# TropComplique/MultiPoseNet

Hardware: AMD Instinct MI355X
Metric: images/sec keypoint fwd+bwd+Adam @512x512 bs32/GPU (higher is better)
Workload: dtype bf16; 1 GPU; MobileNet-v1+FPN+keypoint_subnet fwd+bwd+Adam, 512x512, per-GPU batch 32; global_batch=32, parallelism=dp1, hip_graph=True, rccl_ranks=1

## Files before the change

### include/mpn.h

```cpp
#ifndef MPN_H_
#define MPN_H_

#include <stddef.h>
#include <stdint.h>

#ifdef __cplusplus
extern "C" {
#endif

#define MPN_VERSION 600

enum { MPN_F32 = 0, MPN_BF16 = 1, MPN_F16 = 2  };

enum {
    MPN_OK = 0,
    MPN_ERR_BAD_SHAPE = -1,
    MPN_ERR_BAD_DTYPE = -2,
    MPN_ERR_BAD_ALIGN = -3,
    MPN_ERR_HIP = -4,
    MPN_ERR_BAD_ARG = -5,
    MPN_ERR_WORKSPACE = -6,
    MPN_ERR_BAD_DATA = -7
};

enum { MPN_ACT_NONE = 0, MPN_ACT_RELU = 1, MPN_ACT_RELU6 = 2 };

typedef void* mpn_stream_t;

int mpn_version(void);
int mpn_last_error(char* buf, size_t n);

size_t mpn_heatmap_decode_workspace_bytes(int B);
int mpn_heatmap_decode(const void* heatmaps, int dtype, int B, int h, int w, int C,
                       const double* box_hw, float threshold,
                       int32_t* out_xyv, float* out_score, int32_t* out_index,
                       void* workspace, size_t workspace_bytes, mpn_stream_t stream);

size_t mpn_conv_packed_bytes(int Cin, int Cout, int ksize, int transpose, int dtype);
int mpn_conv_pack_weights(const float* w_hwio, int Cin, int Cout, int ksize, int transpose,
                          int dtype, void* out, mpn_stream_t stream);
size_t mpn_conv_pack_desc_bytes(void);
int mpn_conv_pack_desc_fill(void* desc_host, const float* w_hwio, int Cin, int Cout, int ksize, int transpose,
                            int dtype, void* out, int block_begin);
int mpn_conv_pack_weights_batched(const void* descs_device, int ndesc, int total_blocks, int dtype,
                                  mpn_stream_t stream);
int mpn_conv_num_parts(int N, int H, int W, int ksize);
int mpn_conv_stats_rows(int N, int H, int W, int Cin, int Cout, int ksize, int dtype);
int mpn_conv_fwd(const void* x, const void* w_packed, void* y, int N, int H, int W, int Cin,
                 int Cout, int x_stride, int y_stride, int ksize, int dtype, const float* in_scale,
                 const float* in_shift, int in_act, float* stats_part, const void* up_res,
                 mpn_stream_t stream);
int mpn_conv_fwd_grouped(int njobs, const void* const* x, const void* const* w_packed, void* const* y, int N, const int* H,
                         const int* W, int Cin, int Cout, const int* x_stride, const int* y_stride, int ksize, int dtype,
                         const float* const* in_scale, const float* const* in_shift, int in_act,
                         float* const* stats_part, mpn_stream_t stream);
int mpn_conv_bwd_data_bn_supported(int K, int C, int ksize, int dtype);
int mpn_conv_bwd_data_bn(const void* dy, const void* w_packed_t, void* dx, int N, int H, int W, int K, int C, int dy_stride,
                         int dx_stride, int ksize, int dtype, const void* bn_x, int bn_x_stride, const float* bn_scale,
                         const float* bn_shift, int bn_act, float* part, mpn_stream_t stream);
int mpn_conv_bwd_data_bn_grouped(int njobs, const void* const* dy, const void* const* w_packed_t, void* const* dx, int N,
                                 const int* H, const int* W, int K, int C, const int* dy_stride, const int* dx_stride,
                                 int dtype, const void* const* bn_x, const int* bn_x_stride, const float* const* bn_scale,
                                 const float* const* bn_shift, int bn_act, float* const* part, mpn_stream_t stream);

int mpn_conv_wgrad_num_parts(int N, int H, int W, int Cin, int Cout, int ksize, int dtype);
int mpn_conv_bwd_weight(const void* x, const void* dy, float* part, int N, int H, int W, int Cin,
                        int Cout, int x_stride, int dy_stride, int ksize, int dtype, const float* in_scale,
                        const float* in_shift, int in_act, mpn_stream_t stream);

int mpn_conv1x1_bwd_fused_supported(int Cin, int Cout, int dtype);
int mpn_conv1x1_bwd_fused(const void* x, const void* dy, const float* w, void* dx, float* wpart, float* bn_part, int N, int H, int W,
                          int Cin, int Cout, int x_stride, int dy_stride, int dx_stride, int dtype, const float* in_scale,
                          const float* in_shift, int in_act, mpn_stream_t stream);
int mpn_conv1x1_bwd_fused_apply_supported(int Cin, int Cout, int dtype);
int mpn_conv1x1_bwd_fused_apply(const void* x, const void* g, const void* y_raw, const float* w, void* dx, float* wpart, float* bn_part,
                                int N, int H, int W, int Cin, int Cout, int x_stride, int g_stride, int y_stride, int dx_stride,
                                int dtype, const float* in_scale, const float* in_shift, int in_act, const float* ap_scale,
                                const float* ap_shift, const float* ap_mean, const float* ap_invstd, const float* ap_k1,
                                const float* ap_k2, int ap_act, mpn_stream_t stream);
int mpn_conv_wgrad_grouped_num_parts(int njobs, int N, const int* H, const int* W, int Cin, int Cout, int ksize, int dtype,
                                     int* nparts);
int mpn_conv_bwd_weight_grouped(int njobs, const void* const* x, const void* const* dy, float* const* part, int N,
                                const int* H, const int* W, int Cin, int Cout, const int* x_stride, const int* dy_stride,
                                int ksize, int dtype, const float* const* in_scale, const float* const* in_shift,
                                int in_act, mpn_stream_t stream);

int mpn_bn_stats_num_parts(long long M);
int mpn_bn_stats(const void* x, long long M, int C, int dtype, float* part, mpn_stream_t stream);
int mpn_bn_finalize(float* part, int nparts, int C, long long count, const float* gamma,
                    const float* beta, float* moving_mean, float* moving_var, float momentum,
                    float eps, float* scale, float* shift, float* save_mean, float* save_invstd,
                    mpn_stream_t stream);
int mpn_bn_bwd_reduce_grouped(int njobs, void* const* dA, const void* const* x, const long long* M, int C, int dtype,
                              const float* const* scale, const float* const* shift, const float* const* mean,
                              const float* const* invstd, int act, float* const* part, const int* dA_stride,
                              const int* x_stride, mpn_stream_t stream);
int mpn_bn_bwd_apply_grouped(int njobs, void* const* dA, const void* const* x, const long long* M, int C, int dtype,
                             const float* const* scale, const float* const* shift, const float* const* mean,
                             const float* const* invstd, const float* const* k1, const float* const* k2, int act,
                             const float* const* add_ch0, const int* dA_stride, const int* x_stride,
                             mpn_stream_t stream);
size_t mpn_bn_fin_desc_bytes(void);
size_t mpn_bn_bwd_fin_desc_bytes(void);
int mpn_bn_fin_desc_fill(void* desc_host, const float* part, int nparts, int C, long long count, const float* gamma,
                         const float* beta, float* moving_mean, float* moving_var, float* scale, float* shift,
                         float* save_mean, float* save_invstd, int block_begin);
int mpn_bn_bwd_fin_desc_fill(void* desc_host, const float* part, int nparts, int C, long long count, float* dgamma,
                             float* dbeta, float* k1, float* k2, int block_begin);
int mpn_bn_bwd_fin_desc_fill_raw(void* desc_host, const float* part, int nparts, int C, long long count, float* dgamma,
                                 float* dbeta, float* k1, float* k2, const float* mean, const float* invstd,
                                 int block_begin);
int mpn_bn_finalize_batched(const void* descs_device, int ndesc, int total_blocks, float momentum, float eps,
                            mpn_stream_t stream);
int mpn_bn_bwd_finalize_batched(const void* descs_device, int ndesc, int total_blocks, mpn_stream_t stream);
int mpn_bn_inference_affine(int C, const float* gamma, const float* beta, const float* moving_mean,
                            const float* moving_var, float eps, float* scale, float* shift,
                            mpn_stream_t stream);
int mpn_bn_act_apply(const void* x, void* y, long long M, int C, int dtype, const float* scale,
                     const float* shift, int act, mpn_stream_t stream);
int mpn_bn_bwd_reduce(const void* dA, const void* x, long long M, int C, int dtype,
                      const float* scale, const float* shift, const float* mean,
                      const float* invstd, int act, float* part, mpn_stream_t stream);
int mpn_bn_bwd_finalize(float* part, int nparts, int C, long long count, float* dgamma,
                        float* dbeta, float* k1, float* k2, mpn_stream_t stream);
int mpn_bn_bwd_finalize_raw(float* part, int nparts, int C, long long count, float* dgamma, float* dbeta, float* k1,
                            float* k2, const float* mean, const float* invstd, mpn_stream_t stream);
int mpn_bn_bwd_apply(void* dA, const void* x, long long M, int C, int dtype, const float* scale,
                     const float* shift, const float* mean, const float* invstd, const float* k1,
                     const float* k2, int act, const float* add_ch0, mpn_stream_t stream);

int mpn_dwconv_out_size(int size, int stride);
int mpn_dwconv_num_parts(int N, int H, int W, int C, int stride, int dtype);
int mpn_dwconv_fwd(const void* x, const float* w, void* y, int N, int H, int W, int C, int stride,
                   int dtype, const float* in_scale, const float* in_shift, int in_act, int flip,
                   float* stats_part, mpn_stream_t stream);
int mpn_dwconv_bwd_data(const void* dy, const float* w, void* dx, int N, int H, int W, int C,
                        int stride, int dtype, mpn_stream_t stream);
int mpn_dwconv_bwd_data_bn_num_parts(int N, int H, int W, int C, int stride, int dtype);
int mpn_dwconv_bwd_data_bn(const void* dy, const float* w, void* dx, int N, int H, int W, int C, int stride, int dtype,
                           const void* x_bn, const float* scale, const float* shift, const float* mean,
                           const float* invstd, int act, float* part, mpn_stream_t stream);
int mpn_dwconv_bwd_data_add_supported(int N, int H, int W, int C, int stride, int dtype);
int mpn_dwconv_bwd_data_add(const void* dy, const float* w, void* dx, int N, int H, int W, int C, int stride, int dtype,
                            const void* addend, const void* x_bn, const float* scale, const float* shift,
                            const float* mean, const float* invstd, int act, float* part, mpn_stream_t stream);
int mpn_dwconv_wgrad_num_parts(int N, int H, int W, int C, int stride, int dtype);
int mpn_dwconv_bwd_weight(const void* x, const void* dy, float* part, int N, int H, int W, int C,
                          int stride, int dtype, const float* in_scale, const float* in_shift,
                          int in_act, mpn_stream_t stream);

int mpn_dwconv_bwd_fused_supported(int N, int H, int W, int C, int stride, int dtype);
int mpn_dwconv_bwd_fused(const void* x, const void* dy, const float* w, void* dx, float* wpart, int N, int H, int W, int C,
                         int dtype, const float* in_scale, const float* in_shift, int in_act, const float* mean,
                         const float* invstd, float* bn_part, mpn_stream_t stream);
int mpn_dwconv_bwd_fused_s2(const void* x, const void* dy, const float* w, void* dx, float* wpart, int N, int H, int W, int C,
                            int dtype, const float* in_scale, const float* in_shift, int in_act, const float* mean,
                            const float* invstd, float* bn_part, const void* addend, mpn_stream_t stream);
int mpn_dwconv_bwd_fused_apply_supported(int N, int H, int W, int C, int stride, int dtype);
int mpn_dwconv_bwd_fused_apply(const void* x, const void* g, const void* y_raw, const float* w, void* dx, float* wpart, int N, int H,
                               int W, int C, int dtype, const float* in_scale, const float* in_shift, int in_act, const float* mean,
                               const float* invstd, float* bn_part, const float* ap_scale, const float* ap_shift,
                               const float* ap_mean, const float* ap_invstd, const float* ap_k1, const float* ap_k2, int ap_act,
                               mpn_stream_t stream);
int mpn_dwconv_bwd_fused_s2_apply(const void* x, const void* g, const void* y_raw, const float* w, void* dx, float* wpart, int N, int H,
                                  int W, int C, int dtype, const float* in_scale, const float* in_shift, int in_act,
                                  const float* mean, const float* invstd, float* bn_part, const void* addend, const float* ap_scale,
                                  const float* ap_shift, const float* ap_mean, const float* ap_invstd, const float* ap_k1,
                                  const float* ap_k2, int ap_act, mpn_stream_t stream);

int mpn_stem_conv_fwd(const void* images, int images_u8, const float* w, void* y, int N, int H,
                      int W, int C0, int dtype, mpn_stream_t stream);
int mpn_stem_conv_fwd_num_parts(int N, int H, int W, int C0, int dtype);
int mpn_stem_conv_fwd_stats(const void* images, int images_u8, const float* w, void* y, int N, int H, int W, int C0,
                            int dtype, float* stats_part, mpn_stream_t stream);
int mpn_stem_conv_wgrad_num_parts(int N, int H, int W);
int mpn_stem_conv_bwd_weight(const void* images, int images_u8, const void* dy, float* part, int N,
                             int H, int W, int C0, int dtype, mpn_stream_t stream);

int mpn_bilinear_up_fwd(const void* x, void* y, int N, int h, int w, int C, int upsample,
                        int y_channel_offset, int y_channels_total, int dtype,
                        const float* in_scale, const float* in_shift, int in_act,
                        mpn_stream_t stream);
int mpn_bilinear_up_bwd(const void* dy, void* dx, int N, int h, int w, int C, int upsample,
                        int y_channel_offset, int y_channels_total, int dtype, mpn_stream_t stream);
int mpn_sumpool2x2(const void* src, void* dst, int N, int h, int w, int C, int accumulate,
                   int dtype, mpn_stream_t stream);
int mpn_add_inplace(void* dst, const void* src, long long n, int dtype, mpn_stream_t stream);

int mpn_heatmap_head_fwd(const void* x, const float* w, const float* bias, long long M, int Cin,
                         int dtype, const float* in_scale, const float* in_shift, int in_act,
                         int mode, float* out, float* out_seg, mpn_stream_t stream);
int mpn_heatmap_head_bwd_num_parts(long long M);
int mpn_heatmap_head_bwd(const void* x, const float* dlogits, const float* w, long long M, int Cin,
                         int dtype, const float* in_scale, const float* in_shift, int in_act,
                         void* dA, float* part, mpn_stream_t stream);
int mpn_heatmap_head_bwd_bn_supported(int Cin, int dtype);
int mpn_heatmap_head_bwd_bn(const void* x, const float* dlogits, const float* w, long long M, int Cin, int dtype,
                            const float* in_scale, const float* in_shift, int in_act, void* dA, float* part,
                            float* bn_part, mpn_stream_t stream);

int mpn_keypoint_loss_num_parts(int B, int h, int w);
int mpn_keypoint_loss(const float* logits, const float* heatmaps, const float* loss_masks,
                      const float* segmentation_masks, const int* num_boxes, const void* p2,
                      const void* p3, const void* p4, const void* p5, int p_channels, int p_dtype,
                      float* dlogits, float* daux2, float* daux3, float* daux4, float* daux5,
                      float* part, float* losses_out, int B, int h, int w, mpn_stream_t stream);

int mpn_adam_prepare(long long* step, float* hyper, double initial_learning_rate,
                     double decay_steps, double alpha, double beta1, double beta2,
                     mpn_stream_t stream);
int mpn_adam_step(float* params, const float* grads, float* m, float* v, long long n,
                  const float* hyper, float beta1, float beta2, float eps, float clip,
                  float grad_scale, mpn_stream_t stream);
int mpn_adam_step_cast(float* params, const float* grads, float* m, float* v, long long n, const float* hyper, float beta1,
                       float beta2, float eps, float clip, float grad_scale, int ncast, const long long* cast_begin,
                       const long long* cast_count, void* const* cast_dst, int cast_dtype, mpn_stream_t stream);
int mpn_reduce_partials(const float* part, int nparts, long long n, float* out, int accumulate,
                        float scale, mpn_stream_t stream);
size_t mpn_reduce_desc_bytes(void);
int mpn_reduce_desc_fill(void* desc_host, const float* part, int nparts, long long n, float* out, float scale,
                         int block_begin);
int mpn_reduce_partials_batched(const void* descs_device, int ndesc, int total_blocks, mpn_stream_t stream);
int mpn_axpy(long long n, float a, const float* x, float* y, mpn_stream_t stream);
int mpn_axpy_batched(int count, const float* const* x, float* const* y, const long long* n, float a, mpn_stream_t stream);
int mpn_l2_loss_accumulate(long long n, const float* w, float scale, float* acc, mpn_stream_t stream);
size_t mpn_l2_loss_batched_workspace_bytes(int count, const long long* n);
int mpn_l2_loss_batched(int count, const float* const* w, const long long* n, float scale, float* acc, void* workspace,
                        size_t workspace_bytes, mpn_stream_t stream);

size_t mpn_heatmap_render_workspace_bytes(int total_persons);
int mpn_heatmap_render(const int32_t* keypoints, const float* boxes, const int32_t* first_person,
                       int B, int total_persons, int width, int height, int downsample, float* out,
                       void* workspace, size_t workspace_bytes, mpn_stream_t stream);

enum {
    MPN_AUGMENT_ROTATE = 1, MPN_AUGMENT_COLOR = 2, MPN_AUGMENT_GRAYSCALE = 4, MPN_AUGMENT_PIXEL_SCALE = 8,
    MPN_AUGMENT_FLIP = 16, MPN_AUGMENT_EVAL = 32
};
#define MPN_KEYPOINT_AUGMENT_DESC_BYTES 192
typedef struct mpn_keypoint_augment_desc {
    int64_t src_offset, mask_offset;
    int32_t src_h, src_w, mask_h, mask_w;
    int32_t crop_y, crop_x, crop_h, crop_w;
    int32_t valid_h, valid_w, valid_mh, valid_mw;
    float transform[8], mask_transform[8];
    float window[4];
    float scale_y, scale_x;
    float mask_scale_y, mask_scale_x;
    float color[3];
    uint32_t seed;
    int32_t flags;
    int32_t reserved[3];
} mpn_keypoint_augment_desc;
#ifdef __cplusplus
static_assert(sizeof(mpn_keypoint_augment_desc) == MPN_KEYPOINT_AUGMENT_DESC_BYTES, "descriptor size is fixed");
#endif
size_t mpn_keypoint_augment_desc_bytes(void);
int mpn_keypoint_augment(const uint8_t* sources, const uint8_t* masks, const void* descs, int B, int H, int W,
                         float* images, float* loss_masks, float* segmentation_masks, mpn_stream_t stream);

// ... 358 lines not shown
```

### multiposenet_amd/_lib.py

```python
import ctypes
import os

_HERE = os.path.dirname(os.path.abspath(__file__))
LIB_PATH = os.environ.get("MPN_LIB") or os.path.join(_HERE, "libmpn_hip.so")

MPN_VERSION = 600
MPN_F32, MPN_BF16, MPN_F16 = 0, 1, 2
ACT_NONE, ACT_RELU, ACT_RELU6 = 0, 1, 2

_c = ctypes
_P = _c.c_void_p
_I = _c.c_int
_F = _c.c_float
_D = _c.c_double
_Z = _c.c_size_t
_L = _c.c_longlong

SIGNATURES = {
    "mpn_version": (_I, []),
    "mpn_last_error": (_I, [_c.c_char_p, _Z]),
    "mpn_heatmap_decode_workspace_bytes": (_Z, [_I]),
    "mpn_heatmap_decode": (_I, [_P, _I, _I, _I, _I, _I, _P, _F, _P, _P, _P, _P, _Z, _P]),
    "mpn_heatmap_render_workspace_bytes": (_Z, [_I]),
    "mpn_heatmap_render": (_I, [_P, _P, _P, _I, _I, _I, _I, _I, _P, _P, _Z, _P]),
    "mpn_keypoint_augment_desc_bytes": (_Z, []),
    "mpn_keypoint_augment": (_I, [_P, _P, _P, _I, _I, _I, _P, _P, _P, _P]),
    "mpn_detector_augment_desc_bytes": (_Z, []),
    "mpn_detector_augment": (_I, [_P, _P, _I, _I, _I, _P, _P]),
    "mpn_prn_example_desc_bytes": (_Z, []),
    "mpn_prn_examples_workspace_bytes": (_Z, [_I]),
    "mpn_prn_examples": (_I, [_P, _P, _I, _P, _P, _P, _I, _P, _I, _I, _I, _I, _P, _P, _P, _Z, _P]),
    "mpn_conv_packed_bytes": (_Z, [_I, _I, _I, _I, _I]),
    "mpn_conv_pack_weights": (_I, [_P, _I, _I, _I, _I, _I, _P, _P]),
    "mpn_conv_pack_desc_bytes": (_Z, []),
    "mpn_conv_pack_desc_fill": (_I, [_P, _P, _I, _I, _I, _I, _I, _P, _I]),
    "mpn_conv_pack_weights_batched": (_I, [_P, _I, _I, _I, _P]),
    "mpn_conv_num_parts": (_I, [_I, _I, _I, _I]),
    "mpn_conv_stats_rows": (_I, [_I, _I, _I, _I, _I, _I, _I]),
    "mpn_conv_fwd": (_I, [_P, _P, _P, _I, _I, _I, _I, _I, _I, _I, _I, _I, _P, _P, _I, _P, _P, _P]),
    "mpn_conv_fwd_grouped": (_I, [_I, _P, _P, _P, _I, _P, _P, _I, _I, _P, _P, _I, _I, _P, _P, _I, _P, _P]),
    "mpn_conv_wgrad_num_parts": (_I, [_I, _I, _I, _I, _I, _I, _I]),
    "mpn_conv_bwd_weight": (_I, [_P, _P, _P, _I, _I, _I, _I, _I, _I, _I, _I, _I, _P, _P, _I, _P]),
    "mpn_conv1x1_bwd_fused_supported": (_I, [_I, _I, _I]),
    "mpn_conv1x1_bwd_fused": (_I, [_P, _P, _P, _P, _P, _P, _I, _I, _I, _I, _I, _I, _I, _I, _I, _P, _P, _I, _P]),
    "mpn_conv1x1_bwd_fused_apply_supported": (_I, [_I, _I, _I]),
    "mpn_conv1x1_bwd_fused_apply": (_I, [_P, _P, _P, _P, _P, _P, _P, _I, _I, _I, _I, _I, _I, _I, _I, _I, _I, _P, _P, _I, _P, _P, _P, _P, _P, _P, _I, _P]),
    "mpn_conv_wgrad_grouped_num_parts": (_I, [_I, _I, _P, _P, _I, _I, _I, _I, _P]),
    "mpn_conv_bwd_weight_grouped": (_I, [_I, _P, _P, _P, _I, _P, _P, _I, _I, _P, _P, _I, _I, _P, _P, _I, _P]),
    "mpn_bn_stats_num_parts": (_I, [_L]),
    "mpn_bn_stats": (_I, [_P, _L, _I, _I, _P, _P]),
    "mpn_bn_finalize": (_I, [_P, _I, _I, _L, _P, _P, _P, _P, _F, _F, _P, _P, _P, _P, _P]),
    "mpn_bn_inference_affine": (_I, [_I, _P, _P, _P, _P, _F, _P, _P, _P]),
    "mpn_bn_act_apply": (_I, [_P, _P, _L, _I, _I, _P, _P, _I, _P]),
    "mpn_bn_bwd_reduce": (_I, [_P, _P, _L, _I, _I, _P, _P, _P, _P, _I, _P, _P]),
    "mpn_bn_bwd_finalize": (_I, [_P, _I, _I, _L, _P, _P, _P, _P, _P]),
    "mpn_bn_bwd_apply": (_I, [_P, _P, _L, _I, _I, _P, _P, _P, _P, _P, _P, _I, _P, _P]),
    "mpn_dwconv_out_size": (_I, [_I, _I]),
    "mpn_dwconv_num_parts": (_I, [_I, _I, _I, _I, _I, _I]),
    "mpn_dwconv_fwd": (_I, [_P, _P, _P, _I, _I, _I, _I, _I, _I, _P, _P, _I, _I, _P, _P]),
    "mpn_dwconv_bwd_data": (_I, [_P, _P, _P, _I, _I, _I, _I, _I, _I, _P]),
    "mpn_dwconv_bwd_data_bn_num_parts": (_I, [_I, _I, _I, _I, _I, _I]),
    "mpn_dwconv_bwd_data_bn": (_I, [_P, _P, _P, _I, _I, _I, _I, _I, _I, _P, _P, _P, _P, _P, _I, _P, _P]),
    "mpn_dwconv_bwd_data_add_supported": (_I, [_I, _I, _I, _I, _I, _I]),
    "mpn_dwconv_bwd_data_add": (_I, [_P, _P, _P, _I, _I, _I, _I, _I, _I, _P, _P, _P, _P, _P, _P, _I, _P, _P]),
    "mpn_dwconv_wgrad_num_parts": (_I, [_I, _I, _I, _I, _I, _I]),
    "mpn_dwconv_bwd_weight": (_I, [_P, _P, _P, _I, _I, _I, _I, _I, _I, _P, _P, _I, _P]),
    "mpn_dwconv_bwd_fused_supported": (_I, [_I, _I, _I, _I, _I, _I]),
    "mpn_dwconv_bwd_fused": (_I, [_P, _P, _P, _P, _P, _I, _I, _I, _I, _I, _P, _P, _I, _P, _P, _P, _P]),
    "mpn_dwconv_bwd_fused_s2": (_I, [_P, _P, _P, _P, _P, _I, _I, _I, _I, _I, _P, _P, _I, _P, _P, _P, _P, _P]),
    "mpn_dwconv_bwd_fused_apply_supported": (_I, [_I, _I, _I, _I, _I, _I]),
    "mpn_dwconv_bwd_fused_apply": (_I, [_P, _P, _P, _P, _P, _P, _I, _I, _I, _I, _I, _P, _P, _I, _P, _P, _P, _P, _P, _P, _P, _P, _P, _I, _P]),
    "mpn_dwconv_bwd_fused_s2_apply": (_I, [_P, _P, _P, _P, _P, _P, _I, _I, _I, _I, _I, _P, _P, _I, _P, _P, _P, _P, _P, _P, _P, _P, _P, _P, _I, _P]),
    "mpn_stem_conv_fwd": (_I, [_P, _I, _P, _P, _I, _I, _I, _I, _I, _P]),
    "mpn_stem_conv_fwd_num_parts": (_I, [_I, _I, _I, _I, _I]),
    "mpn_stem_conv_fwd_stats": (_I, [_P, _I, _P, _P, _I, _I, _I, _I, _I, _P, _P]),
    "mpn_stem_conv_wgrad_num_parts": (_I, [_I, _I, _I]),
    "mpn_stem_conv_bwd_weight": (_I, [_P, _I, _P, _P, _I, _I, _I, _I, _I, _P]),
    "mpn_bilinear_up_fwd": (_I, [_P, _P, _I, _I, _I, _I, _I, _I, _I, _I, _P, _P, _I, _P]),
    "mpn_bilinear_up_bwd": (_I, [_P, _P, _I, _I, _I, _I, _I, _I, _I, _I, _P]),
    "mpn_sumpool2x2": (_I, [_P, _P, _I, _I, _I, _I, _I, _I, _P]),
    "mpn_add_inplace": (_I, [_P, _P, _L, _I, _P]),
    "mpn_heatmap_head_fwd": (_I, [_P, _P, _P, _L, _I, _I, _P, _P, _I, _I, _P, _P, _P]),
    "mpn_heatmap_head_bwd_num_parts": (_I, [_L]),
    "mpn_heatmap_head_bwd": (_I, [_P, _P, _P, _L, _I, _I, _P, _P, _I, _P, _P, _P]),
    "mpn_heatmap_head_bwd_bn_supported": (_I, [_I, _I]),
    "mpn_heatmap_head_bwd_bn": (_I, [_P, _P, _P, _L, _I, _I, _P, _P, _I, _P, _P, _P, _P]),
    "mpn_keypoint_loss_num_parts": (_I, [_I, _I, _I]),
    "mpn_keypoint_loss": (_I, [_P] * 9 + [_I, _I] + [_P] * 7 + [_I, _I, _I, _P]),
    "mpn_adam_prepare": (_I, [_P, _P, _D, _D, _D, _D, _D, _P]),
    "mpn_adam_step": (_I, [_P, _P, _P, _P, _L, _P, _F, _F, _F, _F, _F, _P]),
    "mpn_adam_step_cast": (_I, [_P, _P, _P, _P, _L, _P, _F, _F, _F, _F, _F, _I, _P, _P, _P, _I, _P]),
    "mpn_reduce_partials": (_I, [_P, _I, _L, _P, _I, _F, _P]),
    "mpn_reduce_desc_bytes": (_Z, []),
    "mpn_reduce_desc_fill": (_I, [_P, _P, _I, _L, _P, _F, _I]),
    "mpn_reduce_partials_batched": (_I, [_P, _I, _I, _P]),
    "mpn_gemm_nt_num_parts": (_I, [_I]),
    "mpn_gemm_nt": (_I, [_P, _P, _P, _I, _I, _I, _I, _P]),
    "mpn_transpose_cast": (_I, [_P, _I, _P, _I, _I, _I, _P]),
    "mpn_cast": (_I, [_P, _I, _P, _I, _L, _P]),
    "mpn_bias_relu_fwd": (_I, [_P, _I, _P, _P, _I, _I, _I, _P]),
    "mpn_bias_relu_bwd": (_I, [_P, _I, _P, _P, _I, _P, _I, _I, _P]),
    "mpn_prn_loss": (_I, [_P, _P, _I, _P, _I, _I, _I, _P, _P, _P, _F, _P]),
    "mpn_bn_bwd_reduce_grouped": (_I, [_I, _P, _P, _P, _I, _I, _P, _P, _P, _P, _I, _P, _P, _P, _P]),
    "mpn_bn_bwd_apply_grouped": (_I, [_I, _P, _P, _P, _I, _I, _P, _P, _P, _P, _P, _P, _I, _P, _P, _P, _P]),
    "mpn_bn_fin_desc_bytes": (_Z, []),
    "mpn_bn_bwd_fin_desc_bytes": (_Z, []),
    "mpn_bn_fin_desc_fill": (_I, [_P, _P, _I, _I, _L, _P, _P, _P, _P, _P, _P, _P, _P, _I]),
    "mpn_bn_bwd_fin_desc_fill": (_I, [_P, _P, _I, _I, _L, _P, _P, _P, _P, _I]),
    "mpn_bn_finalize_batched": (_I, [_P, _I, _I, _F, _F, _P]),
    "mpn_bn_bwd_finalize_batched": (_I, [_P, _I, _I, _P]),
    "mpn_heatmap_minmax": (_I, [_P, _I, _I, _I, _I, _P, _P]),
    "mpn_prn_crop": (_I, [_P, _P, _P, _P, _I, _I, _I, _I, _I, _I, _I, _F, _P, _P]),
    "mpn_prn_decode": (_I, [_P, _I, _I, _I, _I, _P, _P, _P]),
    "mpn_conv_bwd_data_bn_supported": (_I, [_I, _I, _I, _I]),
    "mpn_conv_bwd_data_bn": (_I, [_P, _P, _P, _I, _I, _I, _I, _I, _I, _I, _I, _I, _P, _I, _P, _P, _I, _P, _P]),
    "mpn_bn_bwd_finalize_raw": (_I, [_P, _I, _I, _L, _P, _P, _P, _P, _P, _P, _P]),
    "mpn_conv_bwd_data_bn_grouped": (_I, [_I, _P, _P, _P, _I, _P, _P, _I, _I, _P, _P, _I, _P, _P, _P, _P, _I, _P, _P]),
    "mpn_bn_bwd_fin_desc_fill_raw": (_I, [_P, _P, _I, _I, _L, _P, _P, _P, _P, _P, _P, _I]),
    "mpn_prn_crop_slots": (_I, [_P, _P, _P, _P, _I, _I, _I, _I, _I, _I, _I, _I, _I, _F, _P, _P]),
    "mpn_prn_residual": (_I, [_P, _P, _I, _L, _P, _P]),
    "mpn_retina_loss_finalize": (_I, [_P, _P, _F, _F, _P, _P, _P, _P]),
    "mpn_axpy": (_I, [_L, _F, _P, _P, _P]),
    "mpn_axpy_batched": (_I, [_I, _P, _P, _P, _F, _P]),
    "mpn_patchify3x3s2": (_I, [_P, _P, _I, _I, _I, _I, _I, _P, _P, _I, _P]),
    "mpn_unpatchify3x3s2": (_I, [_P, _P, _I, _I, _I, _I, _I, _P]),
    "mpn_retina_match_workspace_bytes": (_Z, [_I, _I]),
    "mpn_retina_match": (_I, [_P, _P, _P, _I, _I, _I, _F, _F, _P, _P, _P, _P, _Z, _P]),
    "mpn_retina_loss_num_parts": (_I, [_I, _I]),
    "mpn_retina_loss": (_I, [_P, _P, _P, _P, _P, _P, _I, _P, _P, _P, _P, _P, _I, _F, _F, _F, _F, _P, _P]),
    "mpn_retina_nms_workspace_bytes": (_Z, [_I, _I]),
    "mpn_retina_nms_overflow_offset": (_Z, [_I, _I]),
    "mpn_retina_nms": (_I, [_P, _P, _P, _P, _I, _P, _P, _P, _I, _F, _F, _I, _P, _P, _P, _P, _Z, _P]),
    "mpn_l2_loss_accumulate": (_I, [_L, _P, _F, _P, _P]),
    "mpn_l2_loss_batched_workspace_bytes": (_Z, [_I, _P]),
    "mpn_l2_loss_batched": (_I, [_I, _P, _P, _F, _P, _P, _Z, _P]),
    "mpn_pose_gather_record_bytes": (_Z, [_I, _I]),
    "mpn_pose_gather_row_offset": (_Z, [_I, _I, _I]),
    "mpn_pose_gather": (_I, [_P, _P, _P, _P, _P, _P, _I, _I, _F, _I, _I, _P, _Z, _P]),
    "mpn_pose_gather_sized": (_I, [_P, _P, _P, _P, _P, _P, _I, _I, _F, _P, _P, _Z, _P]),
    "mpn_oks_gt_row_bytes": (_Z, []),
    "mpn_oks_match_out_bytes": (_Z, [_I, _I]),
    "mpn_oks_match": (_I, [_P, _I, _I, _P, _P, _I, _P, _I, _I, _I, _P, _P, _P]),
    "mpn_pose_nms_info_bytes": (_Z, [_I, _I]),
    "mpn_pose_nms": (_I, [_P, _I, _I, _F, _F, _I, _P, _Z, _P, _Z, _P, _P]),
    "mpn_pose_track_state_bytes": (_Z, [_I, _I]),
    "mpn_pose_track_out_bytes": (_Z, [_I, _I]),
    "mpn_pose_track": (_I, [_P, _I, _I, _I, _I, _I, _F, _F, _I, _P, _P, _P, _P]),
    "mpn_pose_track_optimal": (_I, [_P, _I, _I, _I, _I, _I, _F, _F, _I, _P, _P, _P, _P]),
    "mpn_pose_track_motion_state_bytes": (_Z, [_I, _I]),
    "mpn_pose_track_coast_bytes": (_Z, [_I, _I]),
    "mpn_pose_track_motion": (_I, [_P, _I, _I, _I, _I, _I, _I, _F, _F, _I, _F, _F, _P, _P, _P, _P, _P, _P, _P]),
    "mpn_pose_smooth_state_bytes": (_Z, [_I, _I]),
    "mpn_pose_smooth_out_bytes": (_Z, [_I, _I]),
    "mpn_pose_smooth": (_I, [_P, _P, _I, _I, _I, _I, _F, _F, _F, _F, _F, _P, _P, _P, _P]),
    "mpn_coco_masks_image_desc_bytes": (_Z, []),
    "mpn_coco_masks_part_desc_bytes": (_Z, []),
    "mpn_coco_masks_plane_words": (_Z, [_I, _I]),
    "mpn_coco_masks_packed_bytes": (_Z, [_I, _I]),
    "mpn_coco_masks": (_I, [_P, _I, _I, _P, _I, _P, _L, _P, _L, _P, _L, _P, _Z, _P, _Z, _P, _Z, _P]),
    "mpn_image_resize_desc_bytes": (_Z, []),
# ... 169 lines not shown
```

### multiposenet_amd/csrc/conv_wgrad.hip

```cpp
#include "common.h"
#include <type_traits>

namespace {

template <typename T> using HT = H16<std::conditional_t<sizeof(T) == 2, T, bf16_t>>;
typedef float f32x4_t __attribute__((ext_vector_type(4)));

constexpr int kThreads = 256;
constexpr int kHaloW = 18, kHaloH = 10;

struct WgradParams {
    const void* x;
    const void* dy;
    float* part;
    const float* in_scale;
    const float* in_shift;
    int in_act;
    int N, H, W, Cin, Cout;
    int xs, dys;
    int tiles_x, tiles_y;
    long long M;
    int ntiles;
    int nsplit;
    int n_cg, n_cb;
    int xcd_remap;
    const float* wf;
    void* dx;
    int dxs;
    float* bn_part;
    const void* ap_x;
    int ap_xs;
    const float* ap_scale; const float* ap_shift; const float* ap_mean; const float* ap_invstd; const float* ap_k1; const float* ap_k2;
    int ap_act;
#ifdef MPN_DIAG
    unsigned long long* dbg;
#endif
};

__device__ __forceinline__ int fsw256(int r) { return (r & 3) | (((r >> 3) & 1) << 2); }
__device__ __forceinline__ int fsw64(int) { return 0; }
__device__ __forceinline__ int fsw128(int r) { return ((r >> 1) & 1) | (((r >> 3) & 1) << 1); }

template <int RB> __device__ __forceinline__ int lds_off(int row, int seg, int within) {
    const int f = (RB == 64) ? fsw64(row) : (RB == 128 ? fsw128(row) : fsw256(row));
    return row * RB + ((seg ^ f) << 5) + within;
}

template <typename T> struct Raw4h { uint2 v; };
__device__ __forceinline__ void raw4_unpack(const Raw4h<bf16_t>& r, float (&f)[4]) {
    f[0] = __uint_as_float(r.v.x << 16); f[1] = __uint_as_float(r.v.x & 0xffff0000u);
    f[2] = __uint_as_float(r.v.y << 16); f[3] = __uint_as_float(r.v.y & 0xffff0000u);
}
__device__ __forceinline__ void raw4_unpack(const Raw4h<half_t>& r, float (&f)[4]) {
    typedef _Float16 h2_t __attribute__((ext_vector_type(2)));
    const h2_t a = __builtin_bit_cast(h2_t, r.v.x), b = __builtin_bit_cast(h2_t, r.v.y);
    f[0] = (float)a[0]; f[1] = (float)a[1]; f[2] = (float)b[0]; f[3] = (float)b[1];
}
template <typename T> __device__ __forceinline__ float round_to_storage(float v);
template <> __device__ __forceinline__ float round_to_storage<bf16_t>(float v) { return to_f32((bf16_t)v); }
template <> __device__ __forceinline__ float round_to_storage<half_t>(float v) { return (float)(_Float16)v; }
template <typename T> __device__ __forceinline__ uint2 pack4_storage(const float (&g)[4]);
template <> __device__ __forceinline__ uint2 pack4_storage<bf16_t>(const float (&g)[4]) {
    return make_uint2(pack_bf16x2(g[0], g[1]), pack_bf16x2(g[2], g[3]));
}
template <> __device__ __forceinline__ uint2 pack4_storage<half_t>(const float (&g)[4]) {
    typedef _Float16 h2_t __attribute__((ext_vector_type(2)));
    const h2_t a = {(_Float16)g[0], (_Float16)g[1]}, b = {(_Float16)g[2], (_Float16)g[3]};
    return make_uint2(__builtin_bit_cast(unsigned, a), __builtin_bit_cast(unsigned, b));
}

template <typename H> __device__ __forceinline__ typename H::x4 tr_read(const unsigned char* base, int off) {
    return H::tr_read(base + off);
}

template <typename T, int TAPS, int RBA, int RBD>
__global__ __launch_bounds__(kThreads, 2) void conv_wgrad_kernel(const WgradParams p) {
    constexpr int ES = (int)sizeof(T);
    constexpr int VE = 16 / ES;
    constexpr int CG = RBA / ES;
    constexpr int BNW = RBD / ES;
    constexpr int DSLOTS = RBD / 16;
    constexpr int NPIXA = TAPS == 9 ? kHaloW * kHaloH : 128;
    constexpr int MT_TOTAL = CG / 16, NT_TOTAL = BNW / 16;
    constexpr int WM = MT_TOTAL >= 2 ? 2 : 1;
    constexpr int WN = 4 / WM;
    constexpr int MTW = MT_TOTAL / WM;
    constexpr int NTW = NT_TOTAL / WN;
    constexpr int KPIX = ES == 2 ? 32 : 4;
    constexpr int KSTEPS = 128 / KPIX;
    constexpr int ASLOTS = RBA / 16;
    constexpr int AVEC = (NPIXA * ASLOTS + kThreads - 1) / kThreads;
    constexpr int DVEC = 128 * DSLOTS / kThreads;

    extern __shared__ __attribute__((aligned(16))) unsigned char smem[];
    unsigned char* As = smem;
    unsigned char* Ds = smem + NPIXA * RBA;

    const int tid = threadIdx.x;
    const int lane = tid & 63, wave = tid >> 6;
    const int l15 = lane & 15, lq = lane >> 4;

    int b;
    {
        const int nwg = gridDim.x, q = nwg >> 3, r = nwg & 7, xcd = blockIdx.x & 7, k = blockIdx.x >> 3;
        b = (xcd < r ? xcd * (q + 1) : r * (q + 1) + (xcd - r) * q) + k;
    }
    const int cg = b % p.n_cg; b /= p.n_cg;
    const int cb = b % p.n_cb;
    const int split = b / p.n_cb;
    const int ci0 = cg * CG, co0 = cb * BNW;

    const int mt0 = (wave / WN) * MTW;
    const int nt0 = (wave % WN) * NTW;

    f32x4_t acc[TAPS][MTW][NTW];
#pragma unroll
// ... 166 lines not shown
    for (int t = 0; t < TAPS; ++t)
#pragma unroll
        for (int i = 0; i < MTW; ++i)
#pragma unroll
            for (int j = 0; j < NTW; ++j)
#pragma unroll
                for (int r = 0; r < 4; ++r) {
                    const int ci = ci0 + (mt0 + i) * 16 + lq * 4 + r;
                    const int co = co0 + (nt0 + j) * 16 + l15;
                    if (ci < p.Cin && co < p.Cout)
                        dst[((long long)t * p.Cin + ci) * p.Cout + co] = acc[t][i][j][r];
                }
}

template <typename T, int TAPS, int RBA, int RBD, int WM, bool STAGGER, bool DG = false, bool DAPPLY = false>
__device__ __forceinline__ void conv_wgrad_bf16_body(const WgradParams& p, const int blk, const int nblk) {
    using H = H16<T>;
    using X8 = typename H::x8;
    using X4 = typename H::x4;
    constexpr int NT = 512;
    constexpr int VE = 8;
    constexpr int CG = RBA / 2, BNW = RBD / 2;
    constexpr int ASLOTS = RBA / 16, DSLOTS = RBD / 16;
    constexpr int NPIXA = TAPS == 9 ? kHaloW * kHaloH : 128;
    constexpr int MT_TOTAL = CG / 16, NT_TOTAL = BNW / 16;
    constexpr int WN = 8 / WM;
    constexpr int MTW = MT_TOTAL / WM, NTW = NT_TOTAL / WN;
    static_assert(MTW * WM == MT_TOTAL && NTW * WN == NT_TOTAL, "wave layout must tile the block");
    constexpr int AVEC = (NPIXA * ASLOTS + NT - 1) / NT;
    constexpr int DVEC = 128 * DSLOTS / NT;
    constexpr int SA = RBA + 32, SD = RBD + 32;
    constexpr int ABYTES = NPIXA * SA, DBYTES = 128 * SD;
    static_assert(!DG || (TAPS == 1 && !STAGGER), "the fused data gradient: 1x1, waves in step");
    constexpr int OS = RBA + 16;
    constexpr int RBYTES = DG ? 128 * SA : 0, OBYTES = DG ? 128 * OS : 0;
    constexpr int KS2 = BNW / 32;

    constexpr int NBUF = DG ? 1 : 2;
    extern __shared__ __attribute__((aligned(16))) unsigned char smem[];
    float* aff = reinterpret_cast<float*>(smem + NBUF * ABYTES + NBUF * DBYTES);
    unsigned char* Rs = smem + NBUF * ABYTES + NBUF * DBYTES + 2 * CG * (int)sizeof(float);
    unsigned char* Os = Rs + RBYTES;

    const int tid = threadIdx.x;
    const int lane = tid & 63, wave = tid >> 6;
    const int l15 = lane & 15, lq = lane >> 4;

    int b = blk;
    if (p.xcd_remap) {
        const int nwg = nblk, q = nwg >> 3, r = nwg & 7, xcd = blk & 7, k = blk >> 3;
        b = (xcd < r ? xcd * (q + 1) : r * (q + 1) + (xcd - r) * q) + k;
    }
    const int cg = b % p.n_cg; b /= p.n_cg;
    const int cb = b % p.n_cb;
    const int split = b / p.n_cb;
    const int ci0 = cg * CG, co0 = cb * BNW;
    const int mt0 = (wave / WN) * MTW, nt0 = (wave % WN) * NTW;

    f32x4_t acc[TAPS][MTW][NTW];
#pragma unroll
    for (int t = 0; t < TAPS; ++t)
#pragma unroll
        for (int i = 0; i < MTW; ++i)
#pragma unroll
            for (int j = 0; j < NTW; ++j) acc[t][i][j] = (f32x4_t){0.f, 0.f, 0.f, 0.f};

    const T* __restrict__ x = reinterpret_cast<const T*>(p.x);
    const T* __restrict__ dy = reinterpret_cast<const T*>(p.dy);
    const bool affine = p.in_scale != nullptr;
    const float lo = (affine && p.in_act != MPN_ACT_NONE) ? 0.f : -INFINITY;
    const float hi = (affine && p.in_act == MPN_ACT_RELU6) ? 6.f : INFINITY;
    for (int c = tid; c < CG; c += NT) {
        const bool ok = affine && ci0 + c < p.Cin;
        aff[c] = ok ? p.in_scale[ci0 + c] : 1.f;
        aff[CG + c] = ok ? p.in_shift[ci0 + c] : 0.f;
    }

    const int aslot = tid % ASLOTS;
    const int dslot = tid % DSLOTS;

    Vec16<T> v[AVEC], dv[DVEC];
    Vec16<T> ev[DAPPLY ? DVEC : 1];
    unsigned inb = 0u, inbd = 0u;
    static_assert(!DAPPLY || DG, "the apply pass folds into the fused thin backward");
    float* apc = reinterpret_cast<float*>(Os + OBYTES + (DG ? 8 * 2 * CG * (int)sizeof(float) : 0));
    float alo = -INFINITY, ahi = INFINITY;
    if constexpr (DAPPLY) {
        for (int c = tid; c < BNW; c += NT) {
            const bool ok = co0 + c < p.Cout;
            const float s_ = ok ? p.ap_scale[co0 + c] : 0.f, h_ = ok ? p.ap_shift[co0 + c] : 0.f, m_ = ok ? p.ap_mean[co0 + c] : 0.f;
            const float i_ = ok ? p.ap_invstd[co0 + c] : 0.f, a_ = ok ? p.ap_k1[co0 + c] : 0.f, b_ = ok ? p.ap_k2[co0 + c] : 0.f;
            apc[c] = s_; apc[BNW + c] = h_;
            apc[2 * BNW + c] = -s_ * b_ * i_;
            apc[3 * BNW + c] = -s_ * (a_ - m_ * i_ * b_);
        }
        alo = (p.ap_act != MPN_ACT_NONE) ? 0.f : -INFINITY;
        ahi = (p.ap_act == MPN_ACT_RELU6) ? 6.f : INFINITY;
    }

    int relA[AVEC], hyx[AVEC], relD[DVEC];
    {
        const int ace = ci0 + aslot * VE, dce = co0 + dslot * VE;
#pragma unroll
        for (int i = 0; i < AVEC; ++i) {
            const int vi = tid + i * NT;
            const int pix = vi / ASLOTS;
            const bool ok = ace < p.Cin && vi < NPIXA * ASLOTS;
            if (TAPS == 9) {
                const int hy = pix / kHaloW, hx = pix - hy * kHaloW;
                relA[i] = ((hy - 1) * p.W + (hx - 1)) * p.xs + ace;
                hyx[i] = ok ? (hy << 8 | hx) : 0x7fff00;
            } else {
                relA[i] = pix * p.xs + ace;
                hyx[i] = ok ? pix : 0x7fffffff;
            }
        }
#pragma unroll
        for (int i = 0; i < DVEC; ++i) {
            const int r = (tid / DSLOTS) + i * (NT / DSLOTS);
            relD[i] = (TAPS == 9 ? ((r >> 4) * p.W + (r & 15)) : r) * p.dys + dce;
        }
    }
    const bool dvalid = co0 + dslot * VE < p.Cout;
    const int drow0 = tid / DSLOTS;
    constexpr bool BUF = TAPS == 1;
    typedef unsigned u32x4_t __attribute__((ext_vector_type(4)));
    unsigned relAb[BUF ? AVEC : 1], relDb[BUF ? DVEC : 1], relEb[(BUF && DAPPLY) ? DVEC : 1];
    __amdgpu_buffer_rsrc_t rsx, rsd, rse;
    if constexpr (BUF) {
        constexpr unsigned kOut = 0x80000000u;
#pragma unroll
        for (int i = 0; i < AVEC; ++i) relAb[i] = hyx[i] == 0x7fffffff ? kOut : (unsigned)relA[i] * (unsigned)sizeof(T);
#pragma unroll
        for (int i = 0; i < DVEC; ++i) relDb[i] = dvalid ? (unsigned)relD[i] * (unsigned)sizeof(T) : kOut;
        rsx = __builtin_amdgcn_make_buffer_rsrc(const_cast<T*>(x), 0, (int)(((p.M - 1) * p.xs + p.Cin) * (long long)sizeof(T)), 0x00020000);
        rsd = __builtin_amdgcn_make_buffer_rsrc(const_cast<T*>(dy), 0, (int)(((p.M - 1) * p.dys + p.Cout) * (long long)sizeof(T)), 0x00020000);
        if constexpr (DAPPLY) {
#pragma unroll
            for (int i = 0; i < DVEC; ++i)
                relEb[i] = dvalid ? (unsigned)((drow0 + i * (NT / DSLOTS)) * p.ap_xs + co0 + dslot * VE) * (unsigned)sizeof(T) : kOut;
            rse = __builtin_amdgcn_make_buffer_rsrc(const_cast<void*>(p.ap_x), 0, (int)(((p.M - 1) * p.ap_xs + p.Cout) * (long long)sizeof(T)), 0x00020000);
        }
    }

    auto load_tile = [&](int tile) {
        if constexpr (BUF) {
            const unsigned tbA = (unsigned)tile * 128u * (unsigned)p.xs * (unsigned)sizeof(T);
            const unsigned tbD = (unsigned)tile * 128u * (unsigned)p.dys * (unsigned)sizeof(T);
            if constexpr (DAPPLY) {
                const int mleft = (int)(p.M - (long long)tile * 128);
                unsigned md = 0u;
#pragma unroll
                for (int i = 0; i < DVEC; ++i) md |= ((dvalid && drow0 + i * (NT / DSLOTS) < mleft) ? 1u : 0u) << i;
                inbd = md;
            }
            __builtin_amdgcn_sched_barrier(0);
#pragma unroll
            for (int i = 0; i < AVEC; ++i) {
                const u32x4_t q = __builtin_amdgcn_raw_buffer_load_b128(rsx, (int)(relAb[i] + tbA), 0, 0);
                v[i].raw = make_uint4(q.x, q.y, q.z, q.w);
            }
#pragma unroll
            for (int i = 0; i < DVEC; ++i) {
                const u32x4_t q = __builtin_amdgcn_raw_buffer_load_b128(rsd, (int)(relDb[i] + tbD), 0, 0);
                dv[i].raw = make_uint4(q.x, q.y, q.z, q.w);
            }
            if constexpr (DAPPLY) {
                const unsigned tbE = (unsigned)tile * 128u * (unsigned)p.ap_xs * (unsigned)sizeof(T);
#pragma unroll
                for (int i = 0; i < DVEC; ++i) {
                    const u32x4_t q = __builtin_amdgcn_raw_buffer_load_b128(rse, (int)(relEb[i] + tbE), 0, 0);
                    ev[i].raw = make_uint4(q.x, q.y, q.z, q.w);
                }
            }
            __builtin_amdgcn_sched_barrier(0);
            return;
        }
        int oy0 = 0, ox0 = 0, baseA, baseD, mleft = 0;
        if (TAPS == 9) {
            const int tx = tile % p.tiles_x;
            const int t2 = tile / p.tiles_x;
            const int ty = t2 % p.tiles_y;
            const int img = t2 / p.tiles_y;
            oy0 = ty * 8;
            ox0 = tx * 16;
            const int pix0 = (img * p.H + oy0) * p.W + ox0;
            baseA = pix0 * p.xs;
            baseD = pix0 * p.dys;
        } else {
            baseA = tile * 128 * p.xs;
            baseD = tile * 128 * p.dys;
            mleft = (int)(p.M - (long long)tile * 128);
        }
        int oa[AVEC], od[DVEC];
        unsigned ma = 0u, md = 0u;
#pragma unroll
        for (int i = 0; i < AVEC; ++i) {
            bool ok;
            if (TAPS == 9) {
                const int iy = oy0 + (hyx[i] >> 8) - 1, ix = ox0 + (hyx[i] & 255) - 1;
                ok = (unsigned)iy < (unsigned)p.H && (unsigned)ix < (unsigned)p.W;
            } else {
                ok = hyx[i] < mleft;
            }
            oa[i] = ok ? baseA + relA[i] : 0;
            ma |= (ok ? 1u : 0u) << i;
        }
#pragma unroll
        for (int i = 0; i < DVEC; ++i) {
            const int r = drow0 + i * (NT / DSLOTS);
            bool ok = dvalid;
            if (TAPS == 9) ok = ok && oy0 + (r >> 4) < p.H && ox0 + (r & 15) < p.W;
            else ok = ok && r < mleft;
            od[i] = ok ? baseD + relD[i] : 0;
            md |= (ok ? 1u : 0u) << i;
        }
        inb = ma;
        inbd = md;
        __builtin_amdgcn_sched_barrier(0);
#pragma unroll
        for (int i = 0; i < AVEC; ++i) v[i].load(x + oa[i]);
#pragma unroll
        for (int i = 0; i < DVEC; ++i) dv[i].load(dy + od[i]);
        if constexpr (DAPPLY) {
            const T* __restrict__ ax = reinterpret_cast<const T*>(p.ap_x);
#pragma unroll
            for (int i = 0; i < DVEC; ++i) {
                const int r = drow0 + i * (NT / DSLOTS);
                const bool ok = (inbd >> i) & 1u;
                ev[i].load(ax + (ok ? (long long)(tile * 128 + r) * p.ap_xs + co0 + dslot * VE : 0));
            }
        }
        __builtin_amdgcn_sched_barrier(0);
    };

    auto commit_tile = [&](unsigned char* As, unsigned char* Ds) {
        float sc[VE], sh[VE];
        if (affine) {
#pragma unroll
            for (int j = 0; j < VE; j += 4) {
                const float4 a = *reinterpret_cast<const float4*>(aff + aslot * VE + j);
                const float4 c = *reinterpret_cast<const float4*>(aff + CG + aslot * VE + j);
                sc[j] = a.x; sc[j + 1] = a.y; sc[j + 2] = a.z; sc[j + 3] = a.w;
                sh[j] = c.x; sh[j + 1] = c.y; sh[j + 2] = c.z; sh[j + 3] = c.w;
            }
        }
#pragma unroll
        for (int i = 0; i < AVEC; ++i) {
            const int vi = tid + i * NT;
            if (vi < NPIXA * ASLOTS) {
                const int pix = vi / ASLOTS;
                uint4 q = *reinterpret_cast<const uint4*>(&v[i].raw);
                if (affine) {
                    float f[VE];
                    v[i].unpack(f);
#pragma unroll
                    for (int j = 0; j < VE; ++j) f[j] = __builtin_amdgcn_fmed3f(f[j] * sc[j] + sh[j], lo, hi);
                    Vec16<T> o;
                    o.pack(f);
                    q = *reinterpret_cast<const uint4*>(&o.raw);
                }
                if (!BUF && !((inb >> i) & 1u)) q = make_uint4(0u, 0u, 0u, 0u);
                *reinterpret_cast<uint4*>(As + pix * SA + aslot * 16) = q;
                if constexpr (DG) {
                    uint4 r = *reinterpret_cast<const uint4*>(&v[i].raw);
                    if (!BUF && !((inb >> i) & 1u)) r = make_uint4(0u, 0u, 0u, 0u);
                    *reinterpret_cast<uint4*>(Rs + pix * SA + aslot * 16) = r;
                }
            }
        }
#pragma unroll
        for (int i = 0; i < DVEC; ++i) {
            const int r = (tid / DSLOTS) + i * (NT / DSLOTS);
            uint4 q = *reinterpret_cast<const uint4*>(&dv[i].raw);
            if constexpr (DAPPLY) {
                float d[VE], f[VE], asc[VE], ash[VE], acb[VE], acc_[VE];
                dv[i].unpack(d);
                ev[i].unpack(f);
#pragma unroll
                for (int j4 = 0; j4 < VE; j4 += 4) {
                    const f32x4_t q0 = *reinterpret_cast<const f32x4_t*>(apc + dslot * VE + j4), q1 = *reinterpret_cast<const f32x4_t*>(apc + BNW + dslot * VE + j4);
                    const f32x4_t q2 = *reinterpret_cast<const f32x4_t*>(apc + 2 * BNW + dslot * VE + j4), q3 = *reinterpret_cast<const f32x4_t*>(apc + 3 * BNW + dslot * VE + j4);
#pragma unroll
                    for (int j = 0; j < 4; ++j) { asc[j4 + j] = q0[j]; ash[j4 + j] = q1[j]; acb[j4 + j] = q2[j]; acc_[j4 + j] = q3[j]; }
                }
#pragma unroll
                for (int j = 0; j < VE; ++j) {
                    const float pre = f[j] * asc[j] + ash[j];
                    const float gg = (pre > alo && pre < ahi) ? d[j] : 0.f;
                    d[j] = asc[j] * gg + (acb[j] * f[j] + acc_[j]);
                }
                Vec16<T> o;
                o.pack(d);
                q = *reinterpret_cast<const uint4*>(&o.raw);
            }
            if ((!BUF || DAPPLY) && !((inbd >> i) & 1u)) q = make_uint4(0u, 0u, 0u, 0u);
            *reinterpret_cast<uint4*>(Ds + r * SD + dslot * 16) = q;
        }
    };

#ifdef MPN_DIAG
    unsigned long long ph[4] = {0, 0, 0, 0}, t_prev = 0;
#define MPN_WG_STAMP(k) do { if (p.dbg) { const unsigned long long t_ = __builtin_amdgcn_s_memtime(); \
                                          ph[k] += t_ - t_prev; t_prev = t_; } } while (0)
#else
#define MPN_WG_STAMP(k) do { } while (0)
#endif
    const int grp = STAGGER ? wave >> 2 : 0;
    const int ntl = p.ntiles > split ? (p.ntiles - split + p.nsplit - 1) / p.nsplit : 0;
    const int ahead = 1 + grp;
    constexpr int DGS = MT_TOTAL >= 8 ? 4 : (MT_TOTAL >= 4 ? 2 : 1), MTH = MT_TOTAL / DGS;
    const int dg_mt0 = DG ? (wave % DGS) * MTH : 0, dg_pt0 = DG ? (wave / DGS) * DGS : 0;
    X8 wfr[DG ? MTH : 1][DG ? KS2 : 1];
    float bsum[DG ? MTH : 1][4], bsq[DG ? MTH : 1][4];
    if constexpr (DG) {
#pragma unroll
        for (int mt = 0; mt < MTH; ++mt) {
#pragma unroll
            for (int ks = 0; ks < KS2; ++ks) {
                const int ci = ci0 + (dg_mt0 + mt) * 16 + l15, co = co0 + ks * 32 + lq * 8;
                float f[8];
#pragma unroll
                for (int j = 0; j < 8; ++j) f[j] = (ci < p.Cin && co + j < p.Cout) ? p.wf[(long long)ci * p.Cout + co + j] : 0.f;
                Vec16<T> o;
                o.pack(f);
                wfr[mt][ks] = __builtin_bit_cast(X8, o.raw);
            }
#pragma unroll
            for (int r = 0; r < 4; ++r) { bsum[mt][r] = 0.f; bsq[mt][r] = 0.f; }
        }
    }
    if (ntl > 0) load_tile(split);
    __syncthreads();
    if (ntl > 0) commit_tile(smem, smem + NBUF * ABYTES);
    if (grp == 1) {
        if (ntl > 1) load_tile(split + p.nsplit);
        __syncthreads();
        if (ntl > 1) commit_tile(smem + ABYTES, smem + NBUF * ABYTES + DBYTES);
    }
#ifdef MPN_DIAG
    if (p.dbg) t_prev = __builtin_amdgcn_s_memtime();
#endif
#pragma unroll 1
    for (int it = 0; it < ntl; ++it) {
        const int buf = NBUF == 2 ? (it & 1) : 0;
        unsigned char* As = smem + buf * ABYTES;
        unsigned char* Ds = smem + NBUF * ABYTES + buf * DBYTES;
        const bool more = it + ahead < ntl;
        if (more) load_tile(split + (it + ahead) * p.nsplit);
        MPN_WG_STAMP(1);
        __syncthreads();
        MPN_WG_STAMP(2);
        const int qq = l15 >> 2, pp = l15 & 3;
        const unsigned char* a_lane = As + (4 * lq + qq) * SA + pp * 8 + mt0 * 32;
        const unsigned char* d_lane = Ds + (4 * lq + qq) * SD + pp * 8 + nt0 * 32;
        constexpr int STEPS = TAPS * MTW;
        constexpr int TOTAL = 4 * STEPS;
        constexpr int RING0 = NTW >= 4 ? 4 : ((TAPS == 9 && RBA == 256) ? 4 : 6);
        constexpr int RING = RING0 < STEPS ? RING0 : STEPS;
        constexpr int KSA = (TAPS == 9 ? 2 * kHaloW : 32) * SA, KSD = 32 * SD;
        auto a_load = [&](int gs) -> X8 {
            const int ks = gs / STEPS, step = gs % STEPS;
            const int t = step / MTW, i = step % MTW;
            const int row = TAPS == 9 ? (t / 3) * kHaloW + (t % 3) : 0;
            const int second = TAPS == 9 ? kHaloW : 16;
            const X4 l4 = tr_read<H>(a_lane, ks * KSA + row * SA + i * 32);
            const X4 h4 = tr_read<H>(a_lane, ks * KSA + (row + second) * SA + i * 32);
            return __builtin_shufflevector(l4, h4, 0, 1, 2, 3, 4, 5, 6, 7);
        };
        auto b_load = [&](int ks, int j) -> X8 {
            const X4 l4 = tr_read<H>(d_lane, ks * KSD + j * 32);
            const X4 h4 = tr_read<H>(d_lane, ks * KSD + 16 * SD + j * 32);
            return __builtin_shufflevector(l4, h4, 0, 1, 2, 3, 4, 5, 6, 7);
        };
        X8 bfr[2][NTW];
        X8 ar[RING];
#pragma unroll
        for (int j = 0; j < NTW; ++j) bfr[0][j] = b_load(0, j);
#pragma unroll
        for (int r = 0; r < RING - 1; ++r) ar[r] = a_load(r);
// ... 40 lines not shown
                        const float pre = xf[r] * sc4[r] + sh4[r];
                        const float d = round_to_storage<T>(dacc[mt][r]);
                        g[r] = (!bnr || (pre > lo && pre < hi)) ? d : 0.f;
                        bsum[mt][r] += g[r];
                        bsq[mt][r] += g[r] * xf[r];
                    }
                    *reinterpret_cast<uint2*>(Os + px * OS + cl * 2) = pack4_storage<T>(g);
                }
            }
        }
        MPN_WG_STAMP(3);
        __syncthreads();
        MPN_WG_STAMP(2);
        if (more) {
            const int nb = NBUF == 2 ? ((it + ahead) & 1) : 0;
            commit_tile(smem + nb * ABYTES, smem + NBUF * ABYTES + nb * DBYTES);
        }
        if constexpr (DG) {
            const int tile = split + it * p.nsplit;
            const int mleft = (int)(p.M - (long long)tile * 128);
            T* __restrict__ dxp = reinterpret_cast<T*>(p.dx) + (long long)tile * 128 * p.dxs + ci0;
            for (int v0 = tid; v0 < 128 * ASLOTS; v0 += NT) {
                const int pr = v0 / ASLOTS, sl = v0 - pr * ASLOTS;
                if (pr < mleft && ci0 + sl * 8 < p.Cin)
                    *reinterpret_cast<uint4*>(dxp + (long long)pr * p.dxs + sl * 8) = *reinterpret_cast<const uint4*>(Os + pr * OS + sl * 16);
            }
        }
        MPN_WG_STAMP(0);
    }
    if (STAGGER && grp == 0) __syncthreads();
#ifdef MPN_DIAG
    if (p.dbg && lane == 0) {
#pragma unroll
        for (int k = 0; k < 4; ++k) p.dbg[((size_t)blockIdx.x * 8 + wave) * 4 + k] = ph[k];
    }
#endif
#undef MPN_WG_STAMP

    if constexpr (DG) {
        float* red = reinterpret_cast<float*>(Os + OBYTES);
        __syncthreads();
        for (int o = tid; o < 8 * 2 * CG; o += NT) red[o] = 0.f;
        __syncthreads();
#pragma unroll
        for (int mt = 0; mt < MTH; ++mt)
#pragma unroll
            for (int r = 0; r < 4; ++r) {
                float a = bsum[mt][r], b = bsq[mt][r];
#pragma unroll
                for (int o = 1; o < 16; o <<= 1) { a += __shfl_xor(a, o, 64); b += __shfl_xor(b, o, 64); }
                if (l15 == 0) {
                    red[(wave * 2 + 0) * CG + (dg_mt0 + mt) * 16 + lq * 4 + r] = a;
                    red[(wave * 2 + 1) * CG + (dg_mt0 + mt) * 16 + lq * 4 + r] = b;
                }
            }
        __syncthreads();
        for (int o = tid; o < 2 * CG; o += NT) {
            const int which = o / CG, c = o - which * CG;
            if (p.bn_part != nullptr && ci0 + c < p.Cin) {
                float a = 0.f;
#pragma unroll
                for (int w8 = 0; w8 < 8; ++w8) a += red[(w8 * 2 + which) * CG + c];
                p.bn_part[((long long)split * 2 + which) * p.Cin + ci0 + c] = a;
            }
        }
    }
    float* __restrict__ dst = p.part + (long long)split * TAPS * p.Cin * p.Cout;
#pragma unroll
    for (int t = 0; t < TAPS; ++t)
#pragma unroll
        for (int i = 0; i < MTW; ++i)
#pragma unroll
            for (int j = 0; j < NTW; ++j)
#pragma unroll
                for (int r = 0; r < 4; ++r) {
                    const int ci = ci0 + (mt0 + i) * 16 + lq * 4 + r;
                    const int co = co0 + (nt0 + j) * 16 + l15;
                    if (ci < p.Cin && co < p.Cout) {
                        __builtin_nontemporal_store(acc[t][i][j][r], &dst[((long long)t * p.Cin + ci) * p.Cout + co]);
                    }
                }
}

template <typename T, int TAPS, int RBA, int RBD, int WM, bool STAGGER>
__global__ __launch_bounds__(512, 1) void conv_wgrad_bf16_kernel(const WgradParams p) {
    conv_wgrad_bf16_body<T, TAPS, RBA, RBD, WM, STAGGER>(p, blockIdx.x, gridDim.x);
}

template <typename T, int RBA, int RBD, int WM, bool DAPPLY>
__global__ __launch_bounds__(512, 1) void conv1x1_bwd_fused_kernel(const WgradParams p) {
    conv_wgrad_bf16_body<T, 1, RBA, RBD, WM, false, true, DAPPLY>(p, blockIdx.x, gridDim.x);
}

constexpr int kMaxWgradGroup = 5;
struct WgradGroup {
    WgradParams p[kMaxWgradGroup];
    int begin[kMaxWgradGroup + 1];
    int njobs;
};
template <typename T, int TAPS, int RBA, int RBD, int WM, bool STAGGER>
__global__ __launch_bounds__(512, 1) void conv_wgrad_bf16_grouped_kernel(const WgradGroup g) {
    int job = 0;
#pragma unroll
    for (int j = 1; j < kMaxWgradGroup; ++j)
        if (j < g.njobs && (int)blockIdx.x >= g.begin[j]) job = j;
    conv_wgrad_bf16_body<T, TAPS, RBA, RBD, WM, STAGGER>(g.p[job], (int)blockIdx.x - g.begin[job], g.begin[job + 1] - g.begin[job]);
}

struct WgradGeom {
    int n_cg, n_cb, ntiles, nsplit;
};

static bool wgrad_thin1x1(int Cin, int Cout, int ksize) { return ksize == 1 && Cin <= 32 && Cout <= 64; }

WgradGeom wgrad_geom(int N, int H, int W, int Cin, int Cout, int ksize, int es) {
    WgradGeom g;
    int cgsz, bnw, blocks;
    if (es == 2) {
        const bool narrow = ksize == 3 && Cout <= 64;
        cgsz = (ksize == 3 && !narrow) ? 64 : 128;
        bnw = narrow ? 64 : 128;
        if (wgrad_thin1x1(Cin, Cout, ksize)) { cgsz = 32; bnw = 64; }
        blocks = 256;
    } else {
        const bool narrow = ksize == 3 && Cout * es <= 128;
        cgsz = (narrow ? 128 : (ksize == 3 ? 64 : 256)) / es;
        bnw = (narrow ? 128 : 256) / es;
        blocks = 512;
    }
    g.n_cg = (Cin + cgsz - 1) / cgsz;
    g.n_cb = (Cout + bnw - 1) / bnw;
    g.ntiles = ksize == 3 ? N * ((H + 7) / 8) * ((W + 15) / 16) : (int)(((long long)N * H * W + 127) / 128);
    int ns = blocks / (g.n_cg * g.n_cb);
    if (ns < 1) ns = 1;
    const int min_tiles = es == 2 ? 4 : 1;
    if (ns > g.ntiles / min_tiles) ns = g.ntiles / min_tiles;
    if (ns < 1) ns = 1;
    g.nsplit = ns;
    return g;
}

template <int TAPS, int RBA, int RBD> constexpr int wgrad16_smem_bytes() {
    constexpr int smem = 2 * (TAPS == 9 ? kHaloW * kHaloH : 128) * (RBA + 32) + 2 * 128 * (RBD + 32) + 2 * (RBA / 2) * (int)sizeof(float);
    static_assert(smem <= 160 * 1024, "LDS budget");
    return smem;
}

template <int TAPS, int RBA, int RBD, int WM, bool STAGGER> struct Wgrad16 {};

template <typename T, int TAPS, int RBA, int RBD, int WM, bool STAGGER>
int launch_wgrad_bf16_grouped(Wgrad16<TAPS, RBA, RBD, WM, STAGGER>, const WgradGroup& g, int blocks, hipStream_t st) {
    constexpr int smem = wgrad16_smem_bytes<TAPS, RBA, RBD>();
    static mpn_attr_mask_t attr_mask{0};
    MPN_HIP(mpn_ensure_dynamic_lds((const void*)conv_wgrad_bf16_grouped_kernel<T, TAPS, RBA, RBD, WM, STAGGER>, smem, &attr_mask));
    conv_wgrad_bf16_grouped_kernel<T, TAPS, RBA, RBD, WM, STAGGER><<<dim3((unsigned)blocks), dim3(512), smem, st>>>(g);
    MPN_LAUNCH_CHECK();
    return MPN_OK;
}

int wgrad_group_lay(WgradGroup& grp, int njobs) {
    int begin = 0;
    for (int j = 0; j < njobs; ++j) {
        WgradParams& p = grp.p[j];
        const int blocks = p.n_cg * p.n_cb * p.nsplit;
        if (njobs > 1) p.xcd_remap = (begin % 8 == 0 && blocks % 8 == 0) ? 1 : 0;
        grp.begin[j] = begin;
        begin += blocks;
    }
    for (int j = njobs; j <= kMaxWgradGroup; ++j) grp.begin[j] = begin;
    grp.njobs = njobs;
    return begin;
}

template <typename T, int TAPS, int RBA, int RBD, int WM, bool STAGGER>
int launch_wgrad_bf16(Wgrad16<TAPS, RBA, RBD, WM, STAGGER>, const WgradParams& p, hipStream_t st) {
    constexpr int smem = wgrad16_smem_bytes<TAPS, RBA, RBD>();
    static mpn_attr_mask_t attr_mask{0};
    MPN_HIP(mpn_ensure_dynamic_lds((const void*)conv_wgrad_bf16_kernel<T, TAPS, RBA, RBD, WM, STAGGER>, smem, &attr_mask));
    conv_wgrad_bf16_kernel<T, TAPS, RBA, RBD, WM, STAGGER><<<dim3((unsigned)(p.n_cg * p.n_cb * p.nsplit)), dim3(512), smem, st>>>(p);
    MPN_LAUNCH_CHECK();
    return MPN_OK;
}
template <typename T>
int launch_wgrad_bf16(Wgrad16<9, 128, 256, 4, true> wide, const WgradParams& p, hipStream_t st) {
    WgradGroup grp = {};
    grp.p[0] = p;
    const int blocks = wgrad_group_lay(grp, 1);
    return launch_wgrad_bf16_grouped<T>(wide, grp, blocks, st);
}

template <typename Launch>
int wgrad16_dispatch(int Cin, int Cout, int ksize, Launch&& launch) {
    if (wgrad_thin1x1(Cin, Cout, ksize)) return launch(Wgrad16<1, 64, 128, 2, false>{});
    if (ksize == 1) return launch(Wgrad16<1, 256, 256, 4, false>{});
    if (Cout <= 64) return launch(Wgrad16<9, 256, 128, 4, true>{});
    return launch(Wgrad16<9, 128, 256, 4, true>{});
}

template <typename T, int TAPS, int RBA, int RBD>
int launch_wgrad_g(const WgradParams& p, hipStream_t st) {
    constexpr int NPIXA = TAPS == 9 ? kHaloW * kHaloH : 128;
    constexpr int smem = NPIXA * RBA + 128 * RBD;
    static mpn_attr_mask_t attr_mask{0};
    MPN_HIP(mpn_ensure_dynamic_lds((const void*)conv_wgrad_kernel<T, TAPS, RBA, RBD>, smem, &attr_mask));
    conv_wgrad_kernel<T, TAPS, RBA, RBD><<<dim3((unsigned)(p.n_cg * p.n_cb * p.nsplit)), dim3(kThreads), smem, st>>>(p);
    MPN_LAUNCH_CHECK();
    return MPN_OK;
}

template <typename T, int TAPS>
int launch_wgrad(const WgradParams& p, hipStream_t st) {
    constexpr int ES = (int)sizeof(T);
    if (TAPS == 9 && p.Cout * ES <= 128) return launch_wgrad_g<T, TAPS, 128, 128>(p, st);
    return launch_wgrad_g<T, TAPS, (TAPS == 9 ? 64 : 256), 256>(p, st);
}

#ifdef MPN_DIAG
void* g_wgrad_dbg = nullptr;
#endif

int wgrad_check_layer(const char* who, int N, int Cin, int Cout, int ksize, int dtype) {
    MPN_REQUIRE(ksize == 1 || ksize == 3, MPN_ERR_BAD_SHAPE, "%s: ksize must be 1 or 3", who);
    MPN_REQUIRE(dtype == MPN_F32 || dtype == MPN_BF16 || dtype == MPN_F16, MPN_ERR_BAD_DTYPE, "%s: dtype %d", who, dtype);
    const int ve = dtype == MPN_F32 ? 4 : 8;
    MPN_REQUIRE(N > 0 && Cin > 0 && Cout > 0 && Cin % ve == 0 && Cout % ve == 0, MPN_ERR_BAD_SHAPE,
                "%s: bad shape (channels must be multiples of %d)", who, ve);
    return MPN_OK;
}

int wgrad_fill_job(WgradParams& p, const char* who, const void* x, const void* dy, float* part, int N, int H, int W, int Cin, int Cout,
                   int x_stride, int dy_stride, int ksize, int es, const float* in_scale, const float* in_shift, int in_act,
                   const WgradGeom& g, int nsplit) {
    const int ve = 16 / es;
    MPN_REQUIRE(x && dy && part, MPN_ERR_BAD_ARG, "%s: null pointer", who);
    MPN_REQUIRE(mpn_aligned16(x) && mpn_aligned16(dy), MPN_ERR_BAD_ALIGN, "%s: pointers must be 16-byte aligned", who);
    MPN_REQUIRE((in_scale == nullptr) == (in_shift == nullptr), MPN_ERR_BAD_ARG, "%s: scale/shift mismatch", who);
    MPN_REQUIRE(N > 0 && H > 0 && W > 0, MPN_ERR_BAD_SHAPE, "%s: bad size %d x %d x %d", who, N, H, W);
    p = {};
    p.x = x; p.dy = dy; p.part = part;
    p.in_scale = in_scale; p.in_shift = in_shift; p.in_act = in_act;
    p.N = N; p.H = H; p.W = W; p.Cin = Cin; p.Cout = Cout;
    p.xs = x_stride > 0 ? x_stride : Cin; p.dys = dy_stride > 0 ? dy_stride : Cout;
    MPN_REQUIRE(p.xs >= Cin && p.dys >= Cout && p.xs % ve == 0 && p.dys % ve == 0, MPN_ERR_BAD_SHAPE,
                "%s: pixel strides (%d, %d) must be multiples of %d not below the channel counts", who, x_stride, dy_stride, ve);
    p.M = (long long)N * H * W;
    MPN_REQUIRE(p.M * p.xs < (1ll << 31) && p.M * p.dys < (1ll << 31), MPN_ERR_BAD_SHAPE, "%s: tensors must span fewer than 2^31 elements", who);
    MPN_REQUIRE(ksize != 1 || es != 2 || (p.M * p.xs < (1ll << 30) && p.M * p.dys < (1ll << 30)), MPN_ERR_BAD_SHAPE,
                "%s: 16-bit 1x1 tensors must span fewer than 2^31 bytes", who);
    p.tiles_x = (W + 15) / 16; p.tiles_y = (H + 7) / 8;
    p.ntiles = g.ntiles; p.nsplit = nsplit; p.n_cg = g.n_cg; p.n_cb = g.n_cb; p.xcd_remap = 1;
    return MPN_OK;
}

}

#ifdef MPN_DIAG
extern "C" void mpn_diag_set_wgrad_stamps(void* buf) { g_wgrad_dbg = buf; }
#endif

extern "C" int mpn_conv_wgrad_num_parts(int N, int H, int W, int Cin, int Cout, int ksize, int dtype) {
    return wgrad_geom(N, H, W, Cin, Cout, ksize, dtype == MPN_F32 ? 4 : 2).nsplit;
}

extern "C" int mpn_conv_bwd_weight(const void* x, const void* dy, float* part, int N, int H, int W, int Cin, int Cout,
                                   int x_stride, int dy_stride, int ksize, int dtype, const float* in_scale,
                                   const float* in_shift, int in_act, mpn_stream_t stream) {
    if (int rc = wgrad_check_layer("conv wgrad", N, Cin, Cout, ksize, dtype)) return rc;
    const int es = dtype == MPN_F32 ? 4 : 2;
    const WgradGeom g = wgrad_geom(N, H, W, Cin, Cout, ksize, es);
    WgradParams p;
    if (int rc = wgrad_fill_job(p, "conv wgrad", x, dy, part, N, H, W, Cin, Cout, x_stride, dy_stride, ksize, es, in_scale, in_shift, in_act,
                                g, g.nsplit))
        return rc;
#ifdef MPN_DIAG
    p.dbg = (unsigned long long*)g_wgrad_dbg;
#endif
    hipStream_t st = (hipStream_t)stream;
    if (dtype == MPN_F32) return ksize == 3 ? launch_wgrad<float, 9>(p, st) : launch_wgrad<float, 1>(p, st);
    if (dtype == MPN_F16)
        return wgrad16_dispatch(Cin, Cout, ksize, [&](auto geo) { return launch_wgrad_bf16<half_t>(geo, p, st); });
    return wgrad16_dispatch(Cin, Cout, ksize, [&](auto geo) { return launch_wgrad_bf16<bf16_t>(geo, p, st); });
}

namespace {

void wgrad_group_splits(int njobs, int N, const int* H, const int* W, int Cin, int Cout, int ksize, int* nsplit, WgradGeom* geoms) {
    long long total_tiles = 0;
    for (int j = 0; j < njobs; ++j) {
        geoms[j] = wgrad_geom(N, H[j], W[j], Cin, Cout, ksize, 2);
        total_tiles += geoms[j].ntiles;
    }
    const int units = geoms[0].n_cg * geoms[0].n_cb;
    int quantum = 1;
    while ((quantum * units) % 8 != 0) ++quantum;
    int budget = 256 / units;
    if (budget < quantum * njobs) budget = quantum * njobs;
    int used = 0, big = 0;
    for (int j = 0; j < njobs; ++j) {
        const double ideal = (double)budget * geoms[j].ntiles / (double)total_tiles;
        long long ns = ideal >= 4.0 * quantum ? (long long)ideal / quantum * quantum : (long long)(ideal + 0.5);
        const int cap = geoms[j].ntiles / 4 > 0 ? geoms[j].ntiles / 4 : 1;
        if (ns > cap) ns = cap;
        if (ns < 1) ns = 1;
        nsplit[j] = (int)ns;
        used += (int)ns;
        if (geoms[j].ntiles > geoms[big].ntiles) big = j;
    }
    while (used > budget && nsplit[big] > quantum) { nsplit[big] -= quantum; used -= quantum; }
    while (used + quantum <= budget && nsplit[big] + quantum <= geoms[big].ntiles / 4) { nsplit[big] += quantum; used += quantum; }
}

bool wgrad_groupable(int njobs, int dtype) { return njobs >= 2 && njobs <= kMaxWgradGroup && (dtype == MPN_BF16 || dtype == MPN_F16); }

}

extern "C" int mpn_conv_wgrad_grouped_num_parts(int njobs, int N, const int* H, const int* W, int Cin, int Cout, int ksize, int dtype,
                                                int* nparts) {
    MPN_REQUIRE(njobs > 0 && H && W && nparts, MPN_ERR_BAD_ARG, "conv wgrad grouped: bad arguments");
    if (!wgrad_groupable(njobs, dtype)) {
        for (int j = 0; j < njobs; ++j) nparts[j] = mpn_conv_wgrad_num_parts(N, H[j], W[j], Cin, Cout, ksize, dtype);
        return MPN_OK;
    }
    WgradGeom geoms[kMaxWgradGroup];
    wgrad_group_splits(njobs, N, H, W, Cin, Cout, ksize, nparts, geoms);
    return MPN_OK;
}

extern "C" int mpn_conv_bwd_weight_grouped(int njobs, const void* const* x, const void* const* dy, float* const* part, int N,
                                           const int* H, const int* W, int Cin, int Cout, const int* x_stride, const int* dy_stride,
                                           int ksize, int dtype, const float* const* in_scale, const float* const* in_shift,
                                           int in_act, mpn_stream_t stream) {
    const char* who = "conv wgrad grouped";
    MPN_REQUIRE(njobs > 0 && x && dy && part && H && W && in_scale && in_shift, MPN_ERR_BAD_ARG, "%s: bad arguments", who);
    if (!wgrad_groupable(njobs, dtype)) {
        for (int j = 0; j < njobs; ++j)
            if (int rc = mpn_conv_bwd_weight(x[j], dy[j], part[j], N, H[j], W[j], Cin, Cout, x_stride ? x_stride[j] : 0,
                                             dy_stride ? dy_stride[j] : 0, ksize, dtype, in_scale[j], in_shift[j], in_act, stream))
                return rc;
        return MPN_OK;
    }
    if (int rc = wgrad_check_layer(who, N, Cin, Cout, ksize, dtype)) return rc;
    WgradGeom geoms[kMaxWgradGroup];
    int nsplit[kMaxWgradGroup];
    wgrad_group_splits(njobs, N, H, W, Cin, Cout, ksize, nsplit, geoms);
    WgradGroup grp = {};
    for (int j = 0; j < njobs; ++j)
        if (int rc = wgrad_fill_job(grp.p[j], who, x[j], dy[j], part[j], N, H[j], W[j], Cin, Cout, x_stride ? x_stride[j] : 0,
                                    dy_stride ? dy_stride[j] : 0, ksize, 2, in_scale[j], in_shift[j], in_act, geoms[j], nsplit[j]))
            return rc;
    const int blocks = wgrad_group_lay(grp, njobs);
    hipStream_t st = (hipStream_t)stream;
    if (dtype == MPN_F16) return wgrad16_dispatch(Cin, Cout, ksize, [&](auto geo) { return launch_wgrad_bf16_grouped<half_t>(geo, grp, blocks, st); });
    return wgrad16_dispatch(Cin, Cout, ksize, [&](auto geo) { return launch_wgrad_bf16_grouped<bf16_t>(geo, grp, blocks, st); });
}

namespace {
template <typename T, int RBA, int RBD, int WM, bool DAPPLY = false>
int launch_conv1x1_bwd_fused(const WgradParams& p, hipStream_t st) {
    constexpr int CG = RBA / 2;
    constexpr int smem = 128 * (RBA + 32) + 128 * (RBD + 32) + 2 * CG * (int)sizeof(float) + 128 * (RBA + 32) + 128 * (RBA + 16) +
                         8 * 2 * CG * (int)sizeof(float) + (DAPPLY ? 4 * (RBD / 2) * (int)sizeof(float) : 0);
    static_assert(smem <= 160 * 1024, "LDS budget");
    static mpn_attr_mask_t attr_mask{0};
    MPN_HIP(mpn_ensure_dynamic_lds((const void*)conv1x1_bwd_fused_kernel<T, RBA, RBD, WM, DAPPLY>, smem, &attr_mask));
// ... 65 lines not shown
```

### multiposenet_amd/csrc/dwconv_walk.h

```cpp
#pragma once
#include "common.h"

namespace {

constexpr int kThreads = 256;
typedef float f32x2_t __attribute__((ext_vector_type(2)));
typedef __bf16 bf16x2_t __attribute__((ext_vector_type(2)));

template <typename T> struct Raw4;
template <> struct Raw4<float> { float4 v; };
template <> struct Raw4<bf16_t> { uint2 v; };
__device__ __forceinline__ void raw_load(Raw4<float>& r, const float* p) { r.v = *reinterpret_cast<const float4*>(p); }
__device__ __forceinline__ void raw_load(Raw4<bf16_t>& r, const bf16_t* p) { r.v = *reinterpret_cast<const uint2*>(p); }
__device__ __forceinline__ void raw_unpack(const Raw4<float>& r, float (&f)[4]) { f[0] = r.v.x; f[1] = r.v.y; f[2] = r.v.z; f[3] = r.v.w; }
__device__ __forceinline__ void raw_unpack(const Raw4<bf16_t>& r, float (&f)[4]) {
    f[0] = __uint_as_float(r.v.x << 16); f[1] = __uint_as_float(r.v.x & 0xffff0000u);
    f[2] = __uint_as_float(r.v.y << 16); f[3] = __uint_as_float(r.v.y & 0xffff0000u);
}
template <typename T> __device__ __forceinline__ void raw_unpack2(const Raw4<T>& r, f32x2_t& v01, f32x2_t& v23) {
    float f[4];
    raw_unpack(r, f);
    v01 = (f32x2_t){f[0], f[1]};
    v23 = (f32x2_t){f[2], f[3]};
}
__device__ __forceinline__ void store4x2(float* p, f32x2_t a, f32x2_t b) {
    *reinterpret_cast<float4*>(p) = make_float4(a.x, a.y, b.x, b.y);
}
__device__ __forceinline__ void store4x2(bf16_t* p, f32x2_t a, f32x2_t b) {
    const bf16x2_t lo = __builtin_convertvector(a, bf16x2_t), hi = __builtin_convertvector(b, bf16x2_t);
    uint2 q;
    q.x = __builtin_bit_cast(unsigned, lo);
    q.y = __builtin_bit_cast(unsigned, hi);
    *reinterpret_cast<uint2*>(p) = q;
}
template <typename T> __device__ __forceinline__ f32x2_t round_storage(f32x2_t a);
template <> __device__ __forceinline__ f32x2_t round_storage<float>(f32x2_t a) { return a; }
template <> __device__ __forceinline__ f32x2_t round_storage<bf16_t>(f32x2_t a) {
    return __builtin_convertvector(__builtin_convertvector(a, bf16x2_t), f32x2_t);
}

__device__ __forceinline__ int xcd_work_id() {
    const int wid = blockIdx.x, nwg = gridDim.x, q = nwg >> 3, r = nwg & 7, xcd = wid & 7;
    return (xcd < r ? xcd * (q + 1) : r * (q + 1) + (xcd - r) * q) + (wid >> 3);
}

struct SwLane {
    int img, yb, cgb, unit;
    int ox;
    int cc;
    bool ok;
};
template <int XT, bool CB_INNER>
__device__ __forceinline__ SwLane sw_lane(int C, int OW, int ncg, int cols, int xblocks, int yblocks, int cblocks) {
    SwLane l;
    int b = xcd_work_id(), xb;
    if (CB_INNER) {
        l.cgb = b % cblocks; b /= cblocks;
        l.unit = b;
        xb = b % xblocks; b /= xblocks;
        l.yb = b % yblocks;
        l.img = b / yblocks;
    } else {
        xb = b % xblocks; b /= xblocks;
        l.yb = b % yblocks; b /= yblocks;
        l.cgb = b % cblocks;
        l.img = b / cblocks;
        l.unit = (l.img * yblocks + l.yb) * xblocks + xb;
    }
    const int cgl = threadIdx.x % ncg, col = threadIdx.x / ncg;
    const int c = (l.cgb * ncg + cgl) * 4, ox = (xb * cols + col) * XT;
    l.ok = c < C && ox < OW && col < cols;
    l.cc = l.ok ? c : 0;
    l.ox = l.ok ? ox : 0;
    return l;
}

struct InAffine {
    f32x2_t sc01, sc23, sh01, sh23;
    float lo, hi;
    template <bool NULLABLE>
    __device__ __forceinline__ void load(const float* scale, const float* shift, int act, int cc) {
        const bool on = !NULLABLE || scale != nullptr;
        float4 s4 = make_float4(1.f, 1.f, 1.f, 1.f), h4 = make_float4(0.f, 0.f, 0.f, 0.f);
        if (on) { s4 = *reinterpret_cast<const float4*>(scale + cc); h4 = *reinterpret_cast<const float4*>(shift + cc); }
// ... 34 lines not shown
    long long rstep;
    __device__ __forceinline__ void init(int ix0, bool lane_ok, int H_, int W, int C) {
        H = H_;
        rstep = (long long)W * C;
#pragma unroll
        for (int k = 0; k < NC; ++k) {
            const int ix = ix0 + k;
            ok[k] = lane_ok && ix >= 0 && ix < W;
            off[k] = (ok[k] ? ix : 0) * C;
        }
    }
    __device__ __forceinline__ void load(Raw4<T> (&r)[NC], const T* img, int iy) const {
        const T* rowp = img + (long long)min(max(iy, 0), H - 1) * rstep;
#pragma unroll
        for (int k = 0; k < NC; ++k) raw_load(r[k], rowp + off[k]);
    }
    template <bool AFF, bool EDGE, int INSIDE>
    __device__ __forceinline__ void act(const Raw4<T> (&r)[NC], int iy, const InAffine& aff, f32x2_t (&a)[NC][2]) const {
        if (iy < 0 || iy >= H) {
#pragma unroll
            for (int k = 0; k < NC; ++k) { a[k][0] = (f32x2_t){0.f, 0.f}; a[k][1] = (f32x2_t){0.f, 0.f}; }
            return;
        }
#pragma unroll
        for (int k = 0; k < NC; ++k) {
            float f[4];
            raw_unpack(r[k], f);
            if constexpr (AFF) aff.apply(f);
            if (EDGE && k != INSIDE) zero_unless(ok[k], f);
            store_pairs(a[k], f);
        }
    }
};

__device__ __forceinline__ void add_stats(f32x2_t y01, f32x2_t y23, f32x2_t& s01, f32x2_t& s23, f32x2_t& q01, f32x2_t& q23) {
    s01 += y01; s23 += y23;
    q01 += y01 * y01; q23 += y23 * y23;
}
template <typename T> struct BnReduce {
    f32x2_t sc01, sc23, sh01, sh23, is01, is23, nm01, nm23;
    float lo, hi;
    __device__ __forceinline__ void load(const float* scale, const float* shift, const float* mean, const float* invstd, int act, int cc) {
        const float4 s4 = *reinterpret_cast<const float4*>(scale + cc), h4 = *reinterpret_cast<const float4*>(shift + cc);
        const float4 m4 = *reinterpret_cast<const float4*>(mean + cc), i4 = *reinterpret_cast<const float4*>(invstd + cc);
        sc01 = (f32x2_t){s4.x, s4.y}; sc23 = (f32x2_t){s4.z, s4.w};
        sh01 = (f32x2_t){h4.x, h4.y}; sh23 = (f32x2_t){h4.z, h4.w};
        is01 = (f32x2_t){i4.x, i4.y}; is23 = (f32x2_t){i4.z, i4.w};
        nm01 = (f32x2_t){-m4.x * i4.x, -m4.y * i4.y}; nm23 = (f32x2_t){-m4.z * i4.z, -m4.w * i4.w};
        lo = (act != MPN_ACT_NONE) ? 0.f : -INFINITY;
        hi = (act == MPN_ACT_RELU6) ? 6.f : INFINITY;
    }
    __device__ __forceinline__ void add(f32x2_t d01, f32x2_t d23, const Raw4<T>& xr, f32x2_t& s01, f32x2_t& s23, f32x2_t& q01, f32x2_t& q23) const {
        f32x2_t x01, x23;
        raw_unpack2(xr, x01, x23);
        const f32x2_t p01 = x01 * sc01 + sh01, p23 = x23 * sc23 + sh23;
        d01 = round_storage<T>(d01); d23 = round_storage<T>(d23);
        f32x2_t g01, g23;
        g01.x = (p01.x > lo && p01.x < hi) ? d01.x : 0.f; g01.y = (p01.y > lo && p01.y < hi) ? d01.y : 0.f;
        g23.x = (p23.x > lo && p23.x < hi) ? d23.x : 0.f; g23.y = (p23.y > lo && p23.y < hi) ? d23.y : 0.f;
        s01 += g01; s23 += g23;
        q01 += g01 * (x01 * is01 + nm01); q23 += g23 * (x23 * is23 + nm23);
    }
};
template <typename T> struct DyApply {
    f32x2_t sc01, sc23, cb01, cb23, cc01, cc23;
    bool pair67;
    __device__ __forceinline__ void load(const float* scale, const float* mean, const float* invstd, const float* k1, const float* k2, int cc) {
        const float4 s4 = *reinterpret_cast<const float4*>(scale + cc), m4 = *reinterpret_cast<const float4*>(mean + cc);
        const float4 i4 = *reinterpret_cast<const float4*>(invstd + cc);
        const float4 a4 = *reinterpret_cast<const float4*>(k1 + cc), b4 = *reinterpret_cast<const float4*>(k2 + cc);
        const float ss[4] = {s4.x, s4.y, s4.z, s4.w}, mm[4] = {m4.x, m4.y, m4.z, m4.w}, ii[4] = {i4.x, i4.y, i4.z, i4.w};
        const float aa[4] = {a4.x, a4.y, a4.z, a4.w}, bb[4] = {b4.x, b4.y, b4.z, b4.w};
        float cb[4], cc_[4];
#pragma unroll
        for (int j = 0; j < 4; ++j) {
            cb[j] = -ss[j] * bb[j] * ii[j];
            cc_[j] = -ss[j] * (aa[j] - mm[j] * ii[j] * bb[j]);
        }
        sc01 = (f32x2_t){ss[0], ss[1]}; sc23 = (f32x2_t){ss[2], ss[3]};
        cb01 = (f32x2_t){cb[0], cb[1]}; cb23 = (f32x2_t){cb[2], cb[3]};
        cc01 = (f32x2_t){cc_[0], cc_[1]}; cc23 = (f32x2_t){cc_[2], cc_[3]};
        pair67 = (cc & 4) != 0;
    }
    static __device__ __forceinline__ f32x2_t unfused(f32x2_t sc, f32x2_t g, f32x2_t cb, f32x2_t y, f32x2_t cc) {
#pragma clang fp contract(off)
        const f32x2_t t = cb * y, u = sc * g;
        return (cc + t) + u;
    }
    __device__ __forceinline__ void apply(float (&f)[4], const Raw4<T>& yr, unsigned elem) const {
        f32x2_t y01, y23;
        raw_unpack2(yr, y01, y23);
        const f32x2_t g01 = {f[0], f[1]}, g23 = {f[2], f[3]};
        const f32x2_t o01 = __builtin_elementwise_fma(sc01, g01, __builtin_elementwise_fma(cb01, y01, cc01));
        f32x2_t o23 = __builtin_elementwise_fma(sc23, g23, __builtin_elementwise_fma(cb23, y23, cc23));
        const f32x2_t v23 = unfused(sc23, g23, cb23, y23, cc23);
        if (pair67 && ((elem >> 11) & 3u) != 2u) o23 = v23;
        const f32x2_t r01 = round_storage<T>(o01), r23 = round_storage<T>(o23);
        f[0] = r01.x; f[1] = r01.y; f[2] = r23.x; f[3] = r23.y;
    }
};

__device__ __forceinline__ void write_sums_row(float* red, const SwLane& l, int ncg, int cols, int C, float* part, f32x2_t s01, f32x2_t s23,
                                               f32x2_t q01, f32x2_t q23) {
    float st[8] = {s01.x, s01.y, s23.x, s23.y, q01.x, q01.y, q23.x, q23.y};
#pragma unroll
    for (int j = 0; j < 8; ++j) red[threadIdx.x * 8 + j] = l.ok ? st[j] : 0.f;
    __syncthreads();
    if ((int)threadIdx.x < ncg && (l.cgb * ncg + (int)threadIdx.x) * 4 < C) {
        float acc8[8] = {0.f, 0.f, 0.f, 0.f, 0.f, 0.f, 0.f, 0.f};
        for (int cidx = 0; cidx < cols; ++cidx)
#pragma unroll
            for (int j = 0; j < 8; ++j) acc8[j] += red[(cidx * ncg + threadIdx.x) * 8 + j];
        float* dst = part + (long long)l.unit * 2 * C + (l.cgb * ncg + threadIdx.x) * 4;
#pragma unroll
        for (int j = 0; j < 4; ++j) { dst[j] = acc8[j]; dst[C + j] = acc8[4 + j]; }
    }
}
__device__ __forceinline__ void write_taps_row(float* red, const SwLane& l, int ncg, int cols, int C, float* part, const f32x2_t (&a01)[9],
                                               const f32x2_t (&a23)[9]) {
#pragma unroll
    for (int t = 0; t < 9; ++t) {
        float4 v = make_float4(a01[t].x, a01[t].y, a23[t].x, a23[t].y);
        if (!l.ok) v = make_float4(0.f, 0.f, 0.f, 0.f);
        *reinterpret_cast<float4*>(&red[(t * kThreads + threadIdx.x) * 4]) = v;
    }
    __syncthreads();
    const int nch = ncg * 4;
    float* dst = part + (long long)l.unit * 9 * C + l.cgb * nch;
    for (int o = threadIdx.x; o < 9 * nch; o += kThreads) {
        const int t = o / nch, cj = o - t * nch;
        if (l.cgb * nch + cj < C) {
            float sum = 0.f;
            for (int cidx = 0; cidx < cols; ++cidx) sum += red[(t * kThreads + cidx * ncg) * 4 + cj];
            dst[t * C + cj] = sum;
        }
    }
}

template <typename T> __device__ __forceinline__ void quad_load(Raw4<T> (&r)[4], const T* q, long long xrow, int C) {
    raw_load(r[0], q); raw_load(r[1], q + C); raw_load(r[2], q + xrow); raw_load(r[3], q + xrow + C);
}
template <typename T> __device__ __forceinline__ void add_raw4(const Raw4<T>& r, f32x2_t& o01, f32x2_t& o23) {
    float f[4];
    raw_unpack(r, f);
    o01 += (f32x2_t){f[0], f[1]};
    o23 += (f32x2_t){f[2], f[3]};
}

}
```

### multiposenet_amd/csrc/stem.hip

```cpp
#include "common.h"

namespace {

constexpr int kThreads = 256;
constexpr int kTile = 16;
constexpr int kIn = 2 * kTile + 1;
constexpr int kMaxC0 = 64;
constexpr int kFwdTW = 2 * kTile;

template <typename T, bool U8>
__device__ __forceinline__ void stage_patch(const void* images, float* patch, int img, int oy0, int ox0, int H, int W,
                                            int pad_t, int pad_l) {
    const int iy0 = oy0 * 2 - pad_t, ix0 = ox0 * 2 - pad_l;
    constexpr int NEL = kIn * kIn * 3;
    constexpr int PER = (NEL + kThreads - 1) / kThreads;
    float v[PER];
#pragma unroll
    for (int k = 0; k < PER; ++k) {
        const int i = threadIdx.x + k * kThreads;
        const int ch = i % 3;
        const int px = (i / 3) % kIn;
        const int py = i / (3 * kIn);
        const int iy = iy0 + py, ix = ix0 + px;
        float raw = 0.5f;
        if (i < NEL && iy >= 0 && iy < H && ix >= 0 && ix < W) {
            const long long off = (((long long)img * H + iy) * W + ix) * 3 + ch;
            raw = U8 ? (float)reinterpret_cast<const unsigned char*>(images)[off] * (1.0f / 255.0f)
                     : reinterpret_cast<const float*>(images)[off];
        }
        v[k] = raw;
    }
#pragma unroll
    for (int k = 0; k < PER; ++k) {
        const int i = threadIdx.x + k * kThreads;
        if (i < NEL) patch[i] = 2.0f * v[k] - 1.0f;
    }
}

template <typename T>
__device__ __forceinline__ void stem_copy_out(unsigned char* otile, int orow, T* __restrict__ y, int img, int ty, int tx, int OH,
                                              int OW, int C0, float* __restrict__ stats_part) {
    constexpr int VE = Vec16<T>::N;
    const int ppr = C0 * (int)sizeof(T) / 16;
    float ssum[VE], ssq[VE];
#pragma unroll
    for (int j = 0; j < VE; ++j) { ssum[j] = 0.f; ssq[j] = 0.f; }
    for (int i = threadIdx.x; i < kTile * kFwdTW * ppr; i += kThreads) {
        const int pxl = i / ppr, piece = i - pxl * ppr;
        const int r = pxl / kFwdTW, cx = pxl - r * kFwdTW;
        const int yy = ty * kTile + r, xx = tx * kFwdTW + cx;
        if (yy < OH && xx < OW) {
            Vec16<T> ov;
            *reinterpret_cast<uint4*>(&ov.raw) = *reinterpret_cast<const uint4*>(otile + pxl * orow + piece * 16);
            *reinterpret_cast<uint4*>(reinterpret_cast<unsigned char*>(y + (((long long)img * OH + yy) * OW + xx) * C0) + piece * 16) =
                *reinterpret_cast<const uint4*>(&ov.raw);
            if (stats_part != nullptr) {
                float f[VE];
                ov.unpack(f);
#pragma unroll
                for (int j = 0; j < VE; ++j) { ssum[j] += f[j]; ssq[j] += f[j] * f[j]; }
            }
        }
    }
    if (stats_part != nullptr) {
        __syncthreads();
        float* red = reinterpret_cast<float*>(otile);
#pragma unroll
        for (int j = 0; j < VE; ++j) { red[threadIdx.x * 2 * VE + j] = ssum[j]; red[threadIdx.x * 2 * VE + VE + j] = ssq[j]; }
        __syncthreads();
        if ((int)threadIdx.x < 2 * C0) {
            const int which = (int)threadIdx.x / C0, c = (int)threadIdx.x - which * C0;
            const int piece = c / VE, j = c - piece * VE;
            float acc = 0.f;
            for (int t = piece; t < kThreads; t += ppr) acc += red[t * 2 * VE + which * VE + j];
            stats_part[((long long)blockIdx.x * 2 + which) * C0 + c] = acc;
        }
    }
}

typedef float f32x2_t __attribute__((ext_vector_type(2)));

template <typename T, bool U8>
__global__ __launch_bounds__(kThreads) void stem_fwd_kernel(const void* __restrict__ images, const float* __restrict__ w,
// ... 230 lines not shown
            pmask |= (ok ? 1u : 0u) << k;
        }
#pragma unroll
        for (int k = 0; k < DPER; ++k) {
            if (k < ndv) {
                const int i = threadIdx.x + k * kThreads;
                const int vq = i % vpp, px = i / vpp;
                const int oy = oy0 + px / kTile, ox = ox0 + px % kTile;
                const bool ok = oy < OH && ox < OW;
                dvv[k].load(dy + (ok ? (((long long)img * OH + oy) * OW + ox) * C0 + vq * VE : 0));
                dmask |= (ok ? 1u : 0u) << k;
            }
        }
    };
    auto commit_tile = [&]() {
#pragma unroll
        for (int k = 0; k < PER; ++k) {
            const int i = threadIdx.x + k * kThreads;
            if (i < NEL) patch[i] = ((pmask >> k) & 1u) ? 2.0f * pv[k] - 1.0f : 0.0f;
        }
#pragma unroll
        for (int k = 0; k < DPER; ++k) {
            if (k < ndv) {
                const int i = threadIdx.x + k * kThreads;
                const int vq = i % vpp, px = i / vpp;
                float f[VE];
                dvv[k].unpack(f);
                const bool ok = (dmask >> k) & 1u;
#pragma unroll
                for (int j = 0; j < VE; j += 4)
                    *reinterpret_cast<float4*>(g + px * C0 + vq * VE + j) =
                        ok ? make_float4(f[j], f[j + 1], f[j + 2], f[j + 3]) : make_float4(0.f, 0.f, 0.f, 0.f);
            }
        }
    };

    int t = blockIdx.x;
    if (t < ntiles) {
        load_tile(t);
        commit_tile();
    }
    for (; t < ntiles; t += gridDim.x) {
        const bool more = t + (int)gridDim.x < ntiles;
        if (more) load_tile(t + gridDim.x);
        __syncthreads();
        if (active) {
            for (int px = ph; px < kTile * kTile; px += nphase) {
                const int ly = px / kTile, lx = px - ly * kTile;
                const float* pp = patch + ((2 * ly + ky) * kIn + 2 * lx + kx) * 3;
                const float a0 = pp[0], a1 = pp[1], a2 = pp[2];
                const float4 g0 = *reinterpret_cast<const float4*>(g + px * C0 + cq * 8);
                const float4 g1 = *reinterpret_cast<const float4*>(g + px * C0 + cq * 8 + 4);
                const f32x2_t gv[4] = {(f32x2_t){g0.x, g0.y}, (f32x2_t){g0.z, g0.w}, (f32x2_t){g1.x, g1.y}, (f32x2_t){g1.z, g1.w}};
                const f32x2_t b0 = (f32x2_t){a0, a0}, b1 = (f32x2_t){a1, a1}, b2 = (f32x2_t){a2, a2};
#pragma unroll
                for (int j = 0; j < 4; ++j) {
                    acc[0][j] += b0 * gv[j];
                    acc[1][j] += b1 * gv[j];
                    acc[2][j] += b2 * gv[j];
                }
            }
        }
        __syncthreads();
        if (more) commit_tile();
    }
    __syncthreads();
    if (active) {
#pragma unroll
        for (int a = 0; a < 3; ++a)
#pragma unroll
            for (int j = 0; j < 4; ++j) {
                g[ph * nout + (pos * 3 + a) * C0 + cq * 8 + 2 * j] = acc[a][j].x;
                g[ph * nout + (pos * 3 + a) * C0 + cq * 8 + 2 * j + 1] = acc[a][j].y;
            }
    }
    __syncthreads();
    for (int o = threadIdx.x; o < nout; o += kThreads) {
        float s = 0.f;
        for (int q = 0; q < nphase; ++q) s += g[q * nout + o];
        part[(long long)blockIdx.x * nout + o] = s;
    }
}

template <bool U8, int MB>
__global__ __launch_bounds__(kThreads) void stem_wgrad_mfma_kernel(const void* __restrict__ images, const bf16_t* __restrict__ dy,
                                                                   float* __restrict__ part, int N, int H, int W, int OH, int OW,
                                                                   int pad_t, int pad_l, int tiles_x, int tiles_y) {
    typedef H16<bf16_t> HT;
    typedef HT::x8 x8;
    typedef HT::x4 x4;
    typedef HT::acc_t acc_t;
    constexpr int C0 = 16 * MB;
    constexpr int DRS = C0 * 2 + 16;
    extern __shared__ __attribute__((aligned(16))) unsigned char stem_smem[];
    float* patch = reinterpret_cast<float*>(stem_smem);
    unsigned char* dimg = stem_smem + kPR * kPS * sizeof(float);
    const int ntiles = N * tiles_y * tiles_x;
    const int lane = threadIdx.x & 63, wv = threadIdx.x >> 6;
    const int n = lane & 15, kg = lane >> 4, q = n >> 2, pq = n & 3;
    constexpr int VPP = C0 / 8;
    constexpr int DV = kTile * kFwdTW * VPP / kThreads;
    float pv[kPR];
    uint4 dv[DV];
    unsigned long long pmask = 0ull;
    unsigned dmask = 0u;
    const int p_pc = threadIdx.x < kPC ? threadIdx.x : 0;
    auto load_tile = [&](int t) __attribute__((always_inline)) {
        const int tx = t % tiles_x;
        const int t2 = t / tiles_x;
        const int ty = t2 % tiles_y;
        const int img = t2 / tiles_y;
        const int iy0 = ty * kTile * 2 - pad_t, ix0 = tx * kFwdTW * 2 - pad_l;
        pmask = 0ull;
        dmask = 0u;
        int tid = threadIdx.x;
        asm volatile("" : "+v"(tid));
        {
            const int ix = ix0 + p_pc / 3;
            const bool col_ok = tid < kPC && ix >= 0 && ix < W;
            const long long base = ((long long)img * H * W + ix0) * 3 + p_pc;
#pragma unroll
            for (int py = 0; py < kPR; ++py) {
                const int iy = iy0 + py;
                const bool ok = col_ok && iy >= 0 && iy < H;
                const long long off = ok ? base + (long long)iy * W * 3 : 0;
                pv[py] = U8 ? (float)reinterpret_cast<const unsigned char*>(images)[off] * (1.0f / 255.0f)
                            : reinterpret_cast<const float*>(images)[off];
                pmask |= (unsigned long long)(ok ? 1u : 0u) << py;
            }
        }
#pragma unroll
        for (int k = 0; k < DV; ++k) {
            const int i = tid + k * kThreads;
            const int vq = i % VPP, px = i / VPP;
            const int oy = ty * kTile + px / kFwdTW, ox = tx * kFwdTW + px % kFwdTW;
            const bool ok = oy < OH && ox < OW;
            dv[k] = *reinterpret_cast<const uint4*>(dy + (ok ? (((long long)img * OH + oy) * OW + ox) * C0 + vq * 8 : 0));
            dmask |= (ok ? 1u : 0u) << k;
        }
    };
    auto commit_tile = [&]() __attribute__((always_inline)) {
        int tid = threadIdx.x;
        asm volatile("" : "+v"(tid));
        if (tid < kPC) {
#pragma unroll
            for (int py = 0; py < kPR; ++py)
                patch[py * kPS + p_pc] = ((pmask >> py) & 1ull) ? 2.0f * pv[py] - 1.0f : 0.0f;
        }
#pragma unroll
        for (int k = 0; k < DV; ++k) {
            const int i = tid + k * kThreads;
            const int vq = i % VPP, px = i / VPP;
            *reinterpret_cast<uint4*>(dimg + px * DRS + vq * 16) = ((dmask >> k) & 1u) ? dv[k] : make_uint4(0u, 0u, 0u, 0u);
        }
    };
    int kbase[2];
    bool kval[2];
#pragma unroll
    for (int nb = 0; nb < 2; ++nb) {
        const int k = nb * 16 + n;
        kval[nb] = k < 27;
        kbase[nb] = kval[nb] ? (k / 9) * kPS + (k % 9) : 0;
    }
    acc_t acc[MB][2];
#pragma unroll
    for (int mb = 0; mb < MB; ++mb)
#pragma unroll
        for (int nb = 0; nb < 2; ++nb) acc[mb][nb] = (acc_t){0.f, 0.f, 0.f, 0.f};

    int t = blockIdx.x;
    if (t < ntiles) {
        load_tile(t);
        commit_tile();
    }
    for (; t < ntiles; t += gridDim.x) {
        const bool more = t + (int)gridDim.x < ntiles;
        if (more) load_tile(t + gridDim.x);
        __syncthreads();
#pragma unroll 1
        for (int sr = 0; sr < 4; ++sr) {
            const int r = wv * 4 + sr;
            x8 a[MB];
#pragma unroll
            for (int mb = 0; mb < MB; ++mb) {
                const unsigned char* src = dimg + (r * kFwdTW + 8 * kg + q) * DRS + (mb * 16 + 4 * pq) * 2;
                const x4 lo4 = HT::tr_read(src);
                const x4 hi4 = HT::tr_read(src + 4 * DRS);
                a[mb] = __builtin_shufflevector(lo4, hi4, 0, 1, 2, 3, 4, 5, 6, 7);
            }
#pragma unroll
            for (int nb = 0; nb < 2; ++nb) {
                const float* src = patch + (2 * r) * kPS + 6 * (8 * kg) + kbase[nb];
                x8 b_hi, b_lo;
#pragma unroll
                for (int i = 0; i < 8; ++i) {
                    const float raw = src[6 * i];
                    const float f = kval[nb] ? raw : 0.0f;
                    const bf16_t h = (bf16_t)f;
                    b_hi[i] = h;
                    b_lo[i] = (bf16_t)(f - (float)h);
                }
#pragma unroll
                for (int mb = 0; mb < MB; ++mb) {
                    acc[mb][nb] = HT::mfma(a[mb], b_lo, acc[mb][nb]);
                    acc[mb][nb] = HT::mfma(a[mb], b_hi, acc[mb][nb]);
                }
            }
        }
        __syncthreads();
        if (more) commit_tile();
    }
    __syncthreads();
    float* red = reinterpret_cast<float*>(stem_smem);
#pragma unroll
    for (int mb = 0; mb < MB; ++mb)
#pragma unroll
        for (int nb = 0; nb < 2; ++nb)
            *reinterpret_cast<float4*>(red + ((wv * (MB * 2) + mb * 2 + nb) * 64 + lane) * 4) =
                make_float4(acc[mb][nb][0], acc[mb][nb][1], acc[mb][nb][2], acc[mb][nb][3]);
    __syncthreads();
    for (int o = threadIdx.x; o < 27 * C0; o += kThreads) {
        const int k = o / C0, co = o - k * C0;
        const int nb = k >> 4, nn = k & 15, mb = co >> 4, m = co & 15;
        const int ln = (m >> 2) * 16 + nn, e = m & 3;
        float sacc = 0.f;
#pragma unroll
        for (int w4 = 0; w4 < 4; ++w4) sacc += red[((w4 * (MB * 2) + mb * 2 + nb) * 64 + ln) * 4 + e];
        part[(long long)blockIdx.x * (27 * C0) + o] = sacc;
    }
}

template <bool U8, int MB>
int launch_stem_wgrad_mfma(int grid, hipStream_t st, const void* images, const void* dy, float* part, int N, int H, int W, int OH,
                           int OW, int pt, int pl, int tiles_x, int tiles_y) {
    constexpr int sm = kPR * kPS * (int)sizeof(float) + kTile * kFwdTW * (16 * MB * 2 + 16);
    static mpn_attr_mask_t attr_mask{0};
    MPN_HIP(mpn_ensure_dynamic_lds((const void*)stem_wgrad_mfma_kernel<U8, MB>, sm, &attr_mask));
    stem_wgrad_mfma_kernel<U8, MB><<<grid, kThreads, sm, st>>>(images, (const bf16_t*)dy, part, N, H, W, OH, OW, pt, pl, tiles_x, tiles_y);
    return MPN_OK;
}

void same_pad(int size, int* out, int* pad_before) {
    *out = (size + 1) / 2;
    int total = (*out - 1) * 2 + 3 - size;
    if (total < 0) total = 0;
    *pad_before = total / 2;
}

int check(int N, int H, int W, int C0, int dtype) {
    MPN_REQUIRE(dtype == MPN_F32 || dtype == MPN_BF16, MPN_ERR_BAD_DTYPE, "stem: dtype %d", dtype);
    const int ve = dtype == MPN_F32 ? 4 : 8;
    MPN_REQUIRE(N > 0 && H > 0 && W > 0, MPN_ERR_BAD_SHAPE, "stem: bad shape");
    MPN_REQUIRE(C0 > 0 && C0 <= kMaxC0 && C0 % ve == 0, MPN_ERR_BAD_SHAPE, "stem: C0 (%d) must be <= %d and a multiple of %d",
                C0, kMaxC0, ve);
    return MPN_OK;
}

}

extern "C" int mpn_stem_conv_fwd_num_parts(int N, int H, int W, int C0, int dtype) {
    if (check(N, H, W, C0, dtype)) return 0;
    const int ppr = C0 * (dtype == MPN_F32 ? 4 : 2) / 16;
    if (ppr <= 0 || kThreads % ppr != 0 || 2 * C0 > kThreads) return 0;
    int OH, OW, pt, pl;
    same_pad(H, &OH, &pt);
    same_pad(W, &OW, &pl);
    return N * ((OH + kTile - 1) / kTile) * ((OW + kFwdTW - 1) / kFwdTW);
}

extern "C" int mpn_stem_conv_fwd(const void* images, int images_u8, const float* w, void* y, int N, int H, int W, int C0,
                                 int dtype, mpn_stream_t stream) {
    return mpn_stem_conv_fwd_stats(images, images_u8, w, y, N, H, W, C0, dtype, nullptr, stream);
}

extern "C" int mpn_stem_conv_fwd_stats(const void* images, int images_u8, const float* w, void* y, int N, int H, int W, int C0,
                                       int dtype, float* stats_part, mpn_stream_t stream) {
    if (int rc = check(N, H, W, C0, dtype)) return rc;
    MPN_REQUIRE(images && w && y, MPN_ERR_BAD_ARG, "stem_fwd: null pointer");
    MPN_REQUIRE(stats_part == nullptr || mpn_stem_conv_fwd_num_parts(N, H, W, C0, dtype) > 0, MPN_ERR_BAD_SHAPE,
                "stem_fwd: fused statistics not available for C0 = %d (mpn_stem_conv_fwd_num_parts == 0)", C0);
    int OH, OW, pt, pl;
    same_pad(H, &OH, &pt);
    same_pad(W, &OW, &pl);
    const int tiles_y = (OH + kTile - 1) / kTile, tiles_x = (OW + kFwdTW - 1) / kFwdTW;
    const int grid = N * tiles_y * tiles_x;
    hipStream_t st = (hipStream_t)stream;
    if (dtype == MPN_BF16 && C0 % 16 == 0) {
        const int otile_bytes = 2 * kThreads * (C0 * 2 + 16), patch_bytes = kPR * kPS * (int)sizeof(float);
        const int sm = otile_bytes > patch_bytes ? otile_bytes : patch_bytes;
#define MPN_STEM_MFMA(MB)                                                                                                       \
    do {                                                                                                                        \
        if (images_u8) stem_fwd_mfma_kernel<true, MB><<<grid, kThreads, sm, st>>>(images, w, (bf16_t*)y, N, H, W, OH, OW, pt, pl, tiles_x, tiles_y, stats_part); \
        else stem_fwd_mfma_kernel<false, MB><<<grid, kThreads, sm, st>>>(images, w, (bf16_t*)y, N, H, W, OH, OW, pt, pl, tiles_x, tiles_y, stats_part); \
    } while (0)
        if (sm <= 64 * 1024) {
            switch (C0 / 16) {
                case 1: MPN_STEM_MFMA(1); break;
                case 2: MPN_STEM_MFMA(2); break;
                case 3: MPN_STEM_MFMA(3); break;
                default: MPN_STEM_MFMA(4); break;
            }
#undef MPN_STEM_MFMA
            MPN_LAUNCH_CHECK();
            return MPN_OK;
        }
    }
    MPN_DISPATCH_DTYPE(dtype, {
        const int sm = 2 * kThreads * (C0 * (int)sizeof(T) + 16);
        if (images_u8) {
            if (sm > 48 * 1024)
                MPN_HIP(hipFuncSetAttribute((const void*)stem_fwd_kernel<T, true>, hipFuncAttributeMaxDynamicSharedMemorySize, sm));
            stem_fwd_kernel<T, true><<<grid, kThreads, sm, st>>>(images, w, (T*)y, N, H, W, C0, OH, OW, pt, pl, tiles_x, tiles_y, stats_part);
        } else {
            if (sm > 48 * 1024)
                MPN_HIP(hipFuncSetAttribute((const void*)stem_fwd_kernel<T, false>, hipFuncAttributeMaxDynamicSharedMemorySize, sm));
            stem_fwd_kernel<T, false><<<grid, kThreads, sm, st>>>(images, w, (T*)y, N, H, W, C0, OH, OW, pt, pl, tiles_x, tiles_y, stats_part);
        }
    });
    MPN_LAUNCH_CHECK();
    return MPN_OK;
}

extern "C" int mpn_stem_conv_wgrad_num_parts(int N, int H, int W) {
    const int ntiles = N * (((H + 1) / 2 + kTile - 1) / kTile) * (((W + 1) / 2 + kTile - 1) / kTile);
    return ntiles < 512 ? ntiles : 512;
}

extern "C" int mpn_stem_conv_bwd_weight(const void* images, int images_u8, const void* dy, float* part, int N, int H, int W,
                                        int C0, int dtype, mpn_stream_t stream) {
    if (int rc = check(N, H, W, C0, dtype)) return rc;
    MPN_REQUIRE(images && dy && part, MPN_ERR_BAD_ARG, "stem_wgrad: null pointer");
    int OH, OW, pt, pl;
    same_pad(H, &OH, &pt);
    same_pad(W, &OW, &pl);
    const int tiles_y = (OH + kTile - 1) / kTile, tiles_x = (OW + kTile - 1) / kTile;
    const int grid = mpn_stem_conv_wgrad_num_parts(N, H, W);
    hipStream_t st = (hipStream_t)stream;
    MPN_REQUIRE(C0 % 8 == 0, MPN_ERR_BAD_SHAPE, "stem_wgrad: C0 must be a multiple of 8");
    if (dtype == MPN_BF16 && C0 % 16 == 0) {
        const int tx32 = (OW + kFwdTW - 1) / kFwdTW;
        int rc;
#define MPN_STEM_WG(MB)                                                                                                         \
    rc = images_u8 ? launch_stem_wgrad_mfma<true, MB>(grid, st, images, dy, part, N, H, W, OH, OW, pt, pl, tx32, tiles_y)       \
                   : launch_stem_wgrad_mfma<false, MB>(grid, st, images, dy, part, N, H, W, OH, OW, pt, pl, tx32, tiles_y)
        switch (C0 / 16) {
            case 1: MPN_STEM_WG(1); break;
            case 2: MPN_STEM_WG(2); break;
            case 3: MPN_STEM_WG(3); break;
            default: MPN_STEM_WG(4); break;
        }
#undef MPN_STEM_WG
        if (rc) return rc;
        MPN_LAUNCH_CHECK();
        return MPN_OK;
    }
    const size_t sm = (size_t)(kIn * kIn * 3 + 1 + kTile * kTile * C0) * sizeof(float);
    MPN_REQUIRE(sm <= 64 * 1024, MPN_ERR_BAD_SHAPE, "stem_wgrad: C0 too large");
    MPN_DISPATCH_DTYPE(dtype, {
        if (images_u8)
            stem_wgrad_kernel<T, true><<<grid, kThreads, sm, st>>>(images, (const T*)dy, part, N, H, W, C0, OH, OW, pt, pl, tiles_x, tiles_y);
        else
            stem_wgrad_kernel<T, false><<<grid, kThreads, sm, st>>>(images, (const T*)dy, part, N, H, W, C0, OH, OW, pt, pl, tiles_x, tiles_y);
    });
    MPN_LAUNCH_CHECK();
    return MPN_OK;
}
```

### multiposenet_amd/net.py

```python
import math
import os
from collections import OrderedDict

import numpy as np
import torch

from . import _lib, ops
from ._lib import ACT_NONE, ACT_RELU, ACT_RELU6
from .model_state import ModelState, _Arena, is_trainable, resolve_device

NUM_KEYPOINTS = 17
DOWNSAMPLE = 4
DIVISOR = 128
DEPTH = 128
STRIDES_AND_FILTERS = [(1, 64), (2, 128), (1, 128), (2, 256), (1, 256), (2, 512), (1, 512), (1, 512),
                       (1, 512), (1, 512), (1, 512), (2, 1024), (1, 1024)]
FEATURE_BLOCKS = {3: "c2", 5: "c3", 11: "c4", 13: "c5"}


def depth(x, depth_multiplier):
    return max(int(x * depth_multiplier), 8)


def variable_shapes(depth_multiplier=1.0):
    s = OrderedDict()

    def bn(prefix, c):
        for n in ("gamma", "beta", "moving_mean", "moving_variance"):
            s[f"{prefix}/{n}"] = (c,)

    c = depth(32, depth_multiplier)
    s["MobilenetV1/Conv2d_0/weights"] = (3, 3, 3, c)
    bn("MobilenetV1/Conv2d_0/BatchNorm", c)
    for i, (_, f) in enumerate(STRIDES_AND_FILTERS, 1):
        s[f"MobilenetV1/Conv2d_{i}_depthwise/depthwise_weights"] = (3, 3, c, 1)
        bn(f"MobilenetV1/Conv2d_{i}_depthwise/BatchNorm", c)
        f = depth(f, depth_multiplier)
        s[f"MobilenetV1/Conv2d_{i}_pointwise/weights"] = (1, 1, c, f)
        bn(f"MobilenetV1/Conv2d_{i}_pointwise/BatchNorm", f)
        c = f
    feat = {2: depth(128, depth_multiplier), 3: depth(256, depth_multiplier),
            4: depth(512, depth_multiplier), 5: depth(1024, depth_multiplier)}
    s["keypoint_fpn/lateral5/kernel"] = (1, 1, feat[5], DEPTH)
    s["keypoint_fpn/p5/kernel"] = (3, 3, DEPTH, DEPTH)
    for i in (4, 3, 2):
        s[f"keypoint_fpn/lateral{i}/kernel"] = (1, 1, feat[i], DEPTH)
        s[f"keypoint_fpn/p{i}/kernel"] = (3, 3, DEPTH, DEPTH)
    for l in (2, 3, 4, 5):
        bn(f"p{l}_batch_norm", DEPTH)
    for l in (2, 3, 4, 5):
        s[f"phi_subnet_{l}/conv1/kernel"] = (3, 3, DEPTH, DEPTH)
        bn(f"phi_subnet_{l}/bn1", DEPTH)
        s[f"phi_subnet_{l}/conv2/kernel"] = (3, 3, DEPTH, DEPTH)
        bn(f"phi_subnet_{l}/bn2", DEPTH)
    s["final_conv3x3/kernel"] = (3, 3, 4 * DEPTH, 64)
    bn("final_bn", 64)
    s["heatmaps/kernel"] = (1, 1, 64, NUM_KEYPOINTS + 1)
    s["heatmaps/bias"] = (NUM_KEYPOINTS + 1,)
    return s


def internal_shapes(depth_multiplier=1.0):
    ref = variable_shapes(depth_multiplier)
    c0 = depth(32, depth_multiplier)
    c0p = (c0 + 15) // 16 * 16
    if c0p == c0:
        return ref, {}
    shapes, pads = OrderedDict(), {}
    for name, shape in ref.items():
        axis = None
        if name.startswith("MobilenetV1/Conv2d_0/") or name.startswith("MobilenetV1/Conv2d_1_depthwise/BatchNorm/"):
            axis = len(shape) - 1
        elif name in ("MobilenetV1/Conv2d_1_depthwise/depthwise_weights", "MobilenetV1/Conv2d_1_pointwise/weights"):
            axis = 2
        if axis is not None:
            assert shape[axis] == c0
            pads[name] = (axis, c0)
            shape = tuple(c0p if i == axis else d for i, d in enumerate(shape))
        shapes[name] = shape
    return shapes, pads


def initial_values(seed=0, depth_multiplier=1.0):
    rs = np.random.RandomState(seed)
    out = OrderedDict()
    for name, shape in variable_shapes(depth_multiplier).items():
        if name.endswith("/gamma") or name.endswith("moving_variance"):
            v = np.ones(shape)
        elif name.endswith("/beta") or name.endswith("moving_mean"):
            v = np.zeros(shape)
        elif name == "heatmaps/bias":
            v = np.array([-math.log(99.0)] * NUM_KEYPOINTS + [0.0])
        elif name == "heatmaps/kernel":
            v = rs.randn(*shape) * 1e-4
        else:
            fan_in = shape[0] * shape[1] * (shape[2] if not name.endswith("depthwise_weights") else 1)
            v = rs.randn(*shape) * math.sqrt(1.0 / fan_in) * 1.2
        out[name] = v.astype(np.float32)
    return out


DP_DEEP_FROM_BLOCK = 7


def backbone_deep_begin_of(arena, first_block=DP_DEEP_FROM_BLOCK):
    return arena.offsets[f"MobilenetV1/Conv2d_{first_block}_depthwise/depthwise_weights"][0]


def backbone_grad_end_of(arena):
    end = 0
    for k, (o, n, _) in arena.offsets.items():
        if k.startswith("MobilenetV1/"):
            end = max(end, o + (n + 3) // 4 * 4)
    return end


@ops._lib.device_guarded("_init", "load_state_dict", "repack_weights", "prepare_inference", "forward", "predict",
                         "backbone_forward", "subnet_forward", "compute_losses", "backward", "add_weight_decay_gradients",
                         "add_weight_decay_loss", "optimizer_step")
class KeypointNet(ModelState):
    def __init__(self, values=None, depth_multiplier=1.0, dtype=torch.bfloat16, device="cuda:0", seed=0):
        if dtype not in (torch.float32, torch.bfloat16):
            raise ValueError("dtype must be torch.float32 or torch.bfloat16")
        self.dtype, self.device, self.dm = dtype, resolve_device(device), depth_multiplier
        self._init(values, depth_multiplier, dtype, seed)

    def _init(self, values, depth_multiplier, dtype, seed):
        shapes, pads = internal_shapes(depth_multiplier)
        for n, s in shapes.items():
            if n.endswith("gamma") and (s[0] % 16 != 0):
                raise ValueError(f"depth_multiplier={depth_multiplier}: {n} has {s[0]} channels; every layer behind the stem "
                                 f"must be a multiple of 16 channels wide (depth multipliers that are multiples of 0.25)")
        self._init_state(shapes, pads=pads)
        self.load_state_dict(values if values is not None else initial_values(seed, depth_multiplier))
        self._build_layers()
        self._bufs = {}

    def _build_layers(self):
        self.stem_w = self.vars["MobilenetV1/Conv2d_0/weights"]
        self.stem_dw = self.grads["MobilenetV1/Conv2d_0/weights"]
        self.stem_bn = self._bn("MobilenetV1/Conv2d_0/BatchNorm", ACT_RELU6)
        self.blocks = []
        for i, (stride, _) in enumerate(STRIDES_AND_FILTERS, 1):
            d, p = f"MobilenetV1/Conv2d_{i}_depthwise", f"MobilenetV1/Conv2d_{i}_pointwise"
            self.blocks.append(dict(
                i=i, stride=stride,
                dw_w=self.vars[d + "/depthwise_weights"], dw_dw=self.grads[d + "/depthwise_weights"],
                dw_bn=self._bn(d + "/BatchNorm", ACT_RELU6),
                pw=self._conv(p + "/weights"), pw_bn=self._bn(p + "/BatchNorm", ACT_RELU6)))
        self.lateral = {l: self._conv(f"keypoint_fpn/lateral{l}/kernel") for l in (5, 4, 3, 2)}
        self.pconv = {l: self._conv(f"keypoint_fpn/p{l}/kernel") for l in (5, 4, 3, 2)}
        self.p_bn = {l: self._bn(f"p{l}_batch_norm", ACT_RELU) for l in (2, 3, 4, 5)}
        self.phi = {}
        for l in (2, 3, 4, 5):
            s = f"phi_subnet_{l}"
            self.phi[l] = dict(conv1=self._conv(s + "/conv1/kernel"), bn1=self._bn(s + "/bn1", ACT_RELU),
                               conv2=self._conv(s + "/conv2/kernel"), bn2=self._bn(s + "/bn2", ACT_RELU))
        self.final_conv = self._conv("final_conv3x3/kernel")
        self.final_bn = self._bn("final_bn", ACT_RELU)
        self.concat_scale = torch.ones(4 * DEPTH, dtype=torch.float32, device=self.device)
        self.concat_shift = torch.zeros(4 * DEPTH, dtype=torch.float32, device=self.device)
        self.phi[2]["bn2"].scale = self.concat_scale[:DEPTH]
        self.phi[2]["bn2"].shift = self.concat_shift[:DEPTH]
        self.concat_affine = ops.Affine(self.concat_scale, self.concat_shift, ACT_RELU)
        self.heat_w, self.heat_b = self.vars["heatmaps/kernel"], self.vars["heatmaps/bias"]
        ok, nk, _ = self._train_arena.offsets["heatmaps/kernel"]
        ob, nb, _ = self._train_arena.offsets["heatmaps/bias"]
        assert ob == ok + nk, "heatmaps/kernel and heatmaps/bias must be adjacent in the arena"
        self._head_grad = self.grad[ok:ob + nb]
        self.fuse_dw_bn = True
        self.fuse_dw_apply = True
        self.fuse_conv_bn = True
        self._l2 = None
        self._wd = None
        self.cache_inference_affine = False
        self._infer_clean = False
        self.fuse_stem_stats = True
        self._build_pack_table()
        self.all_bn = [self.stem_bn] + [b[k] for b in self.blocks for k in ("dw_bn", "pw_bn")] + \
            [self.p_bn[l] for l in (2, 3, 4, 5)] + [self.phi[l][k] for l in (2, 3, 4, 5) for k in ("bn1", "bn2")] + [self.final_bn]

    def _build_pack_table(self):
        import ctypes
        lib = ops._lib.lib()
        nb = lib.mpn_conv_pack_desc_bytes()
        jobs = [(c, t) for c in self.convs for t in (0, 1)]
        host = (ctypes.c_ubyte * (nb * len(jobs)))()
        begin = 0
        dc = ops._lib.dtype_code(self.dtype)
        for j, (c, t) in enumerate(jobs):
            out = c.packed.bwd if t else c.packed.fwd
            blocks = lib.mpn_conv_pack_desc_fill(ctypes.byref(host, j * nb), ops.ptr(c.w), c.cin, c.cout, c.ksize, t, dc,
                                                 ops.ptr(out), begin)
            assert blocks > 0
            begin += blocks
        self._pack_table = torch.frombuffer(bytearray(host), dtype=torch.uint8).to(self.device)
        self._pack_jobs, self._pack_blocks = len(jobs), begin

    def repack_weights(self):
        if ops.LAUNCH_JOBS_ALONE:
            for c in self.convs:
                c.packed.repack()
            return
        ops.call("mpn_conv_pack_weights_batched", ops.ptr(self._pack_table), self._pack_jobs, self._pack_blocks,
                 ops._lib.dtype_code(self.dtype), ops.stream_ptr())

    def _buffers(self, N, H, W, head=True):
        key = (N, H, W) if head else (N, H, W, "backbone")
        b = self._bufs.get(key)
        if b is not None:
            return b
        if H % DIVISOR or W % DIVISOR:
            raise ValueError(f"image height and width must be multiples of {DIVISOR} (got {H}x{W})")
        dt, dev = self.dtype, self.device

        def act(h, w, c):
            return torch.empty((N, h, w, c), dtype=dt, device=dev)

        b = {"shape": (N, H, W)}
        h, w = H // 2, W // 2
        c = self.stem_w.shape[3]
        b["stem"] = act(h, w, c)
        b["dw"], b["pw"], b["hw"] = [], [], [(h, w)]
        for blk in self.blocks:
            if blk["stride"] == 2:
                h, w = h // 2, w // 2
            b["dw"].append(act(h, w, c))
            c = blk["pw"].cout
            b["pw"].append(act(h, w, c))
            b["hw"].append((h, w))
        if not head:
            nbn0 = ops._lib.lib().mpn_bn_stats_num_parts
            b["stat_part"] = torch.empty(nbn0(N * (H // 2) * (W // 2)) * 2 * b["stem"].shape[3], dtype=torch.float32, device=dev)
            self._bufs[key] = b
            return b
        lv = {l: (H >> l, W >> l) for l in (2, 3, 4, 5)}
        b["lv"] = lv
        b["x"] = {l: act(*lv[l], DEPTH) for l in lv}
        b["p"] = {l: act(*lv[l], DEPTH) for l in lv}
        b["y1"] = {l: act(*lv[l], DEPTH) for l in lv}
        b["concat"] = act(*lv[2], 4 * DEPTH)
        b["y2"] = {l: act(*lv[l], DEPTH) for l in lv if l != 2}
        b["y2"][2] = b["concat"][..., :DEPTH]
        b["final"] = act(*lv[2], 64)
        b["logits"] = torch.empty((N, lv[2][0], lv[2][1], NUM_KEYPOINTS + 1), dtype=torch.float32, device=dev)
        nbn = ops._lib.lib().mpn_bn_stats_num_parts

        def rows(t):
            return t.numel() // t.shape[3]

        stat_floats = nbn(rows(b["stem"])) * 2 * b["stem"].shape[3]
        for i, blk in enumerate(self.blocks):
            hh, ww = b["hw"][i]
            cdw, cpw = b["dw"][i].shape[3], blk["pw"].cout
            stat_floats = max(stat_floats, ops.dwconv_num_parts(N, hh, ww, cdw, blk["stride"], dt) * 2 * cdw,
                              nbn(rows(b["dw"][i])) * 2 * cdw,
                              ops.conv_num_parts(N, *b["hw"][i + 1], 1) * 2 * cpw, nbn(rows(b["pw"][i])) * 2 * cpw,
                              ops.dwconv_bwd_data_bn_num_parts(N, hh, ww, cdw, blk["stride"], dt) * 2 * cdw,
                              ops.dwconv_wgrad_num_parts(N, hh, ww, cdw, blk["stride"], dt) * 2 * cdw,
                              ops.conv_wgrad_num_parts(N, *b["hw"][i + 1], cdw, cpw, 1, dt) * 2 * cdw)
        for l in lv:
            stat_floats = max(stat_floats, ops.conv_num_parts(N, *lv[l], 3) * 2 * DEPTH, nbn(N * lv[l][0] * lv[l][1]) * 2 * DEPTH)
        b["stat_part"] = torch.empty(stat_floats, dtype=torch.float32, device=dev)
        b["stat_lv"] = {l: torch.empty(max(ops.conv_num_parts(N, *lv[l], 3), nbn(N * lv[l][0] * lv[l][1])) * 2 * DEPTH,
                                       dtype=torch.float32, device=dev) for l in lv}
        b["fin"] = None
        b["loss_part"] = torch.empty(ops._lib.lib().mpn_keypoint_loss_num_parts(N, *lv[2]) * 8, dtype=torch.float32, device=dev)
        b["losses"] = torch.zeros(8, dtype=torch.float32, device=dev)
        self._bufs[key] = b
        return b

    def _grad_buffers(self, b):
        if "g" in b:
            return b["g"]
        N, H, W = b["shape"]
        dt, dev = self.dtype, self.device
        g = {}
        g["dlogits"] = torch.empty_like(b["logits"])
        g["daux"] = {l: torch.empty((N, *b["lv"][l]), dtype=torch.float32, device=dev) for l in b["lv"]}
        g["final"] = torch.empty_like(b["final"])
        g["concat"] = torch.empty_like(b["concat"])
        for k in ("y1", "p", "x"):
            g[k] = {l: torch.empty_like(b[k][l]) for l in b["lv"]}
        g["y2"] = {l: torch.empty_like(b["y2"][l]) for l in b["lv"] if l != 2}
        g["y2"][2] = g["concat"][..., :DEPTH]
        g["c"] = {}
        for i, name in FEATURE_BLOCKS.items():
            g["c"][name] = torch.empty_like(b["pw"][i - 1])
        g["pw"] = [torch.empty_like(t) for t in b["pw"]]
        g["dw"] = [torch.empty_like(t) for t in b["dw"]]
        g["stem"] = torch.empty_like(b["stem"])
        lib, dc = ops._lib.lib(), ops._lib.dtype_code(dt)
        sites = []
        grouped_np = {}
        for group in self._wgrad_groups():
            hws = [self._conv_hw(b, c) for c in group]
            for c, np_ in zip(group, ops.conv_wgrad_grouped_num_parts(N, hws, group[0].cin, group[0].cout, group[0].ksize, dt)):
                grouped_np[id(c.dw)] = np_
        for c in self.convs:
            hw = self._conv_hw(b, c)
            np_ = grouped_np.get(id(c.dw))
            if np_ is None:
                np_ = ops.conv_wgrad_num_parts(N, hw[0], hw[1], c.cin, c.cout, c.ksize, dt)
            sites.append((id(c.dw), np_, c.w.numel(), c.dw))
        for i, blk in enumerate(self.blocks):
            hh, ww = b["hw"][i]
            cc = b["dw"][i].shape[3]
            sites.append((id(blk["dw_dw"]), lib.mpn_dwconv_wgrad_num_parts(N, hh, ww, cc, blk["stride"], dc), 9 * cc, blk["dw_dw"]))
        sites.append((id(self.stem_dw), lib.mpn_stem_conv_wgrad_num_parts(N, H, W), self.stem_w.numel(), self.stem_dw))
        sites.append((id(self._head_grad), lib.mpn_heatmap_head_bwd_num_parts(N * b["lv"][2][0] * b["lv"][2][1]),
                      self._head_grad.numel(), self._head_grad))
        total = sum(((np_ * n + 3) // 4) * 4 for _, np_, n, _ in sites)
        slab = torch.empty(total, dtype=torch.float32, device=dev)
        deep_keys = {id(blk[k]) if k == "dw_dw" else id(blk[k].dw) for blk in self.blocks if blk["i"] >= DP_DEEP_FROM_BLOCK
                     for k in ("pw", "dw_dw")}
        shallow_keys = {id(blk[k]) if k == "dw_dw" else id(blk[k].dw) for blk in self.blocks if blk["i"] < DP_DEEP_FROM_BLOCK
                        for k in ("pw", "dw_dw")} | {id(self.stem_dw)}
        g["slab"], jobs, off = {}, ([], [], []), 0
        for key, np_, n, out in sites:
            view = slab[off:off + np_ * n]
            g["slab"][key] = view
            jobs[1 if key in deep_keys else (2 if key in shallow_keys else 0)].append((view, np_, n, out.view(-1)))
            off += ((np_ * n + 3) // 4) * 4
        g["reducer"] = tuple(ops.SlabReducer(j, dev) for j in jobs)
        b["g"] = g
        return g

    def _wgrad_groups(self):
        LV = (2, 3, 4, 5)
        return [[self.phi[l]["conv2"] for l in LV], [self.phi[l]["conv1"] for l in LV], [self.pconv[l] for l in LV]]

    def _conv_hw(self, b, c):
        n = c.name
        if n.startswith("MobilenetV1"):
            i = int(n.split("Conv2d_")[1].split("_")[0])
            return b["hw"][i]
        if n.startswith("keypoint_fpn") or n.startswith("phi_subnet"):
            l = int(n.split("/")[0][-1]) if n.startswith("phi") else int(n.split("/")[1].replace("lateral", "").replace("p", ""))
            return b["lv"][l]
        return b["lv"][2]

    def _finish_bn(self, bn, b, nparts, count, training):
        if training:
            ops.bn_finalize(bn, b["stat_part"], nparts, count, training=True)

    def prepare_inference(self):
        if self.cache_inference_affine and self._infer_clean:
            return
        for bn in self.all_bn:
            ops.bn_inference_affine(bn)
        self._infer_clean = True

    def backbone_forward(self, images, is_training, b=None):
        N, H, W, _ = images.shape
        b = b or self._buffers(N, H, W)
        if not is_training:
            self.prepare_inference()
        else:
            self.mark_variables_changed()
        sp = b["stat_part"]
        c0 = self.stem_w.shape[3]
        stem_rows = ops.stem_conv_fwd_num_parts(N, H, W, c0, self.dtype) if (is_training and self.fuse_stem_stats) else 0
        if stem_rows * 2 * c0 > sp.numel():
            stem_rows = 0
        stem = ops.stem_conv_fwd(images, self.stem_w, c0, self.dtype, out=b["stem"], stats_part=sp if stem_rows > 0 else None)
        if is_training:
            cnt = stem.numel() // stem.shape[3]
            if stem_rows > 0:
                ops.bn_finalize(self.stem_bn, sp, stem_rows, cnt)
            else:
                _, nparts = ops.bn_stats(stem, sp)
                ops.bn_finalize(self.stem_bn, sp, nparts, cnt)
        x, aff = stem, self.stem_bn.affine
        feats = {}
# ... 112 lines not shown
        if part in (None, 0):
            self._backward_head(b, g, feats, sp, slab)
            g["reducer"][0].run()
        for ph in (1, 2):
            if part in (None, ph):
                self._backward_backbone(b, g, images, sp, slab, ph)
                g["reducer"][ph].run()

    def _backward_head(self, b, g, feats, sp, slab):
        if self._fused_conv_bn() and ops.heatmap_head_bwd_bn_supported(b["final"].shape[3], self.dtype):
            rows = ops.heatmap_head_bwd(b["final"], g["dlogits"], self.heat_w, self.final_bn.affine, g["final"], self._head_grad,
                                        slab[id(self._head_grad)], reduce=False, bn_part=sp)
            ops.bn_backward(self.final_bn, g["final"], b["final"], sp, reduced_parts=rows, raw=True)
        else:
            ops.heatmap_head_bwd(b["final"], g["dlogits"], self.heat_w, self.final_bn.affine, g["final"], self._head_grad,
                                 slab[id(self._head_grad)], reduce=False)
            ops.bn_backward(self.final_bn, g["final"], b["final"], sp)
        ops.conv_bwd_weight(b["concat"], g["final"], 3, self.concat_affine, self.final_conv.dw, slab[id(self.final_conv.dw)], reduce=False)
        ops.conv_fwd(g["final"], self.final_conv.packed.bwd, 4 * DEPTH, 3, None, out=g["concat"])
        if b["fin"] is None:
            b["fin"] = self._finalize_tables(b)
        fin, spl = b["fin"], b["stat_lv"]
        LV = (2, 3, 4, 5)
        sps = [spl[l] for l in LV]
        bn2s, bn1s, pbns = [self.phi[l]["bn2"] for l in LV], [self.phi[l]["bn1"] for l in LV], [self.p_bn[l] for l in LV]
        gy2, gy1, gp = [g["y2"][l] for l in LV], [g["y1"][l] for l in LV], [g["p"][l] for l in LV]
        by2, by1, bp = [b["y2"][l] for l in LV], [b["y1"][l] for l in LV], [b["p"][l] for l in LV]
        for l in (3, 4, 5):
            ops.bilinear_up_bwd(g["concat"], 2 ** (l - 2), (l - 2) * DEPTH, DEPTH, out=g["y2"][l])
        ops.bn_bwd_reduce_grouped(bn2s, gy2, by2, sps)
        fin["dbn2"].run()
        none4 = [None] * 4
        fused = self._fused_conv_bn()
        ops.bn_bwd_apply_grouped(bn2s, gy2, by2)
        ops.conv_bwd_weight_grouped(by1, gy2, 3, [self.phi[l]["bn1"].affine for l in LV], [slab[id(self.phi[l]["conv2"].dw)] for l in LV])
        if fused:
            ops.conv_bwd_data_bn_grouped(gy2, [self.phi[l]["conv2"].packed.bwd for l in LV], DEPTH, bn1s, by1, gy1, sps)
        else:
            ops.conv_fwd_grouped([g["y2"][l] for l in LV], [self.phi[l]["conv2"].packed.bwd for l in LV], DEPTH, 3, none4,
                                 [g["y1"][l] for l in LV], none4)
            ops.bn_bwd_reduce_grouped(bn1s, gy1, by1, sps)
        fin["dbn1"].run()
        ops.bn_bwd_apply_grouped(bn1s, gy1, by1)
        ops.conv_bwd_weight_grouped(bp, gy1, 3, [self.p_bn[l].affine for l in LV], [slab[id(self.phi[l]["conv1"].dw)] for l in LV])
        if fused:
            ops.conv_bwd_data_bn_grouped(gy1, [self.phi[l]["conv1"].packed.bwd for l in LV], DEPTH, pbns, bp, gp, sps)
        else:
            ops.conv_fwd_grouped([g["y1"][l] for l in LV], [self.phi[l]["conv1"].packed.bwd for l in LV], DEPTH, 3, none4,
                                 [g["p"][l] for l in LV], none4)
            ops.bn_bwd_reduce_grouped(pbns, gp, bp, sps)
        fin["dp"].run()
        ops.bn_bwd_apply_grouped(pbns, gp, bp, [g["daux"][l] for l in LV])
        ops.conv_bwd_weight_grouped([b["x"][l] for l in LV], gp, 3, none4, [slab[id(self.pconv[l].dw)] for l in LV])
        ops.conv_fwd_grouped(gp, [self.pconv[l].packed.bwd for l in LV], DEPTH, 3, none4, [g["x"][l] for l in LV], none4)
        g["c5_reduced"] = 0
        for l in (2, 3, 4, 5):
            if l > 2:
                ops.sumpool2x2(g["x"][l - 1], g["x"][l], accumulate=True)
            raw, aff = feats[f"c{l}"]
            ops.conv_bwd_weight(raw, g["x"][l], 1, aff, self.lateral[l].dw, slab[id(self.lateral[l].dw)], reduce=False)
            if l == 5 and self.fuse_conv_bn and ops.conv_bwd_data_bn_supported(DEPTH, raw.shape[3], 1, self.dtype):
                g["c5_reduced"] = ops.conv_bwd_data_bn(g["x"][l], self.lateral[l].packed.bwd, raw.shape[3], 1, self.blocks[-1]["pw_bn"], raw,
                                                       g["c"][f"c{l}"], sp)
            else:
                ops.conv_fwd(g["x"][l], self.lateral[l].packed.bwd, raw.shape[3], 1, None, out=g["c"][f"c{l}"])

    def _backward_backbone(self, b, g, images, sp, slab, phase):
        first, last = DP_DEEP_FROM_BLOCK - 1, len(self.blocks) - 1
        if phase == 1:
            dA, reduced, lateral_added = g["c"]["c5"], g.get("c5_reduced", 0), False
            rng = range(last, first - 1, -1)
        else:
            dA, reduced, lateral_added = g["bb_chain"]
            rng = range(first - 1, -1, -1)
        for i in rng:
            feature = FEATURE_BLOCKS.get(self.blocks[i]["i"])
            if feature in ("c2", "c3", "c4") and not lateral_added:
                ops.add_inplace(dA, g["c"][feature])
            dY, applied = self._backward_pointwise(b, g, sp, slab, i, dA, reduced, raw=i == last, fold=self._dw_folds_apply(b, g, i))
            dA, reduced, lateral_added = self._backward_depthwise(b, g, sp, slab, i, dY, apply=not applied)
        if phase == 1:
            g["bb_chain"] = (dA, reduced, lateral_added)
            return
        ops.bn_backward(self.stem_bn, g["stem"], b["stem"], sp, reduced_parts=reduced)
        ops.stem_conv_bwd_weight(images, g["stem"], self.stem_dw, slab[id(self.stem_dw)], reduce=False)

    def _dw_lateral(self, g, i):
        return g["c"][FEATURE_BLOCKS[self.blocks[i - 1]["i"]]] if i > 0 and self.blocks[i - 1]["i"] in FEATURE_BLOCKS else None

    def _dw_walks_fused(self, b, g, i):
        s, (N, _, _, C) = self.blocks[i]["stride"], b["dw"][i].shape
        return (self.fuse_dw_bn and (s == 2 or self._dw_lateral(g, i) is None)
                and ops.dwconv_bwd_fused_supported(N, *b["hw"][i], C, s, self.dtype))

    def _dw_folds_apply(self, b, g, i):
        s, (N, _, _, C) = self.blocks[i]["stride"], b["dw"][i].shape
        return (self.fuse_dw_apply and self._dw_walks_fused(b, g, i)
                and ops.dwconv_bwd_fused_apply_supported(N, *b["hw"][i], C, s, self.dtype))

    def _backward_pointwise(self, b, g, sp, slab, i, dA, reduced, raw, fold=False):
        blk = self.blocks[i]
        pw, x, dY = blk["pw"], b["dw"][i], g["dw"][i]
        fused = self.fuse_conv_bn and ops.conv1x1_bwd_fused_supported(pw.cin, pw.cout, self.dtype) and pw.cin <= 64
        apply = fused and ops.conv1x1_bwd_fused_apply_supported(pw.cin, pw.cout, self.dtype)
        ops.bn_backward(blk["pw_bn"], dA, b["pw"][i], sp, reduced_parts=reduced, raw=raw, apply=not apply)
        rows = 0
        with _lib.tagged("pointwise"):
            if fused:
                rows = ops.conv1x1_bwd_fused(x, dA, pw.w, blk["dw_bn"], dY, slab[id(pw.dw)], sp,
                                             apply_bn=blk["pw_bn"] if apply else None, y_raw=b["pw"][i] if apply else None)
            else:
                ops.conv_bwd_weight(x, dA, 1, blk["dw_bn"].affine, pw.dw, slab[id(pw.dw)], reduce=False)
                if self.fuse_conv_bn and ops.conv_bwd_data_bn_supported(pw.cout, pw.cin, 1, self.dtype):
                    rows = ops.conv_bwd_data_bn(dA, pw.packed.bwd, pw.cin, 1, blk["dw_bn"], x, dY, sp)
                else:
                    ops.conv_fwd(dA, pw.packed.bwd, pw.cin, 1, None, out=dY)
        applied = not (fold and rows > 0)
        ops.bn_backward(blk["dw_bn"], dY, x, sp, reduced_parts=rows, raw=True, apply=applied)
        return dY, applied

    def _backward_depthwise(self, b, g, sp, slab, i, dY, apply=False):
        blk = self.blocks[i]
        x, bn, dA = (b["pw"][i - 1], self.blocks[i - 1]["pw_bn"], g["pw"][i - 1]) if i > 0 else (b["stem"], self.stem_bn, g["stem"])
        N, hw, C, s = dA.shape[0], b["hw"][i], dA.shape[3], blk["stride"]
        lateral = self._dw_lateral(g, i)
        if self._dw_walks_fused(b, g, i):
            _, reduced = ops.dwconv_bwd_fused(x, dY, blk["dw_w"], bn, None, out=dA, wpart=slab[id(blk["dw_dw"])], bn_part=sp,
                                              reduce=False, stride=s, addend=lateral, apply_bn=blk["dw_bn"] if apply else None,
                                              y_raw=b["dw"][i] if apply else None)
            return dA, reduced, lateral is not None
        assert not apply, "only the fused depthwise walk applies the batch-norm backward on load"
        ops.dwconv_bwd_weight(x, dY, s, bn.affine, blk["dw_dw"], slab[id(blk["dw_dw"])], reduce=False)
        late = lateral is not None and not ops.dwconv_bwd_data_add_supported(N, *hw, C, s, self.dtype)
        addend = None if late else lateral
        if self.fuse_dw_bn and not late and ops.dwconv_bwd_data_bn_num_parts(N, *hw, C, s, self.dtype) > 0:
            _, reduced = ops.dwconv_bwd_data(dY, blk["dw_w"], hw, s, out=dA, bn=bn, x_bn=x, part=sp, addend=addend)
            return dA, reduced, addend is not None
        ops.dwconv_bwd_data(dY, blk["dw_w"], hw, s, out=dA, addend=addend)
        return dA, 0, addend is not None

    def add_weight_decay_gradients(self, weight_decay):
        if self._wd is None:
            ks = [k for k in self.vars if ("weights" in k or "kernel" in k) and "depthwise_weights" not in k]
            self._wd = ops.AxpyBatch([self.vars[k] for k in ks], [self.grads[k] for k in ks])
        self._wd.run(weight_decay)

    def add_weight_decay_loss(self, weight_decay):
        total = self._last[0]["losses"][6:7]
        if self._l2 is None:
            self._l2 = ops.L2LossBatch([w for k, w in self.vars.items()
                                        if ("weights" in k or "kernel" in k) and "depthwise_weights" not in k])
        self._l2.run(weight_decay, total)

    def optimizer_step(self, initial_learning_rate, num_steps, grad_scale=1.0):
        ops.adam_prepare(self.global_step, self.hyper, initial_learning_rate, num_steps)
        ops.adam_step(self.theta, self.grad, self.adam_m, self.adam_v, self.hyper, grad_scale=grad_scale)
        self.mark_variables_changed()
        self.repack_weights()
```

### multiposenet_amd/ops.py

```python
import ctypes
from collections import namedtuple

import torch

from . import _lib
from ._lib import ACT_NONE, ACT_RELU, ACT_RELU6, call, ptr, stream_ptr

BN_MOMENTUM = 0.95
BN_EPSILON = 1e-3

LAUNCH_JOBS_ALONE = False

Affine = namedtuple("Affine", ["scale", "shift", "act"])


def _f32(n, dev):
    return torch.empty(n, dtype=torch.float32, device=dev)


def _check_nhwc(x, name="x"):
    if x.dim() != 4 or not x.is_contiguous():
        raise ValueError(f"{name} must be a contiguous NHWC tensor, got shape {tuple(x.shape)}")
    if x.dtype not in (torch.float32, torch.bfloat16):
        raise ValueError(f"{name}: unsupported dtype {x.dtype}")
# ... 83 lines not shown


def conv_fwd_grouped(xs, packeds, cout, ksize, affines, outs, stats_parts):
    n = len(xs)
    if LAUNCH_JOBS_ALONE and n > 1:
        _each_job_alone(conv_fwd_grouped, n, xs, packeds, cout, ksize, affines, outs, stats_parts)
        return outs
    N, _, _, cin = xs[0].shape
    act = next((int(a.act) for a in reversed(affines) if a is not None), ACT_NONE)
    call("mpn_conv_fwd_grouped", n, _arr(xs), _arr(packeds), _arr(outs), N, _arr([x.shape[1] for x in xs], ctypes.c_int),
         _arr([x.shape[2] for x in xs], ctypes.c_int), cin, cout, _arr([_slice_stride(x, cin) for x in xs], ctypes.c_int),
         _arr([_slice_stride(o, cout) for o in outs], ctypes.c_int), ksize, _lib.dtype_code(xs[0].dtype),
         _arr([a.scale if a else None for a in affines]), _arr([a.shift if a else None for a in affines]), act, _arr(stats_parts), stream_ptr())
    return outs


def conv_bwd_data_bn_supported(k, c, ksize, dtype):
    return bool(_lib.lib().mpn_conv_bwd_data_bn_supported(int(k), int(c), int(ksize), _lib.dtype_code(dtype)))


def conv_bwd_data_bn(dy, packed_t, c, ksize, bn, x_bn, out, part):
    N, H, W, k = dy.shape
    call("mpn_conv_bwd_data_bn", ptr(dy), ptr(packed_t), ptr(out), N, H, W, k, int(c), _slice_stride(dy, k), _slice_stride(out, c), int(ksize),
         _lib.dtype_code(dy.dtype), ptr(x_bn), _slice_stride(x_bn, c), ptr(bn.scale), ptr(bn.shift), int(bn.act), ptr(part), stream_ptr())
    return conv_stats_rows(N, H, W, k, c, ksize, dy.dtype)


def conv_bwd_data_bn_grouped(dys, packeds_t, c, bns, xs_bn, outs, parts):
    n = len(dys)
    if LAUNCH_JOBS_ALONE and n > 1:
        return [rows[0] for rows in _each_job_alone(conv_bwd_data_bn_grouped, n, dys, packeds_t, c, bns, xs_bn, outs, parts)]
    N, _, _, k = dys[0].shape
    call("mpn_conv_bwd_data_bn_grouped", n, _arr(dys), _arr(packeds_t), _arr(outs), N, _arr([t.shape[1] for t in dys], ctypes.c_int),
         _arr([t.shape[2] for t in dys], ctypes.c_int), k, int(c), _arr([_slice_stride(t, k) for t in dys], ctypes.c_int),
         _arr([_slice_stride(o, c) for o in outs], ctypes.c_int), _lib.dtype_code(dys[0].dtype), _arr(xs_bn),
         _arr([_slice_stride(x, c) for x in xs_bn], ctypes.c_int), _arr([b.scale for b in bns]), _arr([b.shift for b in bns]),
         int(bns[0].act), _arr(parts), stream_ptr())
    return [conv_stats_rows(N, t.shape[1], t.shape[2], k, c, 3, t.dtype) for t in dys]


def conv1x1_bwd_fused_supported(cin, cout, dtype):
    return _lib.lib().mpn_conv1x1_bwd_fused_supported(int(cin), int(cout), _lib.dtype_code(dtype)) == 1


def conv1x1_bwd_fused_apply_supported(cin, cout, dtype):
    return _lib.lib().mpn_conv1x1_bwd_fused_apply_supported(int(cin), int(cout), _lib.dtype_code(dtype)) == 1


def conv1x1_bwd_fused(x, dy, w, bn, out, wpart, bn_part, apply_bn=None, y_raw=None):
    N, H, W, cin = x.shape
    cout = dy.shape[3]
    rows = conv_wgrad_num_parts(N, H, W, cin, cout, 1, x.dtype)
    if wpart.numel() < rows * cin * cout or (bn_part is not None and bn_part.numel() < rows * 2 * cin):
        raise ValueError("conv1x1_bwd_fused: partial slab too small")
    if apply_bn is not None:
        a = apply_bn
        call("mpn_conv1x1_bwd_fused_apply", ptr(x), ptr(dy), ptr(y_raw), ptr(w), ptr(out), ptr(wpart), ptr(bn_part), N, H, W, cin, cout,
             _slice_stride(x, cin), _slice_stride(dy, cout), _slice_stride(y_raw, cout), _slice_stride(out, cin), _lib.dtype_code(x.dtype),
             ptr(bn.scale), ptr(bn.shift), int(bn.act), ptr(a.scale), ptr(a.shift), ptr(a.mean), ptr(a.invstd), ptr(a.k1), ptr(a.k2),
             int(a.act), stream_ptr())
        return rows
    call("mpn_conv1x1_bwd_fused", ptr(x), ptr(dy), ptr(w), ptr(out), ptr(wpart), ptr(bn_part), N, H, W, cin, cout, _slice_stride(x, cin),
         _slice_stride(dy, cout), _slice_stride(out, cin), _lib.dtype_code(x.dtype), ptr(bn.scale), ptr(bn.shift), int(bn.act), stream_ptr())
    return rows


def conv_wgrad_num_parts(N, H, W, cin, cout, ksize, dtype):
    return _lib.lib().mpn_conv_wgrad_num_parts(N, H, W, cin, cout, ksize, _lib.dtype_code(dtype))


def conv_bwd_weight(x, dy, ksize, affine, dw_out, part=None, reduce=True):
    N, H, W, cin = x.shape
    cout = dy.shape[3]
    nparts = conv_wgrad_num_parts(N, H, W, cin, cout, ksize, x.dtype)
    n = ksize * ksize * cin * cout
    if part is None:
        part = _f32(nparts * n, x.device)
    sc, sh, act = _aff(affine)
    call("mpn_conv_bwd_weight", ptr(x), ptr(dy), ptr(part), N, H, W, cin, cout, _slice_stride(x, cin), _slice_stride(dy, cout),
         ksize, _lib.dtype_code(x.dtype), sc, sh, act, stream_ptr())
    if reduce:
        call("mpn_reduce_partials", ptr(part), nparts, n, ptr(dw_out), 0, 1.0, stream_ptr())
    return dw_out


class SlabReducer:

    def __init__(self, jobs, device):
        self._alone = [SlabReducer([j], device) for j in jobs] if LAUNCH_JOBS_ALONE and len(jobs) > 1 else None
        lib = _lib.lib()
        nb = lib.mpn_reduce_desc_bytes()
        host = (ctypes.c_ubyte * (nb * len(jobs)))()
        begin = 0
        for j, (part, nparts, n, out) in enumerate(jobs):
            blocks = lib.mpn_reduce_desc_fill(ctypes.byref(host, j * nb), ptr(part), int(nparts), int(n), ptr(out), 1.0, begin)
            if blocks <= 0:
                raise ValueError("bad slab reduction job")
            begin += blocks
        self.table = torch.frombuffer(bytearray(host), dtype=torch.uint8).to(device)
        self.njobs, self.blocks = len(jobs), begin
        self._keep = jobs

    def run(self):
        if self._alone is not None:
            for r in self._alone:
                r.run()
            return
        call("mpn_reduce_partials_batched", ptr(self.table), self.njobs, self.blocks, stream_ptr())


def conv_wgrad_grouped_num_parts(N, hws, cin, cout, ksize, dtype):
    n = len(hws)
    if LAUNCH_JOBS_ALONE and n > 1:
        return [nps[0] for nps in _each_job_alone(conv_wgrad_grouped_num_parts, n, N, list(hws), cin, cout, ksize, dtype)]
    out = (ctypes.c_int * n)()
    call("mpn_conv_wgrad_grouped_num_parts", n, N, _arr([h for h, _ in hws], ctypes.c_int), _arr([w for _, w in hws], ctypes.c_int),
         cin, cout, ksize, _lib.dtype_code(dtype), out)
    return list(out)


def conv_bwd_weight_grouped(xs, dys, ksize, affines, parts):
    n = len(xs)
    if LAUNCH_JOBS_ALONE and n > 1:
        _each_job_alone(conv_bwd_weight_grouped, n, xs, dys, ksize, affines, parts)
        return
    N, cin, cout = xs[0].shape[0], xs[0].shape[3], dys[0].shape[3]
    acts = {int(a.act) if a is not None else ACT_NONE for a in affines}
    if len(acts) != 1:
        raise ValueError("grouped jobs must share the activation")
    call("mpn_conv_bwd_weight_grouped", n, _arr(xs), _arr(dys), _arr(parts), N, _arr([t.shape[1] for t in xs], ctypes.c_int),
         _arr([t.shape[2] for t in xs], ctypes.c_int), cin, cout, _arr([_slice_stride(t, cin) for t in xs], ctypes.c_int),
         _arr([_slice_stride(t, cout) for t in dys], ctypes.c_int), ksize, _lib.dtype_code(xs[0].dtype),
         _arr([a.scale if a else None for a in affines]), _arr([a.shift if a else None for a in affines]), acts.pop(), stream_ptr())


class BNState:

    def __init__(self, gamma, beta, moving_mean, moving_var, act):
        C = gamma.numel()
        dev = gamma.device
        self.C, self.act = C, act
        self.gamma, self.beta, self.moving_mean, self.moving_var = gamma, beta, moving_mean, moving_var
        self.scale, self.shift = _f32(C, dev), _f32(C, dev)
        self.mean, self.invstd = _f32(C, dev), _f32(C, dev)
        self.k1, self.k2 = _f32(C, dev), _f32(C, dev)
        self.dgamma = self.dbeta = None

    @property
    def affine(self):
        return Affine(self.scale, self.shift, self.act)

    def channel_slice(self, lo, hi):
        s = object.__new__(BNState)
        s.C, s.act = hi - lo, self.act
        for k in ("gamma", "beta", "moving_mean", "moving_var", "scale", "shift", "mean", "invstd", "k1", "k2"):
            setattr(s, k, getattr(self, k)[lo:hi])
        s.dgamma = self.dgamma[lo:hi] if self.dgamma is not None else None
        s.dbeta = self.dbeta[lo:hi] if self.dbeta is not None else None
        return s


def bn_stats(x, part=None):
    M, C = x.numel() // x.shape[-1], x.shape[-1]
    nparts = _lib.lib().mpn_bn_stats_num_parts(M)
    if part is None:
        part = _f32(nparts * 2 * C, x.device)
# ... 227 lines not shown
    return _lib.lib().mpn_dwconv_bwd_fused_supported(N, H, W, C, stride, _lib.dtype_code(dtype)) == 1


def dwconv_bwd_fused_apply_supported(N, H, W, C, stride, dtype):
    return _lib.lib().mpn_dwconv_bwd_fused_apply_supported(N, H, W, C, stride, _lib.dtype_code(dtype)) == 1


def dwconv_bwd_fused(x, dy, w, bn, dw_out, out=None, wpart=None, bn_part=None, reduce=True, reduce_bn=True, stride=1, addend=None,
                     apply_bn=None, y_raw=None):
    N, H, W, C = x.shape
    dc = _lib.dtype_code(x.dtype)
    if not dwconv_bwd_fused_supported(N, H, W, C, stride, x.dtype):
        raise ValueError("dwconv_bwd_fused: shape not supported")
    if apply_bn is not None:
        if not dwconv_bwd_fused_apply_supported(N, H, W, C, stride, x.dtype):
            raise ValueError("dwconv_bwd_fused: apply_bn not supported for this shape or dtype")
        if y_raw is None or y_raw.shape != dy.shape or y_raw.dtype != dy.dtype or not y_raw.is_contiguous():
            raise ValueError("dwconv_bwd_fused: apply_bn needs y_raw of dy's shape and dtype")
    if addend is not None and (stride != 2 or addend.shape != x.shape or addend.dtype != x.dtype or not addend.is_contiguous()):
        raise ValueError("dwconv_bwd_fused: addend needs stride 2 and the result's shape and dtype")
    if out is None:
        out = torch.empty_like(x)
    rows = _lib.lib().mpn_dwconv_wgrad_num_parts(N, H, W, C, stride, dc)
    if wpart is None:
        wpart = _f32(rows * 9 * C, x.device)
    if reduce_bn and bn_part is None:
        bn_part = _f32(rows * 2 * C, x.device)
    if wpart.numel() < rows * 9 * C or (reduce_bn and bn_part.numel() < rows * 2 * C):
        raise ValueError("dwconv_bwd_fused: partial slab too small")
    ab = apply_bn
    if ab is not None:
        aps = (ptr(ab.scale), ptr(ab.shift), ptr(ab.mean), ptr(ab.invstd), ptr(ab.k1), ptr(ab.k2), int(ab.act))
        name, add = ("mpn_dwconv_bwd_fused_s2_apply", (ptr(addend),)) if stride == 2 else ("mpn_dwconv_bwd_fused_apply", ())
        call(name, ptr(x), ptr(dy), ptr(y_raw), ptr(w), ptr(out), ptr(wpart), N, H, W, C, dc, ptr(bn.scale), ptr(bn.shift), int(bn.act),
             ptr(bn.mean), ptr(bn.invstd), ptr(bn_part) if reduce_bn else None, *add, *aps, stream_ptr())
    elif stride == 2:
        call("mpn_dwconv_bwd_fused_s2", ptr(x), ptr(dy), ptr(w), ptr(out), ptr(wpart), N, H, W, C, dc, ptr(bn.scale), ptr(bn.shift),
             int(bn.act), ptr(bn.mean), ptr(bn.invstd), ptr(bn_part) if reduce_bn else None, ptr(addend), stream_ptr())
    else:
        call("mpn_dwconv_bwd_fused", ptr(x), ptr(dy), ptr(w), ptr(out), ptr(wpart), N, H, W, C, dc, ptr(bn.scale), ptr(bn.shift),
             int(bn.act), ptr(bn.mean), ptr(bn.invstd), ptr(bn_part) if reduce_bn else None, stream_ptr())
    if reduce:
        call("mpn_reduce_partials", ptr(wpart), rows, 9 * C, ptr(dw_out), 0, 1.0, stream_ptr())
    return out, (rows if reduce_bn else 0)


def stem_conv_fwd_num_parts(N, H, W, c0, dtype):
    return _lib.lib().mpn_stem_conv_fwd_num_parts(N, H, W, c0, _lib.dtype_code(dtype))


def stem_conv_fwd(images, w, c0, dtype, out=None, stats_part=None):
    if images.dim() != 4 or images.shape[3] != 3 or not images.is_contiguous():
        raise ValueError("images must be contiguous [N,H,W,3]")
    u8 = images.dtype == torch.uint8
    if not u8 and images.dtype != torch.float32:
        raise ValueError("images must be float32 in [0,1] or uint8")
    N, H, W, _ = images.shape
    if out is None:
        out = torch.empty((N, (H + 1) // 2, (W + 1) // 2, c0), dtype=dtype, device=images.device)
    if stats_part is not None:
        rows = stem_conv_fwd_num_parts(N, H, W, c0, dtype)
        if rows <= 0 or stats_part.numel() < rows * 2 * c0:
            raise ValueError("stem_conv_fwd: fused statistics not available for this shape, or slab too small")
        call("mpn_stem_conv_fwd_stats", ptr(images), int(u8), ptr(w), ptr(out), N, H, W, c0, _lib.dtype_code(dtype),
             ptr(stats_part), stream_ptr())
        return out
    call("mpn_stem_conv_fwd", ptr(images), int(u8), ptr(w), ptr(out), N, H, W, c0, _lib.dtype_code(dtype), stream_ptr())
    return out


def stem_conv_bwd_weight(images, dy, dw_out, part=None, reduce=True):
    N, H, W, _ = images.shape
    c0 = dy.shape[3]
    nparts = _lib.lib().mpn_stem_conv_wgrad_num_parts(N, H, W)
    if part is None:
        part = _f32(nparts * 27 * c0, dy.device)
    call("mpn_stem_conv_bwd_weight", ptr(images), int(images.dtype == torch.uint8), ptr(dy), ptr(part), N, H, W, c0,
         _lib.dtype_code(dy.dtype), stream_ptr())
    if reduce:
        call("mpn_reduce_partials", ptr(part), nparts, 27 * c0, ptr(dw_out), 0, 1.0, stream_ptr())
    return dw_out


def bilinear_up_fwd(x, upsample, out, channel_offset, affine=None):
    N, h, w, C = x.shape
    sc, sh, act = _aff(affine)
    call("mpn_bilinear_up_fwd", ptr(x), ptr(out), N, h, w, C, upsample, channel_offset, out.shape[3],
         _lib.dtype_code(x.dtype), sc, sh, act, stream_ptr())
    return out


def bilinear_up_bwd(dy, upsample, channel_offset, C, out=None):
    N, OH, OW, ctot = dy.shape
    h, w = OH // upsample, OW // upsample
    if out is None:
        out = torch.empty((N, h, w, C), dtype=dy.dtype, device=dy.device)
    call("mpn_bilinear_up_bwd", ptr(dy), ptr(out), N, h, w, C, upsample, channel_offset, ctot, _lib.dtype_code(dy.dtype),
         stream_ptr())
    return out


def sumpool2x2(src, dst=None, accumulate=False):
    N, H2, W2, C = src.shape
    if dst is None:
        dst = torch.empty((N, H2 // 2, W2 // 2, C), dtype=src.dtype, device=src.device)
    call("mpn_sumpool2x2", ptr(src), ptr(dst), N, H2 // 2, W2 // 2, C, int(accumulate), _lib.dtype_code(src.dtype), stream_ptr())
    return dst


def add_inplace(dst, src):
    if dst.shape != src.shape or dst.dtype != src.dtype:
        raise ValueError("add_inplace: shape/dtype mismatch")
    call("mpn_add_inplace", ptr(dst), ptr(src), dst.numel(), _lib.dtype_code(dst.dtype), stream_ptr())
    return dst


def heatmap_head_fwd(x, w, bias, affine, inference=False, out=None, out_seg=None):
    N, H, W, cin = x.shape
    M = N * H * W
    sc, sh, act = _aff(affine)
    if inference:
        if out is None:
            out = torch.empty((N, H, W, 17), dtype=torch.float32, device=x.device)
        if out_seg is None:
            out_seg = torch.empty((N, H, W), dtype=torch.float32, device=x.device)
    elif out is None:
        out = torch.empty((N, H, W, 18), dtype=torch.float32, device=x.device)
    call("mpn_heatmap_head_fwd", ptr(x), ptr(w), ptr(bias), M, cin, _lib.dtype_code(x.dtype), sc, sh, act,
         int(inference), ptr(out), ptr(out_seg), stream_ptr())
    return (out, out_seg) if inference else out


def heatmap_head_bwd_bn_supported(cin, dtype):
    return bool(_lib.lib().mpn_heatmap_head_bwd_bn_supported(int(cin), _lib.dtype_code(dtype)))


def heatmap_head_bwd(x, dlogits, w, affine, dA, dw_db_out, part=None, reduce=True, bn_part=None):
    N, H, W, cin = x.shape
    M = N * H * W
    nparts = _lib.lib().mpn_heatmap_head_bwd_num_parts(M)
    nout = cin * 18 + 18
    if part is None:
        part = _f32(nparts * nout, x.device)
    sc, sh, act = _aff(affine)
    if bn_part is not None:
        if bn_part.numel() < nparts * 2 * cin:
            raise ValueError("heatmap_head_bwd: bn_part too small")
        call("mpn_heatmap_head_bwd_bn", ptr(x), ptr(dlogits), ptr(w), M, cin, _lib.dtype_code(x.dtype), sc, sh, act, ptr(dA),
             ptr(part), ptr(bn_part), stream_ptr())
    else:
        call("mpn_heatmap_head_bwd", ptr(x), ptr(dlogits), ptr(w), M, cin, _lib.dtype_code(x.dtype), sc, sh, act, ptr(dA),
             ptr(part), stream_ptr())
    if reduce:
        call("mpn_reduce_partials", ptr(part), nparts, nout, ptr(dw_db_out), 0, 1.0, stream_ptr())
    return nparts if bn_part is not None else dA


LOSS_NAMES = ["focal_loss", "regression_loss", "segmentation_loss_at_level_2", "segmentation_loss_at_level_3",
              "segmentation_loss_at_level_4", "segmentation_loss_at_level_5", "total_loss", "per_pixel_reg_loss"]


def keypoint_loss(logits, labels, ps, dlogits=None, daux=None, part=None, losses_out=None):
    B, h, w, _ = logits.shape
    dev = logits.device
    nparts = _lib.lib().mpn_keypoint_loss_num_parts(B, h, w)
    if part is None:
# ... 120 lines not shown
```

Baseline: 4367 images/s.

## Fold BN backward apply into pointwise and stem weight-gradient kernels

Adds variants of the 1x1 conv weight-gradient kernel and the stem weight-gradient kernel that apply the batch-norm backward elementwise transform while staging dy. This lets bn_backward skip its separate apply pass for wide pointwise layers and the stem. The pointwise variant also writes the applied gradient to a scratch buffer so the data-gradient conv can consume it. The aim is to remove a full read/write pass over activation gradients, at the cost of more LDS, extra loads in the staging path and bit-exact emulation of the unfused rounding pattern.

```diff
diff --git a/include/mpn.h b/include/mpn.h
--- a/include/mpn.h
+++ b/include/mpn.h
@@ -78,6 +78,11 @@
                                 int dtype, const float* in_scale, const float* in_shift, int in_act, const float* ap_scale,
                                 const float* ap_shift, const float* ap_mean, const float* ap_invstd, const float* ap_k1,
                                 const float* ap_k2, int ap_act, mpn_stream_t stream);
+int mpn_conv_bwd_weight_apply_supported(int Cin, int Cout, int dtype);
+int mpn_conv_bwd_weight_apply(const void* x, const void* g, const void* y_raw, void* dy_out, float* part, int N, int H, int W, int Cin,
+                              int Cout, int x_stride, int g_stride, int y_stride, int ksize, int dtype, const float* in_scale,
+                              const float* in_shift, int in_act, const float* ap_scale, const float* ap_shift, const float* ap_mean,
+                              const float* ap_invstd, const float* ap_k1, const float* ap_k2, int ap_act, mpn_stream_t stream);
 int mpn_conv_wgrad_grouped_num_parts(int njobs, int N, const int* H, const int* W, int Cin, int Cout, int ksize, int dtype,
                                      int* nparts);
 int mpn_conv_bwd_weight_grouped(int njobs, const void* const* x, const void* const* dy, float* const* part, int N,
@@ -176,6 +181,10 @@
 int mpn_stem_conv_wgrad_num_parts(int N, int H, int W);
 int mpn_stem_conv_bwd_weight(const void* images, int images_u8, const void* dy, float* part, int N,
                              int H, int W, int C0, int dtype, mpn_stream_t stream);
+int mpn_stem_conv_bwd_weight_apply_supported(int C0, int dtype);
+int mpn_stem_conv_bwd_weight_apply(const void* images, int images_u8, const void* g, const void* y_raw, float* part, int N, int H, int W,
+                                   int C0, int dtype, const float* ap_scale, const float* ap_shift, const float* ap_mean,
+                                   const float* ap_invstd, const float* ap_k1, const float* ap_k2, int ap_act, mpn_stream_t stream);
 
 int mpn_bilinear_up_fwd(const void* x, void* y, int N, int h, int w, int C, int upsample,
                         int y_channel_offset, int y_channels_total, int dtype,
diff --git a/multiposenet_amd/_lib.py b/multiposenet_amd/_lib.py
--- a/multiposenet_amd/_lib.py
+++ b/multiposenet_amd/_lib.py
@@ -43,6 +43,8 @@
     "mpn_conv_bwd_weight": (_I, [_P, _P, _P, _I, _I, _I, _I, _I, _I, _I, _I, _I, _P, _P, _I, _P]),
     "mpn_conv1x1_bwd_fused_supported": (_I, [_I, _I, _I]),
     "mpn_conv1x1_bwd_fused": (_I, [_P, _P, _P, _P, _P, _P, _I, _I, _I, _I, _I, _I, _I, _I, _I, _P, _P, _I, _P]),
+    "mpn_conv_bwd_weight_apply_supported": (_I, [_I, _I, _I]),
+    "mpn_conv_bwd_weight_apply": (_I, [_P, _P, _P, _P, _P, _I, _I, _I, _I, _I, _I, _I, _I, _I, _I, _P, _P, _I, _P, _P, _P, _P, _P, _P, _I, _P]),
     "mpn_conv1x1_bwd_fused_apply_supported": (_I, [_I, _I, _I]),
     "mpn_conv1x1_bwd_fused_apply": (_I, [_P, _P, _P, _P, _P, _P, _P, _I, _I, _I, _I, _I, _I, _I, _I, _I, _I, _P, _P, _I, _P, _P, _P, _P, _P, _P, _I, _P]),
     "mpn_conv_wgrad_grouped_num_parts": (_I, [_I, _I, _P, _P, _I, _I, _I, _I, _P]),
@@ -76,6 +78,8 @@
     "mpn_stem_conv_fwd_stats": (_I, [_P, _I, _P, _P, _I, _I, _I, _I, _I, _P, _P]),
     "mpn_stem_conv_wgrad_num_parts": (_I, [_I, _I, _I]),
     "mpn_stem_conv_bwd_weight": (_I, [_P, _I, _P, _P, _I, _I, _I, _I, _I, _P]),
+    "mpn_stem_conv_bwd_weight_apply_supported": (_I, [_I, _I]),
+    "mpn_stem_conv_bwd_weight_apply": (_I, [_P, _I, _P, _P, _P, _I, _I, _I, _I, _I, _P, _P, _P, _P, _P, _P, _I, _P]),
     "mpn_bilinear_up_fwd": (_I, [_P, _P, _I, _I, _I, _I, _I, _I, _I, _I, _P, _P, _I, _P]),
     "mpn_bilinear_up_bwd": (_I, [_P, _P, _I, _I, _I, _I, _I, _I, _I, _I, _P]),
     "mpn_sumpool2x2": (_I, [_P, _P, _I, _I, _I, _I, _I, _I, _P]),
diff --git a/multiposenet_amd/csrc/bn_apply_exact.h b/multiposenet_amd/csrc/bn_apply_exact.h
--- /dev/null
+++ b/multiposenet_amd/csrc/bn_apply_exact.h
@@ -0,0 +1,9 @@
+#pragma once
+
+__device__ __forceinline__ bool bn_apply_pair67_unfused(unsigned elem) { return ((elem >> 11) & 3u) != 2u; }
+
+template <typename V> __device__ __forceinline__ V bn_apply_unfused(V sc, V g, V cb, V y, V cc) {
+#pragma clang fp contract(off)
+    const V t = cb * y, u = sc * g;
+    return (cc + t) + u;
+}
diff --git a/multiposenet_amd/csrc/conv_wgrad.hip b/multiposenet_amd/csrc/conv_wgrad.hip
--- a/multiposenet_amd/csrc/conv_wgrad.hip
+++ b/multiposenet_amd/csrc/conv_wgrad.hip
@@ -1,4 +1,5 @@
 #include "common.h"
+#include "bn_apply_exact.h"
 #include <type_traits>
 
 namespace {
@@ -32,6 +33,7 @@
     int ap_xs;
     const float* ap_scale; const float* ap_shift; const float* ap_mean; const float* ap_invstd; const float* ap_k1; const float* ap_k2;
     int ap_act;
+    void* ap_out;
 #ifdef MPN_DIAG
     unsigned long long* dbg;
 #endif
@@ -364,7 +366,7 @@
     Vec16<T> v[AVEC], dv[DVEC];
     Vec16<T> ev[DAPPLY ? DVEC : 1];
     unsigned inb = 0u, inbd = 0u;
-    static_assert(!DAPPLY || DG, "the apply pass folds into the fused thin backward");
+    static_assert(!DAPPLY || TAPS == 1, "the apply pass folds into the 1x1 staging (buffer loads)");
     float* apc = reinterpret_cast<float*>(Os + OBYTES + (DG ? 8 * 2 * CG * (int)sizeof(float) : 0));
     float alo = -INFINITY, ahi = INFINITY;
     if constexpr (DAPPLY) {
@@ -408,7 +410,8 @@
     constexpr bool BUF = TAPS == 1;
     typedef unsigned u32x4_t __attribute__((ext_vector_type(4)));
     unsigned relAb[BUF ? AVEC : 1], relDb[BUF ? DVEC : 1], relEb[(BUF && DAPPLY) ? DVEC : 1];
-    __amdgpu_buffer_rsrc_t rsx, rsd, rse;
+    __amdgpu_buffer_rsrc_t rsx, rsd, rse, rso;
+    unsigned tbDc = 0u;
     if constexpr (BUF) {
         constexpr unsigned kOut = 0x80000000u;
 #pragma unroll
@@ -422,6 +425,7 @@
             for (int i = 0; i < DVEC; ++i)
                 relEb[i] = dvalid ? (unsigned)((drow0 + i * (NT / DSLOTS)) * p.ap_xs + co0 + dslot * VE) * (unsigned)sizeof(T) : kOut;
             rse = __builtin_amdgcn_make_buffer_rsrc(const_cast<void*>(p.ap_x), 0, (int)(((p.M - 1) * p.ap_xs + p.Cout) * (long long)sizeof(T)), 0x00020000);
+            if constexpr (!DG) rso = __builtin_amdgcn_make_buffer_rsrc(p.ap_out, 0, (int)(p.M * p.Cout * (long long)sizeof(T)), 0x00020000);
         }
     }
 
@@ -435,12 +439,28 @@
 #pragma unroll
                 for (int i = 0; i < DVEC; ++i) md |= ((dvalid && drow0 + i * (NT / DSLOTS) < mleft) ? 1u : 0u) << i;
                 inbd = md;
+                tbDc = tbD;
             }
             __builtin_amdgcn_sched_barrier(0);
 #pragma unroll
             for (int i = 0; i < AVEC; ++i) {
                 const u32x4_t q = __builtin_amdgcn_raw_buffer_load_b128(rsx, (int)(relAb[i] + tbA), 0, 0);
                 v[i].raw = make_uint4(q.x, q.y, q.z, q.w);
+            }
+            if constexpr (DAPPLY && !DG) if (p.n_cg == 1) {
+                const unsigned tbE = (unsigned)tile * 128u * (unsigned)p.ap_xs * (unsigned)sizeof(T);
+#pragma unroll
+                for (int i = 0; i < DVEC; ++i) {
+                    const u32x4_t q = __builtin_amdgcn_raw_buffer_load_b128(rsd, (int)(relDb[i] + tbD), 0, 2);
+                    dv[i].raw = make_uint4(q.x, q.y, q.z, q.w);
+                }
+#pragma unroll
+                for (int i = 0; i < DVEC; ++i) {
+                    const u32x4_t q = __builtin_amdgcn_raw_buffer_load_b128(rse, (int)(relEb[i] + tbE), 0, 2);
+                    ev[i].raw = make_uint4(q.x, q.y, q.z, q.w);
+                }
+                __builtin_amdgcn_sched_barrier(0);
+                return;
             }
 #pragma unroll
             for (int i = 0; i < DVEC; ++i) {
@@ -566,11 +586,25 @@
 #pragma unroll
                     for (int j = 0; j < 4; ++j) { asc[j4 + j] = q0[j]; ash[j4 + j] = q1[j]; acb[j4 + j] = q2[j]; acc_[j4 + j] = q3[j]; }
                 }
-#pragma unroll
-                for (int j = 0; j < VE; ++j) {
-                    const float pre = f[j] * asc[j] + ash[j];
-                    const float gg = (pre > alo && pre < ahi) ? d[j] : 0.f;
-                    d[j] = asc[j] * gg + (acb[j] * f[j] + acc_[j]);
+                if constexpr (DG) {
+#pragma unroll
+                    for (int j = 0; j < VE; ++j) {
+                        const float pre = f[j] * asc[j] + ash[j];
+                        const float gg = (pre > alo && pre < ahi) ? d[j] : 0.f;
+                        d[j] = asc[j] * gg + (acb[j] * f[j] + acc_[j]);
+                    }
+                } else {
+                    float gg[VE];
+#pragma unroll
+                    for (int j = 0; j < VE; ++j) {
+                        const float pre = __builtin_fmaf(f[j], asc[j], ash[j]);
+                        gg[j] = (pre > alo && pre < ahi) ? d[j] : 0.f;
+                        d[j] = __builtin_fmaf(asc[j], gg[j], __builtin_fmaf(acb[j], f[j], acc_[j]));
+                    }
+                    if (bn_apply_pair67_unfused((relDb[i] + tbDc) >> 1)) {
+#pragma unroll
+                        for (int j = 6; j < VE; ++j) d[j] = bn_apply_unfused(asc[j], gg[j], acb[j], f[j], acc_[j]);
+                    }
                 }
                 Vec16<T> o;
                 o.pack(d);
@@ -578,6 +612,9 @@
             }
             if ((!BUF || DAPPLY) && !((inbd >> i) & 1u)) q = make_uint4(0u, 0u, 0u, 0u);
             *reinterpret_cast<uint4*>(Ds + r * SD + dslot * 16) = q;
+            if constexpr (DAPPLY && !DG) {
+                if (cg == 0) __builtin_amdgcn_raw_buffer_store_b128((u32x4_t){q.x, q.y, q.z, q.w}, rso, (int)(relDb[i] + tbDc), 0, 0);
+            }
         }
     };
 
@@ -784,9 +821,9 @@
                 }
 }
 
-template <typename T, int TAPS, int RBA, int RBD, int WM, bool STAGGER>
+template <typename T, int TAPS, int RBA, int RBD, int WM, bool STAGGER, bool DAPPLY = false>
 __global__ __launch_bounds__(512, 1) void conv_wgrad_bf16_kernel(const WgradParams p) {
-    conv_wgrad_bf16_body<T, TAPS, RBA, RBD, WM, STAGGER>(p, blockIdx.x, gridDim.x);
+    conv_wgrad_bf16_body<T, TAPS, RBA, RBD, WM, STAGGER, false, DAPPLY>(p, blockIdx.x, gridDim.x);
 }
 
 template <typename T, int RBA, int RBD, int WM, bool DAPPLY>
@@ -842,8 +879,9 @@
     return g;
 }
 
-template <int TAPS, int RBA, int RBD> constexpr int wgrad16_smem_bytes() {
-    constexpr int smem = 2 * (TAPS == 9 ? kHaloW * kHaloH : 128) * (RBA + 32) + 2 * 128 * (RBD + 32) + 2 * (RBA / 2) * (int)sizeof(float);
+template <int TAPS, int RBA, int RBD, bool DAPPLY = false> constexpr int wgrad16_smem_bytes() {
+    constexpr int smem = 2 * (TAPS == 9 ? kHaloW * kHaloH : 128) * (RBA + 32) + 2 * 128 * (RBD + 32) + 2 * (RBA / 2) * (int)sizeof(float) +
+                         (DAPPLY ? 4 * (RBD / 2) * (int)sizeof(float) : 0);
     static_assert(smem <= 160 * 1024, "LDS budget");
     return smem;
 }
@@ -874,12 +912,12 @@
     return begin;
 }
 
-template <typename T, int TAPS, int RBA, int RBD, int WM, bool STAGGER>
+template <typename T, bool DAPPLY = false, int TAPS, int RBA, int RBD, int WM, bool STAGGER>
 int launch_wgrad_bf16(Wgrad16<TAPS, RBA, RBD, WM, STAGGER>, const WgradParams& p, hipStream_t st) {
-    constexpr int smem = wgrad16_smem_bytes<TAPS, RBA, RBD>();
+    constexpr int smem = wgrad16_smem_bytes<TAPS, RBA, RBD, DAPPLY>();
     static mpn_attr_mask_t attr_mask{0};
-    MPN_HIP(mpn_ensure_dynamic_lds((const void*)conv_wgrad_bf16_kernel<T, TAPS, RBA, RBD, WM, STAGGER>, smem, &attr_mask));
-    conv_wgrad_bf16_kernel<T, TAPS, RBA, RBD, WM, STAGGER><<<dim3((unsigned)(p.n_cg * p.n_cb * p.nsplit)), dim3(512), smem, st>>>(p);
+    MPN_HIP(mpn_ensure_dynamic_lds((const void*)conv_wgrad_bf16_kernel<T, TAPS, RBA, RBD, WM, STAGGER, DAPPLY>, smem, &attr_mask));
+    conv_wgrad_bf16_kernel<T, TAPS, RBA, RBD, WM, STAGGER, DAPPLY><<<dim3((unsigned)(p.n_cg * p.n_cb * p.nsplit)), dim3(512), smem, st>>>(p);
     MPN_LAUNCH_CHECK();
     return MPN_OK;
 }
@@ -982,6 +1020,39 @@
     if (dtype == MPN_F16)
         return wgrad16_dispatch(Cin, Cout, ksize, [&](auto geo) { return launch_wgrad_bf16<half_t>(geo, p, st); });
     return wgrad16_dispatch(Cin, Cout, ksize, [&](auto geo) { return launch_wgrad_bf16<bf16_t>(geo, p, st); });
+}
+
+extern "C" int mpn_conv_bwd_weight_apply_supported(int Cin, int Cout, int dtype) {
+    if (dtype != MPN_BF16 || Cin <= 0 || Cout <= 0 || Cin % 8 != 0 || Cout % 8 != 0 || wgrad_thin1x1(Cin, Cout, 1)) return 0;
+    const int cvec = Cout / 8;
+    return ((cvec & (cvec - 1)) == 0 && cvec <= 256) ? 1 : 0;
+}
+
+extern "C" int mpn_conv_bwd_weight_apply(const void* x, const void* g, const void* y_raw, void* dy_out, float* part, int N, int H, int W,
+                                         int Cin, int Cout, int x_stride, int g_stride, int y_stride, int ksize, int dtype,
+                                         const float* in_scale, const float* in_shift, int in_act, const float* ap_scale,
+                                         const float* ap_shift, const float* ap_mean, const float* ap_invstd, const float* ap_k1,
+                                         const float* ap_k2, int ap_act, mpn_stream_t stream) {
+    const char* who = "conv wgrad apply";
+    if (int rc = wgrad_check_layer(who, N, Cin, Cout, ksize, dtype)) return rc;
+    MPN_REQUIRE(ksize == 1 && mpn_conv_bwd_weight_apply_supported(Cin, Cout, dtype), MPN_ERR_BAD_SHAPE,
+                "%s: layer not covered (ksize %d, Cin %d, Cout %d, dtype %d)", who, ksize, Cin, Cout, dtype);
+    MPN_REQUIRE(y_raw && dy_out && ap_scale && ap_shift && ap_mean && ap_invstd && ap_k1 && ap_k2, MPN_ERR_BAD_ARG, "%s: null pointer", who);
+    MPN_REQUIRE(mpn_aligned16(y_raw) && mpn_aligned16(dy_out), MPN_ERR_BAD_ALIGN, "%s: pointers must be 16-byte aligned", who);
+    MPN_REQUIRE(dy_out != g && dy_out != y_raw && dy_out != x, MPN_ERR_BAD_ARG, "%s: dy_out must not alias an input", who);
+    MPN_REQUIRE((g_stride == 0 || g_stride == Cout) && (y_stride == 0 || y_stride == Cout), MPN_ERR_BAD_SHAPE,
+                "%s: g and y_raw must be dense", who);
+    const WgradGeom geo = wgrad_geom(N, H, W, Cin, Cout, 1, 2);
+    WgradParams p;
+    if (int rc = wgrad_fill_job(p, who, x, g, part, N, H, W, Cin, Cout, x_stride, g_stride, 1, 2, in_scale, in_shift, in_act, geo, geo.nsplit))
+        return rc;
+    p.ap_x = y_raw; p.ap_xs = Cout; p.ap_out = dy_out;
+    p.ap_scale = ap_scale; p.ap_shift = ap_shift; p.ap_mean = ap_mean; p.ap_invstd = ap_invstd; p.ap_k1 = ap_k1; p.ap_k2 = ap_k2; p.ap_act = ap_act;
+    hipStream_t st = (hipStream_t)stream;
+    return wgrad16_dispatch(Cin, Cout, 1, [&](auto g16) {
+        if constexpr (std::is_same_v<decltype(g16), Wgrad16<1, 256, 256, 4, false>>) return launch_wgrad_bf16<bf16_t, true>(g16, p, st);
+        else return (int)MPN_ERR_BAD_SHAPE;
+    });
 }
 
 namespace {
diff --git a/multiposenet_amd/csrc/dwconv_walk.h b/multiposenet_amd/csrc/dwconv_walk.h
--- a/multiposenet_amd/csrc/dwconv_walk.h
+++ b/multiposenet_amd/csrc/dwconv_walk.h
@@ -1,5 +1,6 @@
 #pragma once
 #include "common.h"
+#include "bn_apply_exact.h"
 
 namespace {
 
@@ -200,19 +201,14 @@
         cc01 = (f32x2_t){cc_[0], cc_[1]}; cc23 = (f32x2_t){cc_[2], cc_[3]};
         pair67 = (cc & 4) != 0;
     }
-    static __device__ __forceinline__ f32x2_t unfused(f32x2_t sc, f32x2_t g, f32x2_t cb, f32x2_t y, f32x2_t cc) {
-#pragma clang fp contract(off)
-        const f32x2_t t = cb * y, u = sc * g;
-        return (cc + t) + u;
-    }
     __device__ __forceinline__ void apply(float (&f)[4], const Raw4<T>& yr, unsigned elem) const {
         f32x2_t y01, y23;
         raw_unpack2(yr, y01, y23);
         const f32x2_t g01 = {f[0], f[1]}, g23 = {f[2], f[3]};
         const f32x2_t o01 = __builtin_elementwise_fma(sc01, g01, __builtin_elementwise_fma(cb01, y01, cc01));
         f32x2_t o23 = __builtin_elementwise_fma(sc23, g23, __builtin_elementwise_fma(cb23, y23, cc23));
-        const f32x2_t v23 = unfused(sc23, g23, cb23, y23, cc23);
-        if (pair67 && ((elem >> 11) & 3u) != 2u) o23 = v23;
+        const f32x2_t v23 = bn_apply_unfused(sc23, g23, cb23, y23, cc23);
+        if (pair67 && bn_apply_pair67_unfused(elem)) o23 = v23;
         const f32x2_t r01 = round_storage<T>(o01), r23 = round_storage<T>(o23);
         f[0] = r01.x; f[1] = r01.y; f[2] = r23.x; f[3] = r23.y;
     }
diff --git a/multiposenet_amd/csrc/stem.hip b/multiposenet_amd/csrc/stem.hip
--- a/multiposenet_amd/csrc/stem.hip
+++ b/multiposenet_amd/csrc/stem.hip
@@ -1,4 +1,5 @@
 #include "common.h"
+#include "bn_apply_exact.h"
 
 namespace {
 
@@ -395,10 +396,16 @@
     }
 }
 
-template <bool U8, int MB>
+struct StemApply {
+    const bf16_t* y_raw;
+    const float *scale, *shift, *mean, *invstd, *k1, *k2;
+    int act;
+};
+template <bool U8, int MB, bool APPLY = false>
 __global__ __launch_bounds__(kThreads) void stem_wgrad_mfma_kernel(const void* __restrict__ images, const bf16_t* __restrict__ dy,
                                                                    float* __restrict__ part, int N, int H, int W, int OH, int OW,
-                                                                   int pad_t, int pad_l, int tiles_x, int tiles_y) {
+                                                                   int pad_t, int pad_l, int tiles_x, int tiles_y,
+                                                                   const StemApply ap = StemApply{}) {
     typedef H16<bf16_t> HT;
     typedef HT::x8 x8;
     typedef HT::x4 x4;
@@ -408,6 +415,7 @@
     extern __shared__ __attribute__((aligned(16))) unsigned char stem_smem[];
     float* patch = reinterpret_cast<float*>(stem_smem);
     unsigned char* dimg = stem_smem + kPR * kPS * sizeof(float);
+    float* apc = reinterpret_cast<float*>(dimg + kTile * kFwdTW * DRS);
     const int ntiles = N * tiles_y * tiles_x;
     const int lane = threadIdx.x & 63, wv = threadIdx.x >> 6;
     const int n = lane & 15, kg = lane >> 4, q = n >> 2, pq = n & 3;
@@ -415,6 +423,21 @@
     constexpr int DV = kTile * kFwdTW * VPP / kThreads;
     float pv[kPR];
     uint4 dv[DV];
+    uint4 yv[APPLY ? DV : 1];
+    int ctile = 0;
+    float alo = -INFINITY, ahi = INFINITY;
+    if constexpr (APPLY) {
+        static_assert(kThreads % VPP == 0, "a thread keeps its channel vector");
+        for (int c = threadIdx.x; c < C0; c += kThreads) {
+            const float s_ = ap.scale[c], m_ = ap.mean[c], i_ = ap.invstd[c], a_ = ap.k1[c], b_ = ap.k2[c];
+            apc[c] = s_; apc[C0 + c] = ap.shift[c];
+            apc[2 * C0 + c] = -s_ * b_ * i_;
+            apc[3 * C0 + c] = -s_ * (a_ - m_ * i_ * b_);
+        }
+        alo = (ap.act != MPN_ACT_NONE) ? 0.f : -INFINITY;
+        ahi = (ap.act == MPN_ACT_RELU6) ? 6.f : INFINITY;
+        __syncthreads();
+    }
     unsigned long long pmask = 0ull;
     unsigned dmask = 0u;
     const int p_pc = threadIdx.x < kPC ? threadIdx.x : 0;
@@ -448,9 +471,17 @@
             const int vq = i % VPP, px = i / VPP;
             const int oy = ty * kTile + px / kFwdTW, ox = tx * kFwdTW + px % kFwdTW;
             const bool ok = oy < OH && ox < OW;
-            dv[k] = *reinterpret_cast<const uint4*>(dy + (ok ? (((long long)img * OH + oy) * OW + ox) * C0 + vq * 8 : 0));
+            const long long off = ok ? (((long long)img * OH + oy) * OW + ox) * C0 + vq * 8 : 0;
+            if constexpr (APPLY) {
+                Vec16<bf16_t> a, b;
+                a.load_nt(dy + off); b.load_nt(ap.y_raw + off);
+                dv[k] = a.raw; yv[k] = b.raw;
+            } else {
+                dv[k] = *reinterpret_cast<const uint4*>(dy + off);
+            }
             dmask |= (ok ? 1u : 0u) << k;
         }
+        ctile = t;
     };
     auto commit_tile = [&]() __attribute__((always_inline)) {
         int tid = threadIdx.x;
@@ -460,11 +491,47 @@
             for (int py = 0; py < kPR; ++py)
                 patch[py * kPS + p_pc] = ((pmask >> py) & 1ull) ? 2.0f * pv[py] - 1.0f : 0.0f;
         }
+        float asc[8], ash[8], acb[8], acc_[8];
+        unsigned pix0 = 0u;
+        if constexpr (APPLY) {
+            const int vq = tid % VPP;
+#pragma unroll
+            for (int j4 = 0; j4 < 8; j4 += 4) {
+                const float4 q0 = *reinterpret_cast<const float4*>(apc + vq * 8 + j4), q1 = *reinterpret_cast<const float4*>(apc + C0 + vq * 8 + j4);
+                const float4 q2 = *reinterpret_cast<const float4*>(apc + 2 * C0 + vq * 8 + j4), q3 = *reinterpret_cast<const float4*>(apc + 3 * C0 + vq * 8 + j4);
+                asc[j4] = q0.x; asc[j4 + 1] = q0.y; asc[j4 + 2] = q0.z; asc[j4 + 3] = q0.w;
+                ash[j4] = q1.x; ash[j4 + 1] = q1.y; ash[j4 + 2] = q1.z; ash[j4 + 3] = q1.w;
+                acb[j4] = q2.x; acb[j4 + 1] = q2.y; acb[j4 + 2] = q2.z; acb[j4 + 3] = q2.w;
+                acc_[j4] = q3.x; acc_[j4 + 1] = q3.y; acc_[j4 + 2] = q3.z; acc_[j4 + 3] = q3.w;
+            }
+            const int tx = ctile % tiles_x, t2 = ctile / tiles_x;
+            pix0 = ((unsigned)(t2 / tiles_y) * (unsigned)OH + (unsigned)((t2 % tiles_y) * kTile)) * (unsigned)OW + (unsigned)(tx * kFwdTW);
+        }
 #pragma unroll
         for (int k = 0; k < DV; ++k) {
             const int i = tid + k * kThreads;
             const int vq = i % VPP, px = i / VPP;
-            *reinterpret_cast<uint4*>(dimg + px * DRS + vq * 16) = ((dmask >> k) & 1u) ? dv[k] : make_uint4(0u, 0u, 0u, 0u);
+            uint4 q = dv[k];
+            if constexpr (APPLY) {
+                Vec16<bf16_t> a, b;
+                a.raw = dv[k]; b.raw = yv[k];
+                float d[8], f[8], gg[8];
+                a.unpack(d); b.unpack(f);
+#pragma unroll
+                for (int j = 0; j < 8; ++j) {
+                    const float pre = __builtin_fmaf(f[j], asc[j], ash[j]);
+                    gg[j] = (pre > alo && pre < ahi) ? d[j] : 0.f;
+                    d[j] = __builtin_fmaf(asc[j], gg[j], __builtin_fmaf(acb[j], f[j], acc_[j]));
+                }
+                const unsigned elem = (pix0 + (unsigned)(px / kFwdTW) * (unsigned)OW + (unsigned)(px % kFwdTW)) * (unsigned)C0 + (unsigned)vq * 8u;
+                if (bn_apply_pair67_unfused(elem)) {
+#pragma unroll
+                    for (int j = 6; j < 8; ++j) d[j] = bn_apply_unfused(asc[j], gg[j], acb[j], f[j], acc_[j]);
+                }
+                a.pack(d);
+                q = a.raw;
+            }
+            *reinterpret_cast<uint4*>(dimg + px * DRS + vq * 16) = ((dmask >> k) & 1u) ? q : make_uint4(0u, 0u, 0u, 0u);
         }
     };
     int kbase[2];
@@ -545,8 +612,19 @@
 
 template <bool U8, int MB>
 int launch_stem_wgrad_mfma(int grid, hipStream_t st, const void* images, const void* dy, float* part, int N, int H, int W, int OH,
-                           int OW, int pt, int pl, int tiles_x, int tiles_y) {
+                           int OW, int pt, int pl, int tiles_x, int tiles_y, const StemApply* ap = nullptr) {
     constexpr int sm = kPR * kPS * (int)sizeof(float) + kTile * kFwdTW * (16 * MB * 2 + 16);
+    if (ap != nullptr) {
+        if constexpr (kThreads % (2 * MB) == 0) {
+            constexpr int sma = sm + 4 * 16 * MB * (int)sizeof(float);
+            static mpn_attr_mask_t attr_mask_a{0};
+            MPN_HIP(mpn_ensure_dynamic_lds((const void*)stem_wgrad_mfma_kernel<U8, MB, true>, sma, &attr_mask_a));
+            stem_wgrad_mfma_kernel<U8, MB, true><<<grid, kThreads, sma, st>>>(images, (const bf16_t*)dy, part, N, H, W, OH, OW, pt, pl, tiles_x,
+                                                                             tiles_y, *ap);
+            return MPN_OK;
+        }
+        return MPN_ERR_BAD_SHAPE;
+    }
     static mpn_attr_mask_t attr_mask{0};
     MPN_HIP(mpn_ensure_dynamic_lds((const void*)stem_wgrad_mfma_kernel<U8, MB>, sm, &attr_mask));
     stem_wgrad_mfma_kernel<U8, MB><<<grid, kThreads, sm, st>>>(images, (const bf16_t*)dy, part, N, H, W, OH, OW, pt, pl, tiles_x, tiles_y);
@@ -639,8 +717,36 @@
     return ntiles < 512 ? ntiles : 512;
 }
 
+namespace {
+int stem_conv_bwd_weight_impl(const void* images, int images_u8, const void* dy, float* part, int N, int H, int W, int C0, int dtype,
+                              const StemApply* ap, mpn_stream_t stream);
+}
+
 extern "C" int mpn_stem_conv_bwd_weight(const void* images, int images_u8, const void* dy, float* part, int N, int H, int W,
                                         int C0, int dtype, mpn_stream_t stream) {
+    return stem_conv_bwd_weight_impl(images, images_u8, dy, part, N, H, W, C0, dtype, nullptr, stream);
+}
+
+extern "C" int mpn_stem_conv_bwd_weight_apply_supported(int C0, int dtype) {
+    return (dtype == MPN_BF16 && C0 > 0 && C0 <= kMaxC0 && C0 % 16 == 0 && ((C0 / 8) & (C0 / 8 - 1)) == 0) ? 1 : 0;
+}
+
+extern "C" int mpn_stem_conv_bwd_weight_apply(const void* images, int images_u8, const void* g, const void* y_raw, float* part, int N,
+                                              int H, int W, int C0, int dtype, const float* ap_scale, const float* ap_shift,
+                                              const float* ap_mean, const float* ap_invstd, const float* ap_k1, const float* ap_k2,
+                                              int ap_act, mpn_stream_t stream) {
+    if (int rc = check(N, H, W, C0, dtype)) return rc;
+    MPN_REQUIRE(mpn_stem_conv_bwd_weight_apply_supported(C0, dtype), MPN_ERR_BAD_SHAPE, "stem_wgrad_apply: stem not covered (C0 %d, dtype %d)",
+                C0, dtype);
+    MPN_REQUIRE(y_raw && ap_scale && ap_shift && ap_mean && ap_invstd && ap_k1 && ap_k2, MPN_ERR_BAD_ARG, "stem_wgrad_apply: null pointer");
+    MPN_REQUIRE(mpn_aligned16(g) && mpn_aligned16(y_raw), MPN_ERR_BAD_ALIGN, "stem_wgrad_apply: pointers must be 16-byte aligned");
+    const StemApply ap = {(const bf16_t*)y_raw, ap_scale, ap_shift, ap_mean, ap_invstd, ap_k1, ap_k2, ap_act};
+    return stem_conv_bwd_weight_impl(images, images_u8, g, part, N, H, W, C0, dtype, &ap, stream);
+}
+
+namespace {
+int stem_conv_bwd_weight_impl(const void* images, int images_u8, const void* dy, float* part, int N, int H, int W, int C0, int dtype,
+                              const StemApply* ap, mpn_stream_t stream) {
     if (int rc = check(N, H, W, C0, dtype)) return rc;
     MPN_REQUIRE(images && dy && part, MPN_ERR_BAD_ARG, "stem_wgrad: null pointer");
     int OH, OW, pt, pl;
@@ -654,8 +760,8 @@
         const int tx32 = (OW + kFwdTW - 1) / kFwdTW;
         int rc;
 #define MPN_STEM_WG(MB)                                                                                                         \
-    rc = images_u8 ? launch_stem_wgrad_mfma<true, MB>(grid, st, images, dy, part, N, H, W, OH, OW, pt, pl, tx32, tiles_y)       \
-                   : launch_stem_wgrad_mfma<false, MB>(grid, st, images, dy, part, N, H, W, OH, OW, pt, pl, tx32, tiles_y)
+    rc = images_u8 ? launch_stem_wgrad_mfma<true, MB>(grid, st, images, dy, part, N, H, W, OH, OW, pt, pl, tx32, tiles_y, ap)   \
+                   : launch_stem_wgrad_mfma<false, MB>(grid, st, images, dy, part, N, H, W, OH, OW, pt, pl, tx32, tiles_y, ap)
         switch (C0 / 16) {
             case 1: MPN_STEM_WG(1); break;
             case 2: MPN_STEM_WG(2); break;
@@ -678,3 +784,4 @@
     MPN_LAUNCH_CHECK();
     return MPN_OK;
 }
+}
diff --git a/multiposenet_amd/net.py b/multiposenet_amd/net.py
--- a/multiposenet_amd/net.py
+++ b/multiposenet_amd/net.py
@@ -101,6 +101,9 @@
 
 
 DP_DEEP_FROM_BLOCK = 7
+
+
+PW_APPLY_MAX_CIN_TILES = 1
 
 
 def backbone_deep_begin_of(arena, first_block=DP_DEEP_FROM_BLOCK):
@@ -170,6 +173,7 @@
         self._head_grad = self.grad[ok:ob + nb]
         self.fuse_dw_bn = True
         self.fuse_dw_apply = True
+        self.fuse_pw_apply = True
         self.fuse_conv_bn = True
         self._l2 = None
         self._wd = None
@@ -290,6 +294,8 @@
         g["pw"] = [torch.empty_like(t) for t in b["pw"]]
         g["dw"] = [torch.empty_like(t) for t in b["dw"]]
         g["stem"] = torch.empty_like(b["stem"])
+        folded = [t.numel() for blk, t in zip(self.blocks, b["pw"]) if self._pw_folds_apply(blk["pw"])]
+        g["pw_applied"] = torch.empty(max(folded), dtype=dt, device=dev) if folded else None
         lib, dc = ops._lib.lib(), ops._lib.dtype_code(dt)
         sites = []
         grouped_np = {}
@@ -568,8 +574,12 @@
         if phase == 1:
             g["bb_chain"] = (dA, reduced, lateral_added)
             return
-        ops.bn_backward(self.stem_bn, g["stem"], b["stem"], sp, reduced_parts=reduced)
-        ops.stem_conv_bwd_weight(images, g["stem"], self.stem_dw, slab[id(self.stem_dw)], reduce=False)
+        fold = self.fuse_pw_apply and ops.stem_conv_bwd_weight_apply_supported(g["stem"].shape[3], self.dtype)
+        ops.bn_backward(self.stem_bn, g["stem"], b["stem"], sp, reduced_parts=reduced, apply=not fold)
+        if fold:
+            ops.stem_conv_bwd_weight_apply(images, g["stem"], b["stem"], self.stem_bn, slab[id(self.stem_dw)])
+        else:
+            ops.stem_conv_bwd_weight(images, g["stem"], self.stem_dw, slab[id(self.stem_dw)], reduce=False)
 
     def _dw_lateral(self, g, i):
         return g["c"][FEATURE_BLOCKS[self.blocks[i - 1]["i"]]] if i > 0 and self.blocks[i - 1]["i"] in FEATURE_BLOCKS else None
@@ -583,20 +593,31 @@
         s, (N, _, _, C) = self.blocks[i]["stride"], b["dw"][i].shape
         return (self.fuse_dw_apply and self._dw_walks_fused(b, g, i)
                 and ops.dwconv_bwd_fused_apply_supported(N, *b["hw"][i], C, s, self.dtype))
+
+    def _pw_folds_apply(self, pw):
+        thin = self.fuse_conv_bn and ops.conv1x1_bwd_fused_supported(pw.cin, pw.cout, self.dtype) and pw.cin <= 64
+        return (self.fuse_pw_apply and not thin and (pw.cin + 127) // 128 <= PW_APPLY_MAX_CIN_TILES
+                and ops.conv_bwd_weight_apply_supported(pw.cin, pw.cout, self.dtype))
 
     def _backward_pointwise(self, b, g, sp, slab, i, dA, reduced, raw, fold=False):
         blk = self.blocks[i]
         pw, x, dY = blk["pw"], b["dw"][i], g["dw"][i]
         fused = self.fuse_conv_bn and ops.conv1x1_bwd_fused_supported(pw.cin, pw.cout, self.dtype) and pw.cin <= 64
         apply = fused and ops.conv1x1_bwd_fused_apply_supported(pw.cin, pw.cout, self.dtype)
-        ops.bn_backward(blk["pw_bn"], dA, b["pw"][i], sp, reduced_parts=reduced, raw=raw, apply=not apply)
+        wg_apply = not fused and g.get("pw_applied") is not None and self._pw_folds_apply(pw)
+        ops.bn_backward(blk["pw_bn"], dA, b["pw"][i], sp, reduced_parts=reduced, raw=raw, apply=not (apply or wg_apply))
         rows = 0
         with _lib.tagged("pointwise"):
             if fused:
                 rows = ops.conv1x1_bwd_fused(x, dA, pw.w, blk["dw_bn"], dY, slab[id(pw.dw)], sp,
                                              apply_bn=blk["pw_bn"] if apply else None, y_raw=b["pw"][i] if apply else None)
             else:
-                ops.conv_bwd_weight(x, dA, 1, blk["dw_bn"].affine, pw.dw, slab[id(pw.dw)], reduce=False)
+                if wg_apply:
+                    applied_dA = g["pw_applied"][:dA.numel()].view(dA.shape)
+                    ops.conv_bwd_weight_apply(x, dA, b["pw"][i], blk["pw_bn"], blk["dw_bn"].affine, applied_dA, slab[id(pw.dw)])
+                    dA = applied_dA
+                else:
+                    ops.conv_bwd_weight(x, dA, 1, blk["dw_bn"].affine, pw.dw, slab[id(pw.dw)], reduce=False)
                 if self.fuse_conv_bn and ops.conv_bwd_data_bn_supported(pw.cout, pw.cin, 1, self.dtype):
                     rows = ops.conv_bwd_data_bn(dA, pw.packed.bwd, pw.cin, 1, blk["dw_bn"], x, dY, sp)
                 else:
diff --git a/multiposenet_amd/ops.py b/multiposenet_amd/ops.py
--- a/multiposenet_amd/ops.py
+++ b/multiposenet_amd/ops.py
@@ -189,6 +189,22 @@
     if reduce:
         call("mpn_reduce_partials", ptr(part), nparts, n, ptr(dw_out), 0, 1.0, stream_ptr())
     return dw_out
+
+
+def conv_bwd_weight_apply_supported(cin, cout, dtype):
+    return _lib.lib().mpn_conv_bwd_weight_apply_supported(int(cin), int(cout), _lib.dtype_code(dtype)) == 1
+
+
+def conv_bwd_weight_apply(x, g, y_raw, apply_bn, affine, dy_out, part):
+    N, H, W, cin = x.shape
+    cout = g.shape[3]
+    if part.numel() < conv_wgrad_num_parts(N, H, W, cin, cout, 1, x.dtype) * cin * cout or dy_out.numel() < g.numel():
+        raise ValueError("conv_bwd_weight_apply: partial slab or dy_out too small")
+    sc, sh, act = _aff(affine)
+    a = apply_bn
+    call("mpn_conv_bwd_weight_apply", ptr(x), ptr(g), ptr(y_raw), ptr(dy_out), ptr(part), N, H, W, cin, cout, _slice_stride(x, cin),
+         _slice_stride(g, cout), _slice_stride(y_raw, cout), 1, _lib.dtype_code(x.dtype), sc, sh, act, ptr(a.scale), ptr(a.shift),
+         ptr(a.mean), ptr(a.invstd), ptr(a.k1), ptr(a.k2), int(a.act), stream_ptr())
 
 
 class SlabReducer:
@@ -582,6 +598,20 @@
     return dw_out
 
 
+def stem_conv_bwd_weight_apply_supported(c0, dtype):
+    return _lib.lib().mpn_stem_conv_bwd_weight_apply_supported(int(c0), _lib.dtype_code(dtype)) == 1
+
+
+def stem_conv_bwd_weight_apply(images, g, y_raw, apply_bn, part):
+    N, H, W, _ = images.shape
+    c0 = g.shape[3]
+    if part.numel() < _lib.lib().mpn_stem_conv_wgrad_num_parts(N, H, W) * 27 * c0 or not (g.is_contiguous() and y_raw.is_contiguous()):
+        raise ValueError("stem_conv_bwd_weight_apply: partial slab too small or strided tensors")
+    a = apply_bn
+    call("mpn_stem_conv_bwd_weight_apply", ptr(images), int(images.dtype == torch.uint8), ptr(g), ptr(y_raw), ptr(part), N, H, W, c0,
+         _lib.dtype_code(g.dtype), ptr(a.scale), ptr(a.shift), ptr(a.mean), ptr(a.invstd), ptr(a.k1), ptr(a.k2), int(a.act), stream_ptr())
+
+
 def bilinear_up_fwd(x, upsample, out, channel_offset, affine=None):
     N, h, w, C = x.shape
     sc, sh, act = _aff(affine)
```

Measured after the change: 4406 images/s (median of 6 runs). About the same (+0.9%).
